# Darkkey/erlamsa

Measured on AMD Instinct MI355X. Metric: mutated_MB_per_s, higher is better.
Workload: dtype u8 (byte edits) + f64 (AS183 draws)

## Files before the change

erlamsa_amd/csrc/eh_common.h:

```cpp
#pragma once
#include <stdint.h>

#if defined(__HIP_DEVICE_COMPILE__) && !defined(HIPEMU)
#define EH_G __attribute__((address_space(1)))
#else
#define EH_G
#endif

namespace eh {

typedef EH_G uint8_t* bptr;   typedef const EH_G uint8_t* cbptr;
typedef EH_G uint32_t* wptr;  typedef const EH_G uint32_t* cwptr;
typedef EH_G uint64_t* qptr;  typedef const EH_G uint64_t* cqptr;

enum MutaId : int {
  M_SGM, M_JS, M_UW, M_UI, M_AB, M_AD, M_TR2, M_TD, M_NUM, M_TS1, M_TR, M_TS2, M_BD, M_BEI, M_BED,
  M_BF, M_BI, M_BER, M_BR, M_SP, M_SR, M_SD, M_SNAND, M_SRND, M_LD, M_LDS, M_LR2, M_LRI, M_LR,
  M_LS, M_LP, M_LIS, M_LRS, M_FT, M_FN, M_FO, M_LEN, M_B64, M_URI, M_ZIP, M_NIL, M_COUNT
};
enum PatId : int { P_OD, P_ND, P_BU, P_SK, P_SZ, P_CS, P_AR, P_CP, P_CO, P_NU, P_COUNT };
enum GenId : int { G_DIRECT = 0, G_RANDOM = 1, G_FILE = 2, G_JUMP = 3, G_COUNT = 4 };

enum CaseStatus : int { CASE_OK = 0, CASE_CRASHED = 1, CASE_OVERFLOW = 2, CASE_UNSUPPORTED = 3, CASE_ARENA_FULL = 4, CASE_BUDGET = 5 };

constexpr int MAX_FS = 64;
constexpr int MAX_BLOCKS = 2048;
constexpr int MAX_EMITS = 4096;
constexpr int MAX_FRAMES = 16;
constexpr uint32_t TRACE_CAP = 32768;

enum TraceKind : int {
  TRK_AA = 1,
  TRK_AI = 2,
  TRK_SIZER = 3,
  TRK_CSUM = 4,
  TRK_SKIPPED = 5,
  TRK_ARCHIVER = 6,
};
#define EH_ATOMS(X)                                                                                                              \
  X(sgm) X(js) X(uw) X(ui) X(ab) X(ad) X(tr2) X(td) X(num) X(ts1) X(tr) X(ts2) X(bd) X(bei) X(bed) X(bf) X(bi) X(ber) X(br) X(sp)  \
  X(sr) X(sd) X(snand) X(srnd) X(ld) X(lds) X(lr2) X(lri) X(lr) X(ls) X(lp) X(lis) X(lrs) X(ft) X(fn) X(fo) X(len) X(b64) X(uri)  \
  X(zip) X(nil)                                                                                                                   \
  X(failed) X(used) X(pattern) X(skipped_big) X(once_dec) X(many_dec) X(burst) X(skipper) X(sizer) X(csum) X(archiver)            \
  X(compressed) X(no_muta) X(mutate_once) X(empty_stopped) X(decompressed) X(gzip) X(zlib) X(ok) X(success) X(json)               \
  X(base64_mutator) X(sed_utf8_widen) X(sed_utf8_insert) X(ascii_bad) X(ascii_delimeter) X(tree_dup) X(tree_del) X(muta_num)      \
  X(tree_swap_one) X(tree_stutter) X(tree_swap_two) X(byte_drop) X(byte_inc) X(byte_dec) X(byte_flip) X(byte_insert)              \
  X(byte_swap_random) X(byte_repeat) X(seq_perm) X(seq_repeat) X(seq_drop) X(seq_randmask) X(line_del) X(line_del_seq)            \
  X(line_dup) X(line_clone) X(line_repeat) X(line_swap) X(line_perm) X(list_ins) X(list_replace) X(fuse_this) X(fuse_next)        \
  X(fuse_old) X(muta_len) X(muta_zippath) X(nomutation) X(json_swap) X(json_dup) X(json_pump) X(json_repeat) X(json_insert)       \
  X(json_unserialize) X(json_innertext) X(null) X(bool) X(sgml_swap) X(sgml_dup) X(sgml_pump) X(sgml_repeat) X(sgml_insert2)      \
  X(sgml_permparams) X(sgml_breaktag) X(sgml_insert) X(sgml_xmlfeatures) X(xmlns) X(sgml_innertext)
enum AtomId : int {
#define EH_ATOM_ENUM(n) AT_##n,
  EH_ATOMS(EH_ATOM_ENUM)
#undef EH_ATOM_ENUM
  AT_COUNT
};
static_assert((int)AT_nil == (int)M_NIL && (int)AT_sgm == (int)M_SGM && (int)AT_b64 == (int)M_B64, "the mutator codes are the first atoms, in MutaId order");
constexpr int POOL_TIERS = 8;

constexpr uint32_t INITIAL_IP = 24;
constexpr uint32_t AVG_BLOCK_SIZE = 2048;
constexpr uint32_t MIN_BLOCK_SIZE = 256;
constexpr uint32_t MAX_BLOCK_SIZE = 4096;
constexpr uint32_t ABSMAXHALF_BINARY_BLOCK = 500000;
constexpr uint32_t ABSMAX_BINARY_BLOCK = 1000000;
constexpr uint32_t SIZER_MAX_FIRST_BYTES = 512;
constexpr uint32_t PREAMBLE_MAX_BYTES = 32;

struct Blk {
  uint64_t ptr;
  uint32_t len;
  uint32_t aux;
};

struct RunState {
  uint32_t a1, a2, a3;
  int32_t gen;
  int32_t nfs;
  int32_t snand_mask;
  uint8_t fs_name[MAX_FS];
  uint8_t fs_score[MAX_FS];
  uint32_t fs_pri[MAX_FS];
};

struct DevConfig {
  int32_t nsel;
  uint8_t sel_name[MAX_FS];
  uint32_t sel_pri[MAX_FS];
  int32_t npat;
  int32_t pat_total;
  uint8_t pat_id[P_COUNT];
  uint32_t pat_pri[P_COUNT];
  int32_t ngen;
  int32_t gen_total;
  uint8_t gen_id[G_COUNT];
  uint32_t gen_pri[G_COUNT];
  uint32_t max_block_scaled;
  uint32_t min_block_scaled;
  char ssrf_host[64];
  char ssrf_port[12];
};

constexpr uint32_t MAX_PROFILES = 1024;
struct ProfileCfg {
  int32_t nsel;
  uint8_t sel_name[MAX_FS];
  uint32_t sel_pri[MAX_FS];
  int32_t npat;
  int32_t pat_total;
  uint8_t pat_id[P_COUNT];
  uint8_t pad[2];
  uint32_t pat_pri[P_COUNT];
  uint32_t max_block_scaled;
  uint32_t min_block_scaled;
};

constexpr uint32_t CO_JOBS = 64, CO_ARGS = 12;
enum CoKind : uint32_t { CO_COPY = 1, CO_EQUAL = 2, CO_FBPASS = 3, CO_FBCOUNT = 4 };
struct CoJob {
  uint64_t a[CO_ARGS];
  unsigned long long acc;
  uint32_t kind, nchunks, done, pad;
};
struct CoBoard {
  unsigned long long word[CO_JOBS];
  uint32_t owner[CO_JOBS];
  uint32_t open;
  uint32_t posters;
  uint32_t pad[14];
  unsigned long long stat[8];
  CoJob job[CO_JOBS];
};

struct KParams {
  cbptr corpus;
  cqptr coff;
  uint64_t corpus_first;
  uint64_t n_paths;
  uint64_t n;
  uint64_t first_case;
  int32_t mode;
  const EH_G RunState* run;
  const EH_G int64_t* seeds;
  DevConfig cfg;
  uint64_t work_cap;
  uint64_t work_budget;
  uint64_t fuse_stream_min;
  bptr out;
  uint64_t out_cap;
  EH_G unsigned long long* out_cursor;
  qptr out_off;
  qptr out_len;
  EH_G int32_t* status;
  qptr draws;
  EH_G int32_t* lastm;
  qptr cycles;
  qptr peak;
  qptr trace_off;
  wptr trace_len;
  uint32_t flags;
  EH_G unsigned long long* prof;
  EH_G unsigned long long* ticket;
  EH_G unsigned long long* in_bytes;
  bptr slot_base;
  uint64_t slot_stride;
  int32_t ntiers;
  bptr pool_base[POOL_TIERS + 1];
  uint64_t pool_stride[POOL_TIERS + 1];
  uint64_t pool_cap[POOL_TIERS + 1];
  uint32_t pool_cnt[POOL_TIERS + 1];
  wptr pool_ring[POOL_TIERS + 1];
  EH_G unsigned long long* pool_ctr;
  EH_G CoBoard* board;
  EH_G unsigned long long* summary_out;
  uint64_t batch_seq;
  uint32_t co_copy_min, co_copy_chunk;
  uint32_t co_fb_min, co_fb_chunk;
  uint32_t co_linger, pad_co;
  const EH_G ProfileCfg* profiles;
  const EH_G uint32_t* profile_id;
};

struct MutaInfo { const char* name; int pri; int on_gpu; };
struct PatInfo { const char* name; int pri; int on_gpu; };

}
```

erlamsa_amd/csrc/eh_device.h:

```cpp
#pragma once
#include <hip/hip_runtime.h>
#include <stdint.h>

#include "eh_common.h"

namespace eh {

#define EH_LANE ((int)threadIdx.x)
#define EH_DEV __device__ __forceinline__

EH_DEV uint32_t uni(uint32_t v) { return (uint32_t)__builtin_amdgcn_readfirstlane((int)v); }
EH_DEV uint64_t uni64(uint64_t v) { return ((uint64_t)uni((uint32_t)(v >> 32)) << 32) | uni((uint32_t)v); }
EH_DEV void wave_sync() { __syncthreads(); }

struct alignas(16) TabU16x65 { uint16_t v[65]; };
constexpr TabU16x65 as183_powers(uint32_t mult, uint32_t prime) {
  TabU16x65 t{};
  uint32_t a = 1;
  for (int k = 0; k <= 64; k++) { t.v[k] = (uint16_t)a; a = a * mult % prime; }
  return t;
}
__constant__ TabU16x65 c_T1 = as183_powers(171, 30269);
__constant__ TabU16x65 c_T2 = as183_powers(172, 30307);
__constant__ TabU16x65 c_T3 = as183_powers(170, 30323);
// ... 98 lines not shown
EH_DEV bool rng_occurs(Rng& r, uint32_t nom, uint32_t den) {
  uint32_t n = rng_rand(r, den);
  return nom == 1 ? (n != 0) : (n < nom);
}
EH_DEV uint32_t rng_log(Rng& r, uint32_t n) {
  if (n == 0) return 0;
  uint32_t k = rng_rand(r, n);
  if (k == 0) return 0;
  uint32_t hi = 1u << (k - 1);
  return hi | rng_rand(r, hi);
}

#ifdef HIPEMU
EH_DEV uint4 ldg16(const void* p) { uint4 v; memcpy(&v, p, 16); return v; }
EH_DEV uint4 ldg16a(const void* p) { uint4 v; memcpy(&v, p, 16); return v; }
EH_DEV void stg16(void* p, const uint4& v) { memcpy(p, &v, 16); }
EH_DEV void stg16a(void* p, const uint4& v) { memcpy(p, &v, 16); }
EH_DEV uint64_t ldg8(const void* p) { uint64_t v; memcpy(&v, p, 8); return v; }
EH_DEV uint32_t ldg4(const void* p) { uint32_t v; memcpy(&v, p, 4); return v; }
#else
typedef uint32_t eh_v4 __attribute__((ext_vector_type(4)));
typedef eh_v4 __attribute__((aligned(1))) eh_v4u;
typedef uint64_t __attribute__((aligned(1))) eh_u64u;
typedef uint32_t __attribute__((aligned(1))) eh_u32u;
EH_DEV uint4 ldg16(const EH_G void* p) { eh_v4 v = *reinterpret_cast<const EH_G eh_v4u*>(p); uint4 r; r.x = v.x; r.y = v.y; r.z = v.z; r.w = v.w; return r; }
EH_DEV uint4 ldg16a(const EH_G void* p) { eh_v4 v = *reinterpret_cast<const EH_G eh_v4*>(p); uint4 r; r.x = v.x; r.y = v.y; r.z = v.z; r.w = v.w; return r; }
EH_DEV void stg16(EH_G void* p, const uint4& r) { eh_v4 v; v.x = r.x; v.y = r.y; v.z = r.z; v.w = r.w; *reinterpret_cast<EH_G eh_v4u*>(p) = v; }
EH_DEV void stg16a(EH_G void* p, const uint4& r) { eh_v4 v; v.x = r.x; v.y = r.y; v.z = r.z; v.w = r.w; *reinterpret_cast<EH_G eh_v4*>(p) = v; }
EH_DEV uint64_t ldg8(const EH_G void* p) { return *reinterpret_cast<const EH_G eh_u64u*>(p); }
EH_DEV uint32_t ldg4(const EH_G void* p) { return *reinterpret_cast<const EH_G eh_u32u*>(p); }
#endif

#ifdef HIPEMU
constexpr uint32_t CO_COPY_MIN = 8u << 10;
#else
constexpr uint32_t CO_COPY_MIN = 256u << 10;
#endif
__device__ void co_copy(bptr dst, cbptr src, uint32_t n);
__device__ bool co_equal(cbptr a, cbptr b, uint32_t n);
EH_DEV void wave_copy_raw(bptr dst, cbptr src, uint32_t n) {
  const int l = EH_LANE;
  uint32_t head = (uint32_t)((16 - ((uintptr_t)dst & 15)) & 15);
  if (head > n) head = n;
  if ((uint32_t)l < head) dst[l] = src[l];
  dst += head; src += head; n -= head;
  uint32_t nv = n >> 4;
  uint32_t i = l;
  for (; i + 192 < nv; i += 256) {
    const uint4 v0 = ldg16(src + 16 * (size_t)i), v1 = ldg16(src + 16 * (size_t)(i + 64));
    const uint4 v2 = ldg16(src + 16 * (size_t)(i + 128)), v3 = ldg16(src + 16 * (size_t)(i + 192));
    stg16a(dst + 16 * (size_t)i, v0);
    stg16a(dst + 16 * (size_t)(i + 64), v1);
    stg16a(dst + 16 * (size_t)(i + 128), v2);
    stg16a(dst + 16 * (size_t)(i + 192), v3);
  }
  for (; i < nv; i += 64) {
    const uint4 v = ldg16(src + 16 * (size_t)i);
    stg16a(dst + 16 * (size_t)i, v);
  }
  uint32_t done = nv << 4;
  if (done + l < n) dst[done + l] = src[done + l];
}
EH_DEV void wave_copy(bptr dst, cbptr src, uint32_t n) {
  if (__builtin_expect(n >= CO_COPY_MIN, 0)) { co_copy(dst, src, n); return; }
  wave_copy_raw(dst, src, n);
}
EH_DEV void wave_move_down(bptr dst, cbptr src, uint32_t n) {
  const int l = EH_LANE;
  uint32_t nv = n >> 4;
  for (uint32_t base = 0; base < nv; base += 256) {
    uint4 v[4]; bool ok[4];
#pragma unroll
    for (int u = 0; u < 4; u++) { uint32_t i = base + 64u * u + (uint32_t)l; ok[u] = i < nv; if (ok[u]) v[u] = ldg16(src + 16 * (size_t)i); }
    wave_sync();
#pragma unroll
    for (int u = 0; u < 4; u++) { uint32_t i = base + 64u * u + (uint32_t)l; if (ok[u]) stg16(dst + 16 * (size_t)i, v[u]); }
  }
  uint32_t done = nv << 4;
  uint8_t t = 0; bool tk = done + (uint32_t)l < n;
  if (tk) t = src[done + l];
  wave_sync();
  if (tk) dst[done + l] = t;
}
EH_DEV void wave_fill_periodic(bptr dst, cbptr pat, uint32_t plen, uint64_t total) {
  if (total == 0) return;
  uint64_t have = plen < total ? plen : total;
  wave_copy(dst, pat, (uint32_t)have);
  while (have < total) {
    wave_sync();
    uint64_t chunk = have < total - have ? have : total - have;
    uint64_t done = 0;
    while (done < chunk) { uint32_t c = chunk - done > 0x40000000ull ? 0x40000000u : (uint32_t)(chunk - done); wave_copy(dst + have + done, dst + done, c); done += c; }
    have += chunk;
  }
}
EH_DEV bool wave_equal_raw(cbptr a, cbptr b, uint32_t n) {
  const int l = EH_LANE;
  uint32_t nv = n >> 4;
  for (uint32_t base = 0; base < nv; base += 128) {
    uint32_t i0 = base + l, i1 = base + 64 + l;
    bool ne = false;
    uint4 x0, y0, x1, y1;
    if (i0 < nv) { x0 = ldg16(a + 16 * (size_t)i0); y0 = ldg16(b + 16 * (size_t)i0); }
    if (i1 < nv) { x1 = ldg16(a + 16 * (size_t)i1); y1 = ldg16(b + 16 * (size_t)i1); }
    if (i0 < nv) ne |= (x0.x != y0.x) | (x0.y != y0.y) | (x0.z != y0.z) | (x0.w != y0.w);
    if (i1 < nv) ne |= (x1.x != y1.x) | (x1.y != y1.y) | (x1.z != y1.z) | (x1.w != y1.w);
    if (__ballot(ne) != 0) return false;
  }
  uint32_t done = nv << 4;
  bool ne = false;
  if (done + l < n) ne = a[done + l] != b[done + l];
  return __ballot(ne) == 0;
}
EH_DEV bool wave_equal(cbptr a, cbptr b, uint32_t n) {
  if (__builtin_expect(n >= CO_COPY_MIN, 0)) return co_equal(a, b, n);
  return wave_equal_raw(a, b, n);
}

constexpr int MAX_CHUNKS = POOL_TIERS + 1;
constexpr int MAX_NEST = 6;
constexpr int LEX_LEVELS = MAX_NEST + 1;
constexpr int ST_STATE_WORDS = 84;
#define EH_SET_OVERFLOW(c, site) ((c).ovf_line = (site), (c).ovf_need = 0, (c).ovf_req = 0, (c).status = CASE_OVERFLOW)
struct MuFrame;
struct Ctx {
  Rng rng;
  const EH_G KParams* p;
  EH_G Blk* bl;
  EH_G Blk* bl2;
  int nb, cur;
  EH_G Blk* em;
  int nem;
  uint32_t max_block_scaled;
  bptr aux;
  bptr ws;
  uint64_t ws_used, ws_cap;
  int nchunk;
  int view;
  uint64_t ws_lo;
  uint64_t ch_vstart[MAX_CHUNKS], ch_vend[MAX_CHUNKS]; bptr ch_base[MAX_CHUNKS]; uint32_t ch_area[MAX_CHUNKS]; int32_t ch_tier[MAX_CHUNKS];
  uint64_t lex_ptr[LEX_LEVELS];
  bptr trace;
  uint32_t ntrace, tr_base;
  uint32_t co_posted;
  int32_t call_req, mu_phase, call_nres, call_nfs;
  uint64_t call_bin; uint32_t call_len;
  EH_G MuFrame* mu;
  uint64_t t_case;
  uint32_t min_block_scaled;
  int32_t m_aux;
  uint64_t ws_peak, ws_top;
  int status;
  int lastm;
  uint64_t work;
  int r_kind;
  bptr r_ptr;
  uint32_t r_len;
  int r_flush;
  int r_drop_next;
  int r_changed;
  int r2; bptr r2_ptr; uint32_t r2_len;
  int nfs;
  uint64_t work_budget;
  uint64_t ovf_need, ovf_req;
  int ovf_line;
  int depth;
  int gen_pending;
  uint32_t gen_e1, gen_e2;
  int pat_ret; uint32_t pat_ip; int pat_cont;
  uint32_t fp_on, fp_g, fp_special, fp_keypos, fp_bA, fp_bB;
};
__shared__ Ctx g_ctx;
#ifdef HIPEMU
#define EH_LDS_ARRAY(type, name, n) static type name[n]
#define EH_KEEP(v) do {} while (0)
#else
// ... 35 lines not shown
  if (nb > 1) tr_b(c, b1);
  if (nv > 0) tr_v(c, v0);
  if (nv > 1) tr_v(c, v1);
  if (nv > 2) tr_v(c, v2);
}
__device__ __noinline__ void tr_name_emit(cbptr nm, uint32_t nl, uint32_t up) {
  Ctx& c = g_ctx;
  tr_b(c, TRK_ARCHIVER); tr_v(c, nl + 3u * up);
  for (uint32_t k = 0; k < up; k++) { tr_b(c, '.'); tr_b(c, '.'); tr_b(c, '/'); }
  for (uint32_t k = 0; k < nl; k++) tr_b(c, uni(nm[k]));
}
EH_DEV void tr_aa(Ctx& c, int a, int b) { if (__builtin_expect(c.trace != nullptr, 0)) tr_aa_emit(a, b); }
EH_DEV void tr_ai(Ctx& c, int a, int64_t v) { if (__builtin_expect(c.trace != nullptr, 0)) tr_ai_emit(a, v); }
EH_DEV void tr_drop_before(Ctx& c, uint32_t start) {
  if (!c.trace || start <= c.tr_base || c.ntrace >= TRACE_CAP) return;
  const uint32_t n = c.ntrace - start;
  wave_sync();
  if (n) wave_move_down(c.trace + c.tr_base, c.trace + start, n);
  wave_sync();
  c.ntrace = c.tr_base + n;
}

EH_DEV void pool_nap() {
#ifndef HIPEMU
  __builtin_amdgcn_s_sleep(64);
#else
  fprintf(stderr, "hipemu: a wait for a pool area can never end with one wavefront running (block %u)\n", blockIdx.x); abort();
#endif
}
EH_DEV uint32_t pool_pop(const EH_G KParams& p, int t) {
  uint32_t v = 0xFFFFFFFFu;
  if (EH_LANE == 0) {
    unsigned long long h = atomicAdd(&p.pool_ctr[2 * t], 1ull);
    wptr e = p.pool_ring[t] + (h % p.pool_cnt[t]);
    v = atomicExch(e, 0xFFFFFFFFu);
    if (v == 0xFFFFFFFFu) {
      uint64_t w0 = __builtin_readcyclecounter();
      for (;;) { pool_nap(); v = atomicExch(e, 0xFFFFFFFFu); if (v != 0xFFFFFFFFu) break; }
      atomicAdd(&p.pool_ctr[20 + t], (unsigned long long)(__builtin_readcyclecounter() - w0));
      atomicAdd(&p.pool_ctr[30 + t], 1ull);
    }
    unsigned long long back = atomicAdd(&p.pool_ctr[2 * t + 1], 0ull);
    unsigned long long outn = h + 1 + p.pool_cnt[t] > back ? h + 1 + p.pool_cnt[t] - back : 0;
    atomicMax(&p.pool_ctr[40 + t], outn);
  }
#ifndef EH_NO_POOL_FENCE
  __threadfence();
#endif
  return uni(v);
}
EH_DEV void pool_push(const EH_G KParams& p, int t, uint32_t v) {
#ifndef EH_NO_POOL_FENCE
  __threadfence();
#endif
  if (EH_LANE == 0) {
    unsigned long long h = atomicAdd(&p.pool_ctr[2 * t + 1], 1ull);
    wptr e = p.pool_ring[t] + (h % p.pool_cnt[t]);
    while (atomicCAS(e, 0xFFFFFFFFu, v) != 0xFFFFFFFFu) pool_nap();
  }
}

struct CoArgs { uint64_t a[CO_ARGS]; };
__device__ void co_exec(const EH_G CoJob* j, uint32_t t);
EH_DEV void co_nap() {
#ifndef HIPEMU
  __builtin_amdgcn_s_sleep(16);
#else
  fprintf(stderr, "hipemu: a wait for a helper's chunk can never end with one wavefront running (block %u)\n", blockIdx.x); abort();
#endif
}
EH_DEV void co_release() {
#ifndef HIPEMU
  __builtin_amdgcn_fence(__ATOMIC_RELEASE, "agent");
  asm volatile("s_waitcnt vmcnt(0)" ::: "memory");
#endif
}
EH_DEV void co_acquire() {
#ifndef HIPEMU
  __builtin_amdgcn_fence(__ATOMIC_ACQUIRE, "agent");
#endif
}
EH_DEV uint32_t co_ld32(const EH_G uint32_t* p) { return __atomic_load_n(p, __ATOMIC_RELAXED); }
EH_DEV unsigned long long co_ld64(const EH_G unsigned long long* p) { return __atomic_load_n(p, __ATOMIC_RELAXED); }
__device__ __noinline__ bool co_run(uint32_t kind, uint32_t nchunks, CoArgs args, unsigned long long* acc) {
  Ctx& c = g_ctx;
  EH_G CoBoard* bd = c.p ? c.p->board : nullptr;
  const int l = EH_LANE;
  if (!bd || nchunks < 2) return false;
  uint32_t slot = CO_JOBS;
  if (l == 0) {
    const uint32_t h = (blockIdx.x * 2654435761u) >> 26;
    for (uint32_t k = 0; k < 4 && slot == CO_JOBS; k++) { const uint32_t s = (h + 17u * k) & (CO_JOBS - 1); if (atomicCAS(&bd->owner[s], 0u, 1u) == 0u) slot = s; }
    if (slot == CO_JOBS) atomicAdd(&bd->stat[4], 1ull);
  }
  slot = uni(slot);
  if (slot == CO_JOBS) return false;
  EH_G CoJob* j = &bd->job[slot];
  unsigned long long gen = 0;
  if (l == 0) {
#pragma unroll
    for (uint32_t k = 0; k < CO_ARGS; k++) j->a[k] = args.a[k];
    j->kind = kind; j->nchunks = nchunks; j->done = 0; j->acc = 0;
  }
  wave_sync();
  co_release();
  if (l == 0) {
    if (!c.co_posted) atomicAdd(&bd->posters, 1u);
    gen = ((co_ld64(&bd->word[slot]) >> 32) + 1ull) | 1ull;
    atomicExch(&bd->word[slot], gen << 32);
    atomicAdd(&bd->open, 1u);
    atomicAdd(&bd->stat[0], 1ull);
  }
  c.co_posted = 1;
  uint32_t mine = 0;
  for (;;) {
    unsigned long long old = 0;
    if (l == 0) old = atomicAdd(&bd->word[slot], 1ull);
    const uint32_t t = uni((uint32_t)old);
    if (t >= nchunks) break;
    co_exec(j, t);
    mine++;
  }
  wave_sync();
  unsigned long long sum = 0;
  if (l == 0) {
    atomicAdd(&j->done, mine);
    const uint64_t w0 = __builtin_readcyclecounter();
    while (co_ld32(&j->done) < nchunks) co_nap();
    atomicAdd(&bd->open, 0xFFFFFFFFu);
    atomicExch(&bd->word[slot], (gen + 1ull) << 32);
    sum = co_ld64(&j->acc);
    atomicAdd(&bd->stat[2], (unsigned long long)mine);
    atomicAdd(&bd->stat[3], (unsigned long long)(__builtin_readcyclecounter() - w0));
  }
  sum = uni64(sum);
  co_acquire();
  if (l == 0) atomicExch(&bd->owner[slot], 0u);
  if (acc) *acc = sum;
  return true;
}
__device__ __noinline__ void co_help(EH_G CoBoard* bd, uint32_t most) {
  const int l = EH_LANE;
  uint32_t ran = 0;
  for (uint32_t guard = 0; guard < 64 && ran < most; guard++) {
    if (uni(co_ld32(&bd->open)) == 0) return;
    const unsigned long long w = co_ld64(&bd->word[l]);
    const bool cand = ((w >> 32) & 1ull) && (uint32_t)w < co_ld32(&bd->job[l].nchunks);
    unsigned long long m = __ballot(cand);
    if (!m) return;
    const uint32_t rot = blockIdx.x & 63u;
    const unsigned long long mr = rot ? ((m >> rot) | (m << (64u - rot))) : m;
    const uint32_t s = ((uint32_t)__builtin_ctzll(mr) + rot) & 63u;
    unsigned long long old = 0;
    if (l == 0) old = atomicAdd(&bd->word[s], 1ull);
    old = uni64(old);
    if (!((old >> 32) & 1ull)) continue;
    co_acquire();
    const EH_G CoJob* j = &bd->job[s];
    const uint32_t nchunks = uni(co_ld32(&j->nchunks)), t = (uint32_t)old;
    if (uni64(co_ld64(&bd->word[s])) >> 32 != old >> 32 || t >= nchunks) continue;
    co_exec(j, t);
    ran++;
    wave_sync();
    co_release();
    if (l == 0) { atomicAdd(&bd->job[s].done, 1u); atomicAdd(&bd->stat[1], 1ull); }
  }
}
__device__ __noinline__ void co_copy(bptr dst, cbptr src, uint32_t n) {
  const EH_G KParams* kp = g_ctx.p;
  if (!kp || !kp->board || n < kp->co_copy_min) { wave_copy_raw(dst, src, n); return; }
  const uint32_t ch = kp->co_copy_chunk;
  CoArgs a; for (uint32_t k = 0; k < CO_ARGS; k++) a.a[k] = 0;
  a.a[0] = (uint64_t)dst; a.a[1] = (uint64_t)src; a.a[2] = n; a.a[3] = ch;
  if (!co_run(CO_COPY, (n + ch - 1) / ch, a, nullptr)) wave_copy_raw(dst, src, n);
}
__device__ __noinline__ bool co_equal(cbptr x, cbptr y, uint32_t n) {
  const EH_G KParams* kp = g_ctx.p;
  if (!kp || !kp->board || n < 2 * kp->co_copy_min) return wave_equal_raw(x, y, n);
  const uint32_t ch = kp->co_copy_chunk;
  CoArgs a; for (uint32_t k = 0; k < CO_ARGS; k++) a.a[k] = 0;
  a.a[0] = (uint64_t)x; a.a[1] = (uint64_t)y; a.a[2] = n; a.a[3] = ch;
  unsigned long long ne = 0;
  if (!co_run(CO_EQUAL, (n + ch - 1) / ch, a, &ne)) return wave_equal_raw(x, y, n);
  return ne == 0;
}

struct LexChunk;
struct LexCache { uint64_t ptr; uint32_t len; int32_t n; EH_G LexChunk* tab; uint32_t tcap; uint32_t pad; };
constexpr uint32_t AUX_LEXCACHE = 2048;
constexpr uint64_t AUX_BYTES = 4096;
constexpr uint64_t SLOT_TABLE_BYTES = (uint64_t)(2 * MAX_BLOCKS + MAX_EMITS) * sizeof(Blk) + AUX_BYTES + TRACE_CAP;
EH_DEV EH_G LexCache& lex_slot(Ctx& c) { return ((EH_G LexCache*)(c.aux + AUX_LEXCACHE))[c.depth]; }
EH_DEV void lex_forget_from(Ctx& c, uint64_t v0) {
  const uint64_t key = c.lex_ptr[c.depth];
  if (key == 0) return;
  bool dead = false;
  for (int j = 0; j <= c.nchunk; j++) {
    uint64_t v = key - (uint64_t)(uintptr_t)c.ch_base[j], lo = v0 > c.ch_vstart[j] ? v0 : c.ch_vstart[j];
    if (v >= lo && v < c.ch_vstart[j] + c.p->pool_cap[c.ch_tier[j]]) dead = true;
  }
  if (dead) { c.lex_ptr[c.depth] = 0; if (EH_LANE == 0) lex_slot(c).n = -1; }
}
EH_DEV void ws_set_view(Ctx& c, int j) { c.view = j; c.ws = c.ch_base[j]; c.ws_lo = c.ch_vstart[j]; c.ws_cap = c.ch_vend[j]; }
EH_DEV bool ws_slow(Ctx& c, uint64_t need, int site) {
  int j = c.nchunk;
  while (j > 0 && c.ws_used < c.ch_vstart[j]) j--;
  for (; j <= c.nchunk; j++) {
    uint64_t at = c.ws_used > c.ch_vstart[j] ? c.ws_used : c.ch_vstart[j];
    if (at + need <= c.ch_vend[j]) { c.ws_used = at; ws_set_view(c, j); return true; }
  }
  const int k = c.nchunk;
  EH_SET_OVERFLOW(c, site); c.ovf_need = c.ws_used + need + (c.ch_vstart[k] + c.p->pool_cap[c.ch_tier[k]] - c.ch_vend[k]); c.ovf_req = need;
  return false;
}
EH_DEV uint64_t ws_max_request(const Ctx& c) { return c.p->pool_cap[c.p->ntiers]; }
EH_DEV bptr ws_alloc(Ctx& c, uint64_t n) {
  uint64_t need = (n + 15) & ~(uint64_t)15;
  if ((c.ws_used < c.ws_lo || c.ws_used + need > c.ws_cap) && !ws_slow(c, need, 102)) return nullptr;
  bptr p = c.ws + c.ws_used;
  c.ws_used += need;
  if (c.ws_used > c.ws_peak) c.ws_peak = c.ws_used;
  return p;
}
EH_DEV bptr ws_alloc_top(Ctx& c, uint64_t n) {
  uint64_t need = (n + 15) & ~(uint64_t)15;
  if ((c.ws_used < c.ws_lo || c.ws_used + need > c.ws_cap) && !ws_slow(c, need, 501)) return nullptr;
  c.ws_cap -= need; c.ch_vend[c.view] = c.ws_cap; c.ws_top += need;
  return c.ws + c.ws_cap;
}
__device__ __noinline__ void ws_release_to(Ctx&, uint64_t mark) {
  Ctx& c = g_ctx;
  c.ws_used = mark;
  while (c.nchunk > 0 && mark <= c.ch_vstart[c.nchunk]) {
    const int k = c.nchunk;
    const EH_G KParams& p = *c.p;
    bptr lo = c.ch_base[k] + c.ch_vstart[k]; bptr hi = lo + p.pool_cap[c.ch_tier[k]];
    for (int d = 0; d < LEX_LEVELS; d++) {
      EH_G LexCache* lc = (EH_G LexCache*)(c.aux + AUX_LEXCACHE) + d;
      uint64_t tab = uni64((uint64_t)lc->tab), key = c.lex_ptr[d];
      bool tin = uni(lc->tcap) != 0 && tab >= (uint64_t)lo && tab < (uint64_t)hi, kin = key >= (uint64_t)lo && key < (uint64_t)hi;
      if (tin || kin) { c.lex_ptr[d] = 0; if (EH_LANE == 0) { lc->n = -1; if (tin) lc->tcap = 0; } }
    }
    wave_sync();
    pool_push(p, c.ch_tier[k], c.ch_area[k]);
    c.nchunk = k - 1;
  }
  int j = c.nchunk;
  while (j > 0 && mark < c.ch_vstart[j]) j--;
  ws_set_view(c, j);
}
__device__ __noinline__ bool ws_regrow(Ctx&, uint64_t mark, int* last_tier) {
  Ctx& c = g_ctx;
  const EH_G KParams& p = *c.p;
  const uint64_t asked = c.ovf_need > mark ? c.ovf_need - mark : c.ovf_req, req = c.ovf_req;
  const int site = c.ovf_line;
  ws_release_to(c, mark);
  int tt = c.ch_tier[c.nchunk] + 1;
  if (tt <= *last_tier) tt = *last_tier + 1;
  while (tt < p.ntiers && p.pool_cap[tt] < asked + asked / 4) tt++;
  if (tt > p.ntiers || c.nchunk + 1 >= MAX_CHUNKS || req > p.pool_cap[tt] || asked > p.pool_cap[tt]) { EH_SET_OVERFLOW(c, site); return false; }
  wave_sync();
  const uint32_t area = pool_pop(p, tt);
  const int k = c.nchunk + 1;
  c.ch_vstart[k] = mark; c.ch_vend[k] = mark + p.pool_cap[tt]; c.ch_tier[k] = tt; c.ch_area[k] = area;
  c.ch_base[k] = (bptr)((uintptr_t)(p.pool_base[tt] + (uint64_t)area * p.pool_stride[tt]) - (uintptr_t)mark);
  c.nchunk = k;
  ws_set_view(c, k);
// ... 562 lines not shown
```

erlamsa_amd/csrc/eh_engine.hip:

```cpp
#include <hip/hip_runtime.h>
#include <stdio.h>
#include <stdlib.h>
#include <string.h>

#include <algorithm>
#include <atomic>
#include <condition_variable>
#include <map>
#include <mutex>
#include <thread>
#include <unordered_map>
#include <string>
#include <vector>

#include "../../include/erlamsa_hip.h"
#include "eh_otp_sort.h"
#include "eh_device.h"
#include "eh_text.h"
#include "eh_lex.h"
#include "eh_tree.h"
#include "eh_field.h"
#include "eh_fuse.h"
#include "eh_fuse2.h"
#include "eh_doc.h"
// ... 16 lines not shown
  switch (fn) {
    case M_LD: case M_LDS: case M_LR2: case M_LRI: case M_LR: case M_LS: case M_LP: return muta_line(c, (int)fn);
    case M_LIS: return muta_st_line(c, (int)fn, st);
    case M_LRS: return muta_st_line(c, (int)fn, st + 1);
    case M_NUM: return muta_num(c);
    case M_AB: case M_AD: return muta_ascii(c, lex_slot(c), (int)fn);
    case M_URI: return muta_uri(c, lex_slot(c));
    case M_B64: return muta_b64(c, lex_slot(c));
    case M_ZIP: return muta_zip(c);
    case M_LEN: return muta_len(c);
    case M_FT: case M_FN: case M_FO: return muta_fuse(c, (int)fn, (EH_G FoState*)(c.aux + 704));
    case M_TR2: case M_TD: case M_TS1: case M_TS2: case M_TR: return muta_tree(c, (int)fn);
    case M_SGM: return muta_sgml(c);
    case M_JS: return muta_json(c);
    default: c.status = CASE_UNSUPPORTED; c.r_kind = R_SAME; return 0;
  }
}

template <class Sel, class Gen>
EH_DEV void setup_run(const Sel& sel, const Gen& cfg, int64_t s1, int64_t s2, int64_t s3, Rng& rng, int& gen, int& snand_mask,
                      uint32_t& e_pri, uint32_t& e_meta, int& nfs) {
  const int l = EH_LANE;
  rng.draws = 0;
  rng_seed(rng, s1, s2, s3);
  snand_mask = (int)rng_rand(rng, 3);
  (void)rng_rand(rng, 1);
  nfs = sel.nsel;
  uint32_t score = 0;
  if (l < nfs) {
    double u = rng_peek(rng, (uint32_t)(nfs - 1 - l) + 1);
    uint32_t n = (uint32_t)(u * 10.0);
    score = n < 2 ? 2 : n;
  }
  rng_skip(rng, (uint64_t)nfs);
  uint32_t name = l < nfs ? sel.sel_name[l] : 0;
  e_pri = l < nfs ? sel.sel_pri[l] : 0;
  uint32_t mask = name == M_SNAND ? (uint32_t)snand_mask : 3u;
  e_meta = em_pack(score, name, name, mask);
  uint32_t g = rng_rand(rng, (uint32_t)cfg.gen_total);
  gen = cfg.gen_id[cfg.ngen - 1];
  for (int i = 0; i < cfg.ngen; i++) {
    if (g == 0 || g < cfg.gen_pri[i]) { gen = cfg.gen_id[i]; break; }
    g -= cfg.gen_pri[i];
  }
}
struct SelView { int32_t nsel; const EH_G uint8_t* sel_name; const EH_G uint32_t* sel_pri; };
template <class Pats>
EH_DEV int choose_pattern(const Pats& t, Rng& rng) {
  uint32_t r = rng_rand(rng, (uint32_t)t.pat_total);
  int pat = t.npat > 0 ? t.pat_id[t.npat - 1] : -1;
  for (int k = 0; k < t.npat; k++) {
    if (r == 0 || r < t.pat_pri[k]) { pat = t.pat_id[k]; break; }
    r -= t.pat_pri[k];
  }
  return pat;
}

__global__ void __launch_bounds__(64) eh_prologue_kernel(KParams p, int64_t s1, int64_t s2, int64_t s3, RunState* out_, KParams* params_out_,
                                                         unsigned long long* counters_) {
  EH_G RunState* out = (EH_G RunState*)out_; EH_G KParams* params_out = (EH_G KParams*)params_out_; EH_G unsigned long long* counters = (EH_G unsigned long long*)counters_;
  const int l = EH_LANE;
  for (int i = l; i < 512; i += 64) counters[i] = 0;
#ifdef EH_PROF
  if (l == 0) counters[8 + 2 * 127] = ~0ull;
#endif
  static_assert(sizeof(KParams) % 4 == 0, "KParams is copied word by word");
  cwptr src = (cwptr)&p;
  wptr dst = (wptr)params_out;
  for (int i = l; i < (int)(sizeof(KParams) / 4); i += 64) dst[i] = src[i];
  if (p.mode != 0) return;
  Rng rng; int gen, mask, nfs; uint32_t e_pri, e_meta;
  setup_run(p.cfg, p.cfg, s1, s2, s3, rng, gen, mask, e_pri, e_meta, nfs);
  if (l == 0) { out->a1 = rng.a1; out->a2 = rng.a2; out->a3 = rng.a3; out->gen = gen; out->nfs = nfs; out->snand_mask = mask; }
  if (l < nfs) { out->fs_name[l] = (uint8_t)em_name(e_meta); out->fs_score[l] = (uint8_t)em_score(e_meta); out->fs_pri[l] = e_pri; }
}

#include "eh_patterns.h"
#include "eh_gen.h"

__device__ __noinline__ void co_exec(const EH_G CoJob* j, uint32_t t) {
  const uint32_t kind = uni(co_ld32(&j->kind));
  const uint64_t a0 = uni64(j->a[0]), a1 = uni64(j->a[1]), a2 = uni64(j->a[2]);
  if (kind == CO_COPY || kind == CO_EQUAL) {
    const uint32_t ch = uni((uint32_t)j->a[3]);
    const uint64_t off = (uint64_t)t * ch;
    const uint32_t len = a2 - off < ch ? (uint32_t)(a2 - off) : ch;
    if (kind == CO_COPY) wave_copy_raw((bptr)a0 + off, (cbptr)a1 + off, len);
    else if (!wave_equal_raw((cbptr)a0 + off, (cbptr)a1 + off, len)) { if (EH_LANE == 0) atomicAdd((EH_G unsigned long long*)&j->acc, 1ull); }
    return;
  }
  if (kind == CO_FBPASS) { fb_pass_chunk(j, t); return; }
}

EH_DEV void sys_store(EH_G unsigned long long* p, unsigned long long v) {
#ifdef HIPEMU
  *p = v;
#else
  __hip_atomic_store(p, v, __ATOMIC_RELAXED, __HIP_MEMORY_SCOPE_SYSTEM);
#endif
}
constexpr int CTR_OCC = 272;
constexpr int CTR_STATUS = 264;
constexpr unsigned int CO_LINGER = 24;
#ifndef EH_WAVES_PER_SIMD
#define EH_WAVES_PER_SIMD 2
#endif
__global__ void __launch_bounds__(64, EH_WAVES_PER_SIMD) eh_mutate_kernel(const KParams* __restrict__ pp_) {
  const EH_G KParams* pp = (const EH_G KParams*)pp_;
  const int l = EH_LANE;
  const EH_G KParams& p = *pp;
  Ctx& c = g_ctx;
  LaneTab lt;
  c.p = pp;
  c.work_budget = p.work_budget;
#ifdef EH_PROF
  if (l == 0) { unsigned long long t = __builtin_amdgcn_s_memrealtime(); atomicMin(&pp->prof[2 * 127], t ? t : 1ull); atomicMax(&pp->prof[2 * 127 + 1], t); }
#endif
  const uint32_t slot_id = blockIdx.x;
  bptr slot = p.slot_base + (uint64_t)slot_id * p.slot_stride;
  c.bl = (EH_G Blk*)slot;
  c.bl2 = c.bl + MAX_BLOCKS;
  c.em = c.bl2 + MAX_BLOCKS;
  c.aux = (bptr)(c.em + MAX_EMITS);
  bptr const trace0 = c.aux + AUX_BYTES;
  bptr const ws0 = trace0 + TRACE_CAP;

  Rng parent; int gen0 = 0; uint32_t pri0 = 0, meta0 = 0; int nfs0 = 0;
  if (p.mode == 0) {
    const EH_G RunState* rs = p.run;
    parent.a1 = rs->a1; parent.a2 = rs->a2; parent.a3 = rs->a3; parent.draws = 0;
    gen0 = rs->gen; nfs0 = rs->nfs;
    if (l < nfs0) {
      uint32_t name = rs->fs_name[l];
      pri0 = rs->fs_pri[l];
      meta0 = em_pack(rs->fs_score[l], name, name, name == M_SNAND ? (uint32_t)rs->snand_mask : 3u);
    }
  }

  const unsigned long long wg_t0 = __builtin_amdgcn_s_memrealtime();
  unsigned long long case_ticks = 0, linger_ticks = 0;
  const uint64_t TICKET_BATCH = 4;
  uint64_t tk_next = 0, tk_end = 0;
  while (true) {
    if (tk_next == tk_end) {
      unsigned long long t = 0;
      if (l == 0) t = atomicAdd(p.ticket, (unsigned long long)TICKET_BATCH);
      tk_next = uni64(t); tk_end = tk_next + TICKET_BATCH;
    }
    if (p.board && uni(co_ld32(&p.board->open)) != 0) co_help(p.board, 2);
    uint64_t i = tk_next++;
    if (i >= p.n) {
#ifndef HIPEMU
      if (p.board) {
        unsigned int mine = p.co_linger;
        if (l == 0) mine = (unsigned int)atomicAdd(p.ticket + 4, 1ull);
        if (uni(mine) < p.co_linger) {
          const unsigned long long lg0 = __builtin_amdgcn_s_memrealtime();
          EH_G CoBoard* bd = p.board;
          for (uint32_t spins = 0; spins < (1u << 24); spins++) {
            if (uni64(co_ld64(p.ticket + 3)) >= p.n || uni(co_ld32(&bd->posters)) == 0) break;
            if (uni(co_ld32(&bd->open)) != 0) co_help(bd, 8);
            else { for (int z = 0; z < 6; z++) __builtin_amdgcn_s_sleep(127); }
          }
          linger_ticks = __builtin_amdgcn_s_memrealtime() - lg0;
        }
      }
#endif
      break;
    }
    c.co_posted = 0;
    const unsigned long long case_t0 = __builtin_amdgcn_s_memrealtime();
    uint64_t tick0 = __builtin_readcyclecounter();
#ifndef HIPEMU
    c.t_case = tick0;
#else
    c.t_case = 0;
#endif
    c.nchunk = 0; c.ws_peak = 0; c.ws_top = 0;
    c.trace = (p.flags & EH_FLAG_META_TRACE) ? trace0 : nullptr; c.ntrace = 0; c.tr_base = 0; c.m_aux = -1;
    c.ch_vstart[0] = 0; c.ch_vend[0] = p.work_cap; c.ch_base[0] = ws0; c.ch_tier[0] = 0; c.ch_area[0] = slot_id;
    ws_set_view(c, 0);
    for (int d = 0; d < LEX_LEVELS; d++) c.lex_ptr[d] = 0;
    unsigned long long base = 0; uint64_t total = 0;
    c.work = 0; c.depth = 0;
    c.status = CASE_OK; c.lastm = -1; c.nb = 0; c.cur = 0; c.nem = 0; c.ws_used = 0;
    c.r_kind = R_SAME; c.r_flush = 0; c.r_drop_next = 0; c.r2 = 0;
    if (l == 0) { ((EH_G StState*)c.aux)[0].count = 0; ((EH_G StState*)c.aux)[1].count = 0; for (int d = 0; d < LEX_LEVELS; d++) { EH_G LexCache& lc = ((EH_G LexCache*)(c.aux + AUX_LEXCACHE))[d]; lc.n = -1; lc.tcap = 0; } ((EH_G FoState*)(c.aux + 704))->has = 0; }
    wave_sync();
    int gen;
    Rng pr;
    c.max_block_scaled = p.cfg.max_block_scaled; c.min_block_scaled = p.cfg.min_block_scaled;
    if (p.mode == 0) {
      pr = parent;
      rng_skip(pr, 3 * (p.first_case + i - 1));
      gen = gen0; lt.e_pri = pri0; lt.e_meta = meta0; c.nfs = nfs0;
    } else {
      int mask;
      SelView sel = {p.cfg.nsel, p.cfg.sel_name, p.cfg.sel_pri};
      if (p.profile_id) {
        const EH_G ProfileCfg* pf = p.profiles + uni(p.profile_id[i]);
        c.max_block_scaled = uni(pf->max_block_scaled); c.min_block_scaled = uni(pf->min_block_scaled);
        sel.nsel = (int32_t)uni((uint32_t)pf->nsel); sel.sel_name = pf->sel_name; sel.sel_pri = pf->sel_pri;
      }
      setup_run(sel, p.cfg, p.seeds[3 * i], p.seeds[3 * i + 1], p.seeds[3 * i + 2], pr, gen, mask, lt.e_pri, lt.e_meta, c.nfs);
    }
#ifdef EH_PROF
#define EH_PH(k) do { uint64_t now_ = __builtin_readcyclecounter(); if (l == 0) { atomicAdd(&p.prof[2 * (64 + (k))], (unsigned long long)(now_ - ph0)); atomicAdd(&p.prof[2 * (64 + (k)) + 1], 1ull); } ph0 = now_; } while (0)
    uint64_t ph0 = __builtin_readcyclecounter();
#else
#define EH_PH(k) do {} while (0)
#endif
    int64_t t1 = (int64_t)rng_erand(pr, 99999), t2 = (int64_t)rng_erand(pr, 99999), t3 = (int64_t)rng_erand(pr, 99999);
    c.rng.draws = 0;
    rng_seed(c.rng, t1, t2, t3);

    uint64_t o0 = p.coff[p.corpus_first + i], o1 = p.coff[p.corpus_first + i + 1];
    o0 = uni64(o0); o1 = uni64(o1);
    EH_PH(0);
    c.gen_pending = 0;
    if (gen == G_DIRECT) gen_direct(c, p.corpus + o0, (uint32_t)(o1 - o0));
    else if (gen == G_RANDOM) gen_random(c);
    else if (gen == G_FILE) { c.gen_e1 = rng_erand(c.rng, (uint32_t)p.n_paths) - 1; c.gen_pending = G_FILE; }
    else { c.gen_e1 = rng_erand(c.rng, (uint32_t)p.n_paths) - 1; c.gen_e2 = rng_erand(c.rng, (uint32_t)p.n_paths) - 1; c.gen_pending = G_JUMP; }
    EH_PH(1);

    if (c.status == CASE_OK) {
      const int pat = p.mode != 0 && p.profile_id ? choose_pattern(p.profiles[uni(p.profile_id[i])], c.rng) : choose_pattern(p.cfg, c.rng);
      if (pat < 0) c.status = CASE_CRASHED; else run_patterns(c, lt, pat);
    }

    EH_PH(2);
    wave_sync();
    total = 0; base = 0;
    if (c.status == CASE_OK) for (int k = 0; k < c.nem; k++) total += blk_load(c.em, k).len;
    if (total > 0) {
      if (l == 0) base = atomicAdd(p.out_cursor, (unsigned long long)((total + 15) & ~15ull));
      base = uni64(base);
      if (base + total > p.out_cap) { c.status = CASE_ARENA_FULL; total = 0; }
    }
    if (total > 0) {
      uint64_t pos = base;
      for (int k = 0; k < c.nem; k++) { Blk b = blk_load(c.em, k); wave_copy(p.out + pos, (cbptr)b.ptr, b.len); pos += b.len; }
    }
    unsigned long long tbase = 0;
// ... 14 lines not shown
      atomicAdd(p.ticket + 5, (unsigned long long)total);
      atomicAdd(p.ticket + CTR_STATUS + (c.status >= 0 && c.status < 6 ? c.status : 1), 1ull);
    }
    wave_sync();
    if (c.nchunk > 0) ws_release_to(c, 0);
    if (l == 0) {
      p.out_off[i] = base; p.out_len[i] = total; p.status[i] = c.status;
      p.draws[i] = c.rng.draws; p.lastm[i] = c.status == CASE_OVERFLOW ? -c.ovf_line : c.lastm; p.cycles[i] = __builtin_readcyclecounter() - tick0;
      p.peak[i] = c.ws_peak + c.ws_top;
      if (p.flags & EH_FLAG_META_TRACE) { p.trace_off[i] = tbase; p.trace_len[i] = c.trace ? c.ntrace : 0u; }
    }
    case_ticks += __builtin_amdgcn_s_memrealtime() - case_t0;
    wave_sync();
  }
  wave_sync();
  unsigned long long left = 0;
  if (l == 0) {
    atomicAdd(p.ticket + 7, __builtin_amdgcn_s_memrealtime() - wg_t0);
    atomicAdd(p.ticket + CTR_OCC, case_ticks);
    atomicAdd(p.ticket + CTR_OCC + 1, linger_ticks);
  }
  if (l == 0) left = atomicAdd(p.ticket + 6, 1ull);
  if (uni64(left) + 1 == (unsigned long long)gridDim.x && p.summary_out) {
    if (l < 6) sys_store(p.summary_out + 3 + l, co_ld64(p.ticket + CTR_STATUS + l));
    if (l == 6) { sys_store(p.summary_out + 1, co_ld64(p.ticket + 5)); sys_store(p.summary_out + 2, p.n); }
    if (l == 7) { sys_store(p.summary_out + 10, co_ld64(p.ticket + 7)); sys_store(p.summary_out + 11, co_ld64(p.ticket + CTR_OCC)); sys_store(p.summary_out + 12, co_ld64(p.ticket + CTR_OCC + 1)); sys_store(p.summary_out + 13, (unsigned long long)gridDim.x); }
    wave_sync();
    if (l == 0) sys_store(p.summary_out + 9, p.batch_seq);
  }
}

__global__ void __launch_bounds__(64) eh_order_scan_kernel(const uint64_t* out_len_, uint64_t* ord_off_, uint64_t n) {
  cqptr out_len = (cqptr)out_len_; qptr ord_off = (qptr)ord_off_;
  const int l = EH_LANE;
  uint64_t run = 0;
  for (uint64_t base = 0; base < n; base += 64) {
    uint64_t i = base + (uint64_t)l;
    uint64_t v = i < n ? out_len[i] : 0;
    uint64_t inc = v;
#pragma unroll
    for (int d = 1; d < 64; d <<= 1) {
      uint64_t t = ((uint64_t)(uint32_t)__shfl_up((int)(uint32_t)(inc >> 32), d) << 32) | (uint32_t)__shfl_up((int)(uint32_t)inc, d);
      if (l >= d) inc += t;
    }
    if (i < n) ord_off[i] = run + inc - v;
    run += uni64(((uint64_t)(uint32_t)__shfl((int)(uint32_t)(inc >> 32), 63) << 32) | (uint32_t)__shfl((int)(uint32_t)inc, 63));
  }
  if (l == 0) ord_off[n] = run;
}
__global__ void __launch_bounds__(64) eh_order_gather_kernel(const uint8_t* src_, uint8_t* dst_, const uint64_t* out_off_, const uint64_t* out_len_,
                                                             const uint64_t* ord_off_, uint64_t n, uint64_t ord_base) {
  cbptr src = (cbptr)src_; bptr dst = (bptr)dst_; cqptr out_off = (cqptr)out_off_, out_len = (cqptr)out_len_, ord_off = (cqptr)ord_off_;
  for (uint64_t i = blockIdx.x; i < n; i += gridDim.x) {
    uint64_t len = uni64(out_len[i]), so = uni64(out_off[i]), d0 = uni64(ord_off[i]) - ord_base;
    uint64_t done = 0;
    while (done < len) { uint32_t c = len - done > 0x40000000ull ? 0x40000000u : (uint32_t)(len - done); wave_copy_raw(dst + d0 + done, src + so + done, c); done += c; }
  }
}

__global__ void __launch_bounds__(64) eh_test_copy_kernel(uint8_t* buf_, const uint32_t* jobs_, uint32_t njobs, uint32_t* eq_out_) {
  bptr buf = (bptr)buf_; cwptr jobs = (cwptr)jobs_; wptr eq_out = (wptr)eq_out_;
  g_ctx.p = nullptr;
  for (uint32_t j = blockIdx.x; j < njobs; j += gridDim.x) {
    uint32_t kind = jobs[5 * j], d = jobs[5 * j + 1], s = jobs[5 * j + 2], n = jobs[5 * j + 3], pl = jobs[5 * j + 4];
    if (kind == 0) wave_copy_raw(buf + d, buf + s, n);
    else if (kind == 1) wave_fill_periodic(buf + d, buf + s, pl, n);
    else if (kind == 2) { bool e = wave_equal_raw(buf + d, buf + s, n); if (EH_LANE == 0) eq_out[j] = e ? 1u : 0u; }
    else {
      MaskWin<4> a, b; a.p = buf + s; a.L = n; b.p = buf + s; b.L = n;
      mw_load(a, d, LexCls()); mw_load_ref(b, d, LexCls());
      uint32_t bad = 0;
      for (int k = 0; k < 4; k++) bad += a.m[k] != b.m[k] ? 1u : 0u;
      bad += a.inrange != b.inrange ? 1u : 0u;
      MaskWin<4> c2, d2; c2.p = buf + s; c2.L = n; d2.p = buf + s; d2.L = n;
      mw_load(c2, d, DelimCls()); mw_load_ref(d2, d, DelimCls());
      for (int k = 0; k < 4; k++) bad += c2.m[k] != d2.m[k] ? 1u : 0u;
      bad = wave_sum(bad);
      if (EH_LANE == 0) eq_out[j] = bad;
    }
    wave_sync();
  }
}

__global__ void __launch_bounds__(64) eh_test_zlib_kernel(int op, const uint8_t* in_, uint64_t n, uint8_t* out_, uint64_t cap, uint8_t* scratch_, uint64_t* res_) {
  cbptr in = (cbptr)in_; bptr out = (bptr)out_, scratch = (bptr)scratch_; qptr res = (qptr)res_;
  g_ctx.p = nullptr;
  uint64_t len = 0; int ok = 1;
  if (op <= 2) { len = z_compress((EH_G ZDef*)scratch, op, in, n, out, cap); ok = len != 0; }
  else {
    EH_G ZInf* zi = (EH_G ZInf*)scratch; uint64_t off = 0;
    ok = z_uncompress_size(zi, op - 3, in, n, &len, &off);
    if (ok && len > cap) ok = 0;
    if (ok) ok = z_uncompress_write(zi, op - 3, in, n, off, out, len);
  }
  if (EH_LANE == 0) { res[0] = len; res[1] = (uint64_t)ok; }
}

}

#include "eh_host_queues.h"
__attribute__((constructor)) static void eh_runtime_defaults() {
  const int want = eh::hw_queues_to_write(getenv("GPU_MAX_HW_QUEUES"));
  if (want) { char v[16]; snprintf(v, sizeof v, "%d", want); setenv("GPU_MAX_HW_QUEUES", v, 1); }
}

#include "eh_host.h"
#include "eh_host_pool.h"
#include "eh_host_launch.h"
#include "eh_host_corpus.h"
#include "eh_host_results.h"
#include "eh_host_coalesce.h"
#include "eh_host_options.h"
#include "eh_host_unique.h"
#include "eh_host_seen.h"
#include "eh_host_promote.h"
#include "eh_host_selftest.h"
```

erlamsa_amd/csrc/eh_fuse.h:

```cpp
#pragma once
#include "eh_field.h"

namespace eh {

struct FNode { uint32_t fo, fc, to, tc; };

EH_DEV uint32_t wave_sort64(uint32_t key) {
  const uint32_t l = (uint32_t)EH_LANE;
#pragma unroll
  for (uint32_t k2 = 2; k2 <= 64; k2 <<= 1) {
#pragma unroll
    for (uint32_t j = k2 >> 1; j > 0; j >>= 1) {
      uint32_t other = (uint32_t)__shfl_xor((int)key, (int)j);
      bool up = (l & k2) == 0 || k2 == 64, lower = (l & j) == 0;
      bool take_min = lower == up;
      uint32_t mn = key < other ? key : other, mx = key < other ? other : key;
      key = take_min ? mn : mx;
    }
  }
  return key;
}
EH_DEV uint32_t lanes_le(uint32_t v, uint32_t cnt, uint32_t x) {
  uint32_t lo = 0;
#pragma unroll
// ... 278 lines not shown
  EH_PT0;
  uint32_t from = la, tpos = lb;
  uint32_t prof_rounds = 0;
  c.fp_on = 0;
  if ((sym ? (uint64_t)la : (uint64_t)la + lb) > FL_NMAX && !c.work_budget && !(c.p->flags & EH_FLAG_FUSE_NO_REDUCE)) {
    const uint32_t rd = fr_peek_rounds(c.rng);
    if (rd < 64) {
      const uint32_t R = rd + 2u;
      uint32_t la2 = la, lb2 = lb;
      cbptr A2 = fr_reduce(c, A, &la2, R);
      if (!A2) return false;
      cbptr B2 = A2;
      if (sym) lb2 = la2; else { B2 = fr_reduce(c, B, &lb2, R); if (!B2) return false; }
      if ((uint64_t)la2 + lb2 <= ((uint64_t)la + lb) / 4u * 3u) {
        EH_PT(c, 97);
        c.fp_on = 1;
        bool ok;
        if ((sym ? (uint64_t)la2 : (uint64_t)la2 + lb2) <= FL_NMAX && !(c.p->flags & EH_FLAG_FUSE_NO_LDS)) ok = fuse_jump_lds(c, A2, la2, B2, lb2, sym, &from, &tpos, &prof_rounds);
        else ok = fuse_jump_stream(c, A2, la2, B2, lb2, sym, &from, &tpos, &prof_rounds);
        c.fp_on = 0;
        if (!ok) return false;
        EH_PT(c, 54);
        const uint32_t g = c.fp_g, par = g & 1u;
        from = la; tpos = lb;
        if (g == 0) { from = rng_rand(c.rng, la); tpos = rng_rand(c.rng, lb); }
        else if (c.fp_special) { (void)rng_rand(c.rng, 1); (void)rng_rand(c.rng, 1); }
        else {
          cbptr key = A2 + c.fp_keypos;
          const uint32_t limA = la > g ? la - g : 0u, limB = lb > g ? lb - g : 0u;
          const uint32_t fc0 = fr_occ(A, la, limA, key, g, FR_NONE, nullptr), fc = fc0 + c.fp_bA;
          uint32_t pos = 0;
          if (fc > 0) { uint32_t j = rng_rand(c.rng, fc); j = par ? fc - 1u - j : j; if (j < fc0) { (void)fr_occ(A, la, limA, key, g, j, &pos); from = uni(pos) + g; } }
          const uint32_t tc0 = sym ? fc0 : fr_occ(B, lb, limB, key, g, FR_NONE, nullptr), tc = tc0 + c.fp_bB;
          if (tc > 0) { uint32_t j = rng_rand(c.rng, tc); j = par ? tc - 1u - j : j; if (j < tc0) { (void)fr_occ(B, lb, limB, key, g, j, &pos); tpos = uni(pos) + g; } }
        }
        EH_PT(c, 55);
        goto jump;
      }
    }
    EH_PT(c, 98);
    c.ws_used = mark;
  }
  if ((sym ? (uint64_t)la : (uint64_t)la + lb) <= FL_NMAX && !(c.p->flags & EH_FLAG_FUSE_NO_LDS)) {
    if (!fuse_jump_lds(c, A, la, B, lb, sym, &from, &tpos, &prof_rounds)) { if (c.status == CASE_BUDGET) c.ws_used = mark; return false; }
  } else if ((uint64_t)la + lb >= c.p->fuse_stream_min) {
    if (!fuse_jump_stream(c, A, la, B, lb, sym, &from, &tpos, &prof_rounds)) { if (c.status == CASE_BUDGET) c.ws_used = mark; return false; }
  } else {
    FuseGen g[2];
    for (int k = 0; k < 2; k++) {
      g[k].nd = (EH_G FNode*)ws_alloc(c, ((uint64_t)la + 4) * sizeof(FNode));
      g[k].F = (wptr)ws_alloc(c, ((uint64_t)la + 4) * 4);
      g[k].T = sym ? g[k].F : (wptr)ws_alloc(c, ((uint64_t)lb + 4) * 4);
      if (!g[k].nd || !g[k].F || !g[k].T) return false;
    }
    if (la > 1) for (uint32_t i = l; i < la; i += 64) g[0].F[i] = i;
    if (lb > 1 && !sym) for (uint32_t i = l; i < lb; i += 64) g[0].T[i] = i;
    if (l == 0) { FNode n0; n0.fo = 0; n0.fc = la; n0.to = 0; n0.tc = lb; g[0].nd[0] = n0; }
    uint32_t nn = 1, par = 0;
    int64_t fuel = 100000;
    uint64_t gen_entries = (uint64_t)la + lb;
    wave_sync();
    while (true) {
      if (fuel < 0) break;
      if (rng_rand(c.rng, 8) == 0) break;
      if (c.work_budget) {
        c.work += 16ull * gen_entries;
        if (c.work > c.work_budget) { c.status = CASE_BUDGET; c.ws_used = mark; return false; }
      }
      uint32_t nchild = fuse_round(A, la, B, lb, g[par], nn, g[par ^ 1], par, sym, &gen_entries);
      if (nchild == 0) break;
      par ^= 1; nn = nchild;
      fuel -= (int64_t)nchild;
      prof_rounds++;
    }
    uint32_t ni = rng_rand(c.rng, nn);
    FNode nd = g[par].nd[par ? nn - 1 - ni : ni];
    uint32_t fo = uni(nd.fo), fc = uni(nd.fc), to = sym ? fo : uni(nd.to), tc = sym ? fc : uni(nd.tc);
    if (fc > 0) { uint32_t j = rng_rand(c.rng, fc); from = fc == 1 ? fo : uni(g[par].F[fo + (par ? fc - 1 - j : j)]); }
    if (tc > 0) { uint32_t j = rng_rand(c.rng, tc); tpos = tc == 1 ? to : uni(g[par].T[to + (par ? tc - 1 - j : j)]); }
  }
jump:
#ifdef EH_PROF
  {
    uint32_t tot = la + lb, b = 0; while ((256u << b) < tot && b < 13) b++;
    EH_PT(c, 112 + b);
    if (EH_LANE == 0) { atomicAdd(&c.p->prof[2 * 126], (unsigned long long)prof_rounds); atomicAdd(&c.p->prof[2 * 126 + 1], 1ull); }
  }
#endif
  c.ws_used = mark;
  uint32_t nl = from + (lb - tpos);
  bptr dst = ws_alloc(c, nl);
  if (!dst) return false;
  wave_copy(dst, A, from);
  wave_copy(dst + from, B + tpos, lb - tpos);
  wave_sync();
  *out = dst; *outlen = nl;
  return true;
}

struct FoState { uint64_t ptr; uint32_t len; uint32_t has; };

__device__ __noinline__ int muta_fuse(Ctx&, int fn, EH_G FoState* fo) {
  EH_CTX;
  Blk hb = blk_load(c.bl, c.cur);
  cbptr H = (cbptr)hb.ptr; uint32_t L = hb.len;
  c.r_kind = R_SAME;
  bptr r; uint32_t rl;
  if (fn == M_FT) {
    if (!fuse_lists(c, H, L, H, L, &r, &rl)) return 0;
    int d = rng_delta(c.rng);
    c.r_kind = R_NEW; c.r_ptr = r; c.r_len = rl;
    return d;
  }
  uint32_t h1 = L / 2;
  if (fn == M_FN) {
    Blk nb = hb; bool have_next = c.cur + 1 < c.nb;
    if (have_next) nb = blk_load(c.bl, c.cur + 1);
    bptr abl; uint32_t abll;
    if (!fuse_lists(c, H, h1, (cbptr)nb.ptr, nb.len, &abl, &abll)) return 0;
    if (!fuse_lists(c, abl, abll, H + h1, L - h1, &r, &rl)) return 0;
    int d = rng_delta(c.rng);
    c.r_kind = R_NEW; c.r_ptr = r; c.r_len = rl; c.r_flush = 1; c.r_drop_next = have_next ? 1 : 0;
    return d;
  }
  uint32_t has = uni(fo->has);
  uint64_t optr = has ? uni64(fo->ptr) : hb.ptr; uint32_t olen = has ? uni(fo->len) : L;
  uint32_t o1 = olen / 2;
  bptr a; uint32_t al; bptr b; uint32_t bl;
  if (!fuse_lists(c, H, h1, (cbptr)optr, o1, &a, &al)) return 0;
  if (!fuse_lists(c, (cbptr)optr + o1, olen - o1, H + h1, L - h1, &b, &bl)) return 0;
  uint32_t swap = rng_rand(c.rng, 3);
  int d = rng_delta(c.rng);
  if (EH_LANE == 0) { if (!has || swap == 0) { fo->ptr = hb.ptr; fo->len = L; } fo->has = 1; }
  wave_sync();
  c.r_kind = R_NEW; c.r_ptr = a; c.r_len = al; c.r_flush = 1;
  c.r2_ptr = b; c.r2_len = bl; c.r2 = 1;
  return d;
}

}
```

erlamsa_amd/csrc/eh_fuse2.h:

```cpp
#pragma once
#include "eh_fuse.h"

namespace eh {

constexpr uint32_t FB_DEAD = 0xFFFFFFFFu;
constexpr uint32_t FB_LDS_SC_NODES = 1024, FB_LDS_NEXT = 2048, FB_LDS_WORDS = 2048, FB_LDS_N1_NODES = 2048;
constexpr uint32_t FB_TEST_WORDS = 65536;
struct RkWord { uint32_t mask, prefix; };

EH_DEV uint32_t fb_tr(uint32_t b, uint32_t g) { return (g & 1u) ? 255u - b : b; }
EH_DEV uint32_t fb_ld(cwptr p) { return __atomic_load_n(p, __ATOMIC_RELAXED); }
EH_DEV uint32_t wave_min(uint32_t v) {
#pragma unroll
  for (int d = 32; d > 0; d >>= 1) { uint32_t t = (uint32_t)__shfl_xor((int)v, d); v = t < v ? t : v; }
  return uni(v);
}
EH_DEV void fb_clear(wptr p, uint32_t nwords) {
  uint4 z; z.x = z.y = z.z = z.w = 0;
  for (uint32_t i = 4u * (uint32_t)EH_LANE; i < nwords; i += 256) stg16a(p + i, z);
}

__device__ __noinline__ void fb_bits0(cbptr S, uint32_t len, wptr M) {
  const uint32_t l = (uint32_t)EH_LANE;
  for (uint32_t i = l; i < 256; i += 64) g_fuse_lds[i] = 0;
// ... 357 lines not shown
  const bool coop = c.p->board != nullptr && (la >= co_min || lb >= co_min);
  EH_PT0;
  uint32_t special_node = FB_DEAD;
  while (true) {
    if (fuel < 0) break;
    if (rng_rand(c.rng, 8) == 0) break;
    if (c.work_budget) {
      c.work += 16ull * gen_entries;
      if (c.work > c.work_budget) { c.status = CASE_BUDGET; return false; }
    }
    if (!ids[0]) {
      for (int s = 0; s < nside; s++) { ids[s] = (wptr)ws_alloc(c, ((uint64_t)len[s] + 8) * 4); if (!ids[s]) return false; }
    }
    if (nn > rk_rows) {
      rk_rows = nn < 1024u ? 1024u : nn;
      RK = (EH_G RkWord*)ws_alloc(c, ((uint64_t)rk_rows + 4) * 64);
      SC = (EH_G ScEnt*)ws_alloc(c, ((uint64_t)rk_rows + 4) * 8);
      if (!RK || !SC) return false;
    }
    if (nn > m_rows) {
      m_rows = nn < 1024u ? 1024u : nn;
      for (int s = 0; s < nside; s++) {
        M[s] = (wptr)ws_alloc(c, ((uint64_t)m_rows + 4) * 32); N1[s] = (wptr)ws_alloc(c, ((uint64_t)m_rows + 8) * 4);
        if (!M[s] || !N1[s]) return false;
        fb_clear(M[s], (m_rows + 4) * 8u); fb_clear(N1[s], (m_rows + 8u) & ~3u);
      }
      wave_sync();
    }
    const uint32_t nwords = nn * 8u;
    EH_PT(c, 100);
    if (!have_bits) for (int s = 0; s < nside; s++) fb_bits0(S[s], len[s], M[s]);
    EH_PT(c, 101);
    uint32_t e_pos[2] = {FB_DEAD, FB_DEAD}, e_alone[2] = {0, 0}, e_w[2] = {0, 0}, e_bit[2] = {0, 0};
    for (int s = 0; s < nside; s++) {
      if (len[s] < g + 1) continue;
      uint32_t ep = len[s] - 1 - g;
      uint32_t id = g == 0 ? 0u : uni(ids[s][ep]);
      if (id == FB_DEAD) continue;
      uint32_t b = fb_tr(uni(S[s][len[s] - 1]), g);
      e_pos[s] = ep; e_w[s] = id * 8u + (b >> 5); e_bit[s] = 1u << (b & 31u);
      e_alone[s] = fb_end_member(M[s], cur_n1 ? N1[s] : nullptr, id, b) ? 0u : 1u;
    }
    wave_sync();
    EH_PT(c, 102);
    const bool forced = !sym && e_pos[0] != FB_DEAD && e_alone[0];
    uint32_t sp = FB_DEAD, nfull = 0;
    uint32_t nchild = fb_scan(M[0], sym ? nullptr : M[1], cur_n1 ? N1[0] : nullptr, (cur_n1 && !sym) ? N1[1] : nullptr, nwords,
                              forced ? e_w[0] : FB_DEAD, forced ? e_bit[0] : 0u, RK, SC, &sp, &nfull);
    EH_PT(c, 103);
    if (nchild == 0) break;
    fuel -= (int64_t)nchild;
    const bool next = fuel >= 0 && (uint32_t)(rng_peek(c.rng, 1) * 8.0) != 0;
    const bool lds = next && nchild * 8u <= FB_LDS_WORDS && !coop;
    const bool n1 = next && !lds && nchild <= 2u * nn;
    const bool n1_lds = n1 && nchild <= FB_LDS_N1_NODES && !coop;
    const EH_G ScEnt* look = nfull * 4u <= nn ? SC : nullptr;
    const bool sc_lds = look && nn <= FB_LDS_SC_NODES;
    if (sc_lds) { cwptr scw = (cwptr)SC; lanes_sync(); for (uint32_t i = l; i < 2u * nn; i += 64) g_fuse_lds[i] = scw[i]; lanes_sync(); }
    if (next && nchild > m_rows) {
      m_rows = nchild;
      for (int s = 0; s < nside; s++) {
        M[s] = (wptr)ws_alloc(c, ((uint64_t)m_rows + 4) * 32); N1[s] = (wptr)ws_alloc(c, ((uint64_t)m_rows + 8) * 4);
        if (!M[s] || !N1[s]) return false;
        fb_clear(M[s], (m_rows + 4) * 8u); fb_clear(N1[s], (m_rows + 8u) & ~3u);
      }
      wave_sync();
    }
    uint64_t entries = 0;
    for (int s = 0; s < nside; s++) {
      if (lds) { for (uint32_t i = l; i < nchild * 8u; i += 64) g_fuse_lds[FB_LDS_NEXT + i] = 0; lanes_sync(); }
      if (n1_lds) { for (uint32_t i = l; i < nchild; i += 64) g_fuse_lds[FB_LDS_NEXT + i] = 0; lanes_sync(); }
      EH_PT(c, 104);
      bool ek = sym ? (!e_alone[0] && (g & 1u)) : (e_alone[s] || (g & 1u));
      uint32_t kill = (s == 1 && forced) ? sp : FB_DEAD;
      const int ins = lds ? 1 : n1_lds ? 4 : n1 ? 3 : (next && nchild * 8u <= FB_TEST_WORDS) ? 2 : 0;
      wptr mn = (ins == 0 && !next) ? nullptr : M[s]; wptr n1n = (ins == 3 || ins == 4) ? N1[s] : nullptr;
      uint32_t alive = 0;
      bool posted = false;
      if (coop && len[s] >= co_min) {
        CoArgs a; for (uint32_t k = 0; k < CO_ARGS; k++) a.a[k] = 0;
        a.a[0] = (uint64_t)S[s]; a.a[1] = (uint64_t)len[s] | ((uint64_t)g << 32); a.a[2] = (uint64_t)ids[s]; a.a[3] = (uint64_t)RK; a.a[4] = (uint64_t)look;
        a.a[5] = (uint64_t)kill | ((uint64_t)e_pos[s] << 32); a.a[6] = (ek ? 1u : 0u) | ((uint32_t)ins << 8) | (sc_lds ? 2u : 0u); a.a[7] = (uint64_t)mn; a.a[8] = (uint64_t)n1n; a.a[9] = nn; a.a[10] = co_chunk;
        unsigned long long acc = 0;
        posted = co_run(CO_FBPASS, (len[s] + co_chunk - 1) / co_chunk, a, &acc);
        alive = (uint32_t)acc;
      }
      if (!posted)
        alive = ins == 1 ? fb_pass<1>(S[s], len[s], ids[s], g, RK, look, sc_lds, kill, ek ? e_pos[s] : FB_DEAD, len[s], mn, nullptr)
              : ins == 4 ? fb_pass<4>(S[s], len[s], ids[s], g, RK, look, sc_lds, kill, ek ? e_pos[s] : FB_DEAD, len[s], mn, n1n)
              : ins == 3 ? fb_pass<3>(S[s], len[s], ids[s], g, RK, look, sc_lds, kill, ek ? e_pos[s] : FB_DEAD, len[s], mn, n1n)
              : ins == 2 ? fb_pass<2>(S[s], len[s], ids[s], g, RK, look, sc_lds, kill, ek ? e_pos[s] : FB_DEAD, len[s], mn, nullptr)
              : fb_pass<0>(S[s], len[s], ids[s], g, RK, look, sc_lds, kill, ek ? e_pos[s] : FB_DEAD, len[s], mn, nullptr);
      entries += alive;
      EH_PT(c, lds ? 105 : (n1_lds ? 96 : (n1 ? 111 : (next ? (nchild * 8u <= FB_TEST_WORDS ? 110 : 106) : 107))));
      if (lds) { lanes_sync(); for (uint32_t i = l; i < nchild * 8u; i += 64) M[s][i] = g_fuse_lds[FB_LDS_NEXT + i]; wave_sync(); }
      if (n1_lds) { lanes_sync(); for (uint32_t i = l; i < nchild; i += 64) N1[s][i] = g_fuse_lds[FB_LDS_NEXT + i]; wave_sync(); }
    }
    if (sym) entries *= 2; else if (forced) entries += 2;
    gen_entries = entries;
    special_node = forced ? sp : FB_DEAD;
    nn = nchild; g++; have_bits = next; cur_n1 = n1;
    EH_PT(c, 108);
    (*rounds)++;
  }
  const uint32_t par = g & 1u;
  uint32_t ni = rng_rand(c.rng, nn);
  uint32_t node = par ? nn - 1 - ni : ni;
  if (c.fp_on) {
    c.fp_g = g; c.fp_special = 0; c.fp_keypos = 0; c.fp_bA = 0; c.fp_bB = 0;
    if (g == 0) return true;
    if (node == special_node) { c.fp_special = 1; return true; }
    const uint32_t fcn = fb_count(ids[0], la, node);
    const uint32_t m0 = fb_find(ids[0], la, node, 0), ml = fb_find(ids[0], la, node, fcn - 1u);
    c.fp_keypos = m0;
    c.fp_special = (fcn == 1u && m0 + g == la) ? 1u : 0u;
    c.fp_bA = (ml + g == la) ? 1u : 0u;
    if (sym) c.fp_bB = c.fp_bA;
    else { const uint32_t tcn = fb_count(ids[1], lb, node); c.fp_bB = (tcn > 0 && fb_find(ids[1], lb, node, tcn - 1u) + g == lb) ? 1u : 0u; }
    EH_PT(c, 109);
    return true;
  }
  if (g == 0) {
    *from = rng_rand(c.rng, la);
    *tpos = rng_rand(c.rng, lb);
    return true;
  }
  if (node == special_node) { (void)rng_rand(c.rng, 1); (void)rng_rand(c.rng, 1); *from = la; *tpos = lb; return true; }
  uint32_t fc = fb_count(ids[0], la, node);
  uint32_t tc = sym ? fc : fb_count(ids[1], lb, node);
  uint32_t f = la, t = lb;
  if (fc > 0) { uint32_t j = rng_rand(c.rng, fc); f = fb_find(ids[0], la, node, par ? fc - 1 - j : j) + g; }
  if (tc > 0) { uint32_t j = rng_rand(c.rng, tc); t = fb_find(sym ? ids[0] : ids[1], lb, node, par ? tc - 1 - j : j) + g; }
  *from = f; *tpos = t;
  EH_PT(c, 109);
  return true;
}

}
```

erlamsa_amd/csrc/eh_host_launch.h:

```cpp
#pragma once
const uint64_t SEED_ROW = 3 * sizeof(int64_t) + sizeof(uint32_t);
static int ensure_seeds(eh_ctx* ctx, uint64_t n) {
  HIPCHK(ctx, ctx->profiles.d_table.grow(MAX_PROFILES));
  HIPCHK(ctx, ctx->res.d_seeds.grow(n * SEED_ROW));
  return EH_OK;
}
static int64_t* seeds_of(eh_ctx* ctx) { return (int64_t*)ctx->res.d_seeds.p; }
static uint32_t* profile_ids_of(eh_ctx* ctx) { return (uint32_t*)(seeds_of(ctx) + 3 * (ctx->res.d_seeds.cap / SEED_ROW)); }

static int ensure_results(eh_ctx* ctx, uint64_t n) {
  HIPCHK(ctx, ctx->res.d_cycles.grow(n));
  HIPCHK(ctx, ctx->res.d_peak.grow(n));
  HIPCHK(ctx, ctx->res.d_toff.grow(n));
  HIPCHK(ctx, ctx->res.d_tlen.grow(n));
  HIPCHK(ctx, ctx->res.d_off.grow(n));
  HIPCHK(ctx, ctx->res.d_len.grow(n));
  HIPCHK(ctx, ctx->res.d_status.grow(n));
  HIPCHK(ctx, ctx->res.d_draws.grow(n));
  HIPCHK(ctx, ctx->res.d_lastm.grow(n));
  return EH_OK;
}

static int reserve(eh_ctx* ctx, uint64_t n, uint64_t in_bytes) {
  HIPCHK(ctx, hipSetDevice(ctx->device));
  int rc = ensure_results(ctx, n ? n : 1);
  if (rc) return rc;
  uint64_t work_cap = ctx->max_case_bytes ? ctx->max_case_bytes : (8ull << 20);
  uint64_t big = ctx->big_case_bytes ? ctx->big_case_bytes : (32 * work_cap < (1024ull << 20) ? 32 * work_cap : (1024ull << 20));
  if (big < work_cap) big = work_cap;
  rc = pool_acquire(ctx, work_cap, big, ctx->pool_bytes_opt);
  if (rc) return rc;
  uint32_t want_slots = ctx->max_slots_opt ? ctx->max_slots_opt : (uint32_t)ctx->cus * 4u * EH_WAVES_PER_SIMD;
  if (want_slots > n) want_slots = (uint32_t)(n ? n : 1);
  uint64_t stride = (SLOT_TABLE_BYTES + work_cap + 255) & ~255ull;
  if (!ctx->d_slots || ctx->nslots < want_slots || ctx->slot_cap != work_cap) {
    HIPCHK(ctx, ctx->d_slots.reset(stride * want_slots));
    ctx->nslots = want_slots; ctx->slot_cap = work_cap; ctx->slot_stride = stride;
  }
  uint64_t want_out = ctx->out_capacity_opt ? ctx->out_capacity_opt : (8 * (in_bytes ? in_bytes : ctx->corpus.bytes) + (2048ull << 20));
  HIPCHK(ctx, ctx->res.d_out.grow(want_out));
  return EH_OK;
}

static int launch(eh_ctx* ctx, int mode, const int64_t seed[3], uint64_t first_case, uint64_t corpus_first, uint64_t n, hipStream_t st, bool profiled = false) {
  if (!ctx->configured || !ctx->corpus.d) { ctx->err = "configure and load a corpus first"; return EH_E_STATE; }
  if (corpus_first + n > ctx->corpus.n || (mode == 0 && first_case < 1)) { ctx->err = "case range outside the corpus"; return EH_E_INVALID; }
  if (ctx->corpus.n < (uint64_t)ctx->needs_paths || ctx->corpus.n > 0xFFFFFFFFull) { ctx->err = "generator file needs one corpus entry (path), jump two"; return EH_E_INVALID; }
  HIPCHK(ctx, hipSetDevice(ctx->device));
  uint64_t in_bytes = 0;
  if (!ctx->corpus.h_off.empty()) in_bytes = ctx->corpus.h_off[corpus_first + n] - ctx->corpus.h_off[corpus_first];
  int rc = reserve(ctx, n, in_bytes);
  if (rc) return rc;
  HIPCHK(ctx, ctx->res.d_counters.grow(512));
  HIPCHK(ctx, ctx->res.d_run.grow(1));
  HIPCHK(ctx, ctx->res.d_params.grow(1));
  if (!ctx->res.h_sum) { HIPCHK(ctx, hipHostMalloc((void**)&ctx->res.h_sum, 128, hipHostMallocDefault)); memset(ctx->res.h_sum, 0, 128); }

  KParams p;
  memset(&p, 0, sizeof(p));
  p.corpus = dp(ctx->corpus.d); p.coff = dp(ctx->corpus.d_off); p.corpus_first = corpus_first; p.n_paths = ctx->corpus.n; p.n = n; p.first_case = first_case;
  p.mode = mode; p.run = dp(ctx->res.d_run); p.seeds = dp(seeds_of(ctx)); p.cfg = ctx->cfg;
  if (profiled) { p.profiles = dp(ctx->profiles.d_table); p.profile_id = dp(profile_ids_of(ctx)); }
  const DevPool* pl = ctx->pool;
  p.work_cap = pl->work_cap;
  p.work_budget = ctx->work_budget;
  p.fuse_stream_min = ctx->fuse_stream_min;
  p.out = dp(ctx->res.d_out); p.out_cap = ctx->res.d_out.cap; p.out_cursor = dp(ctx->res.d_counters + 1);
  p.out_off = dp(ctx->res.d_off); p.out_len = dp(ctx->res.d_len); p.status = dp(ctx->res.d_status); p.draws = dp(ctx->res.d_draws); p.lastm = dp(ctx->res.d_lastm); p.cycles = dp(ctx->res.d_cycles); p.peak = dp(ctx->res.d_peak); p.trace_off = dp(ctx->res.d_toff); p.trace_len = dp(ctx->res.d_tlen); p.flags = ctx->flags;
  p.ticket = dp(ctx->res.d_counters); p.in_bytes = dp(ctx->res.d_counters + 2); p.prof = dp(ctx->res.d_counters + 8);
  p.slot_base = dp(ctx->d_slots); p.slot_stride = ctx->slot_stride;
  p.ntiers = pl->ntiers; p.pool_ctr = dp(pl->d_ctr); p.pool_cap[0] = pl->work_cap;
  p.board = (ctx->flags & EH_FLAG_NO_COOP) ? dp((CoBoard*)nullptr) : dp(pl->d_board);
  co_defaults(&p, ctx->cus);
  p.summary_out = dp(ctx->res.h_sum); p.batch_seq = ++ctx->res.batch_seq;
  if (n == 0) { memset(ctx->res.h_sum, 0, 128); ctx->res.h_sum[9] = ctx->res.batch_seq; }
  for (int t = 1; t <= pl->ntiers; t++) { p.pool_base[t] = dp(pl->base[t]); p.pool_stride[t] = pl->stride[t]; p.pool_cap[t] = pl->cap[t]; p.pool_cnt[t] = pl->cnt[t]; p.pool_ring[t] = dp(pl->ring[t]); }
  uint32_t grid0 = ctx->nslots < n ? ctx->nslots : (uint32_t)n;

  hipLaunchKernelGGL(eh_prologue_kernel, dim3(1), dim3(64), 0, st, p, mode == 0 ? seed[0] : 0, mode == 0 ? seed[1] : 0, mode == 0 ? seed[2] : 0,
                     ctx->res.d_run, ctx->res.d_params, ctx->res.d_counters);
  HIPCHK(ctx, hipEventRecord(ctx->res.ev0, st));
  if (n > 0) hipLaunchKernelGGL(eh_mutate_kernel, dim3(grid0), dim3(64), 0, st, (const KParams*)ctx->res.d_params);
  HIPCHK(ctx, hipEventRecord(ctx->res.ev1, st));
  HIPCHK(ctx, hipGetLastError());
  ctx->res.ordered = false;
  if ((ctx->flags & EH_FLAG_ORDERED_OUTPUT) && n > 0) {
    HIPCHK(ctx, ctx->res.d_out2.grow(ctx->res.d_out.cap));
    HIPCHK(ctx, ctx->res.d_ord.grow(n + 1));
    hipLaunchKernelGGL(eh_order_scan_kernel, dim3(1), dim3(64), 0, st, ctx->res.d_len, ctx->res.d_ord, n);
    uint32_t g = (uint32_t)ctx->cus * 32u; if (g > n) g = (uint32_t)n;
    hipLaunchKernelGGL(eh_order_gather_kernel, dim3(g), dim3(64), 0, st, ctx->res.d_out, ctx->res.d_out2, ctx->res.d_off, ctx->res.d_len, ctx->res.d_ord, n, 0ull);
    HIPCHK(ctx, hipMemcpyAsync(ctx->res.d_off, ctx->res.d_ord, n * 8, hipMemcpyDeviceToDevice, st));
    HIPCHK(ctx, hipGetLastError());
    ctx->res.d_out.swap(ctx->res.d_out2);
    ctx->res.ordered = true;
  }
  ctx->res.last_stream = st; ctx->res.last_n = n; ctx->res.last_in_bytes = in_bytes; ctx->res.have_result = true;
  return EH_OK;
}

int eh_create(int device, eh_ctx** out) {
  if (!out) return EH_E_INVALID;
  *out = nullptr;
  int count = 0;
  if (hipGetDeviceCount(&count) != hipSuccess || count <= 0 || device < 0 || device >= count) return EH_E_NODEVICE;
  eh_ctx* ctx = new (std::nothrow) eh_ctx();
  if (!ctx) return EH_E_NOMEM;
  ctx->device = device;
  if (hipSetDevice(device) != hipSuccess) { delete ctx; return EH_E_NODEVICE; }
  hipDeviceProp_t prop;
  if (hipGetDeviceProperties(&prop, device) != hipSuccess) { delete ctx; return EH_E_NODEVICE; }
  ctx->cus = prop.multiProcessorCount;
  if (hipEventCreate(&ctx->res.ev0) != hipSuccess || hipEventCreate(&ctx->res.ev1) != hipSuccess) {
    eh_destroy(ctx);
    return EH_E_HIP;
  }
  *out = ctx;
  return EH_OK;
}

void eh_destroy(eh_ctx* ctx) {
  if (!ctx) return;
  (void)hipSetDevice(ctx->device);
  (void)hipDeviceSynchronize();
  if (ctx->comm) { ehcomm::Api* a = ehcomm::api(); if (a->h) (void)a->CommDestroy(ctx->comm); ctx->comm = nullptr; }
  pool_release(ctx);
  delete ctx;
}

int eh_reserve(eh_ctx* ctx, uint64_t max_cases) {
  if (!ctx) return EH_E_INVALID;
  if (!ctx->configured || !ctx->corpus.d) { ctx->err = "configure and load a corpus first"; return EH_E_STATE; }
  std::lock_guard<std::mutex> g(ctx->co_lock);
  int rc = reserve(ctx, max_cases, 0);
  return rc ? rc : ensure_seeds(ctx, max_cases);
}

int eh_fuzz_batch(eh_ctx* ctx, const int64_t seed[3], uint64_t first_case, uint64_t corpus_first, uint64_t n, void* stream) {
  if (!ctx || !seed) return EH_E_INVALID;
  std::lock_guard<std::mutex> g(ctx->co_lock); if (int rc = co_idle(ctx)) return rc;
  return launch(ctx, 0, seed, first_case, corpus_first, n, (hipStream_t)stream);
}
static int fuzz_calls(eh_ctx* ctx, const int64_t* seeds, const uint32_t* profile, uint64_t corpus_first, uint64_t n, void* stream) {
  if (profile) {
    if (!ctx->configured) { ctx->err = "configure first"; return EH_E_STATE; }
    const uint32_t count = (uint32_t)ctx->profiles.list.size();
    for (uint64_t i = 0; i < n; i++) if (profile[i] >= count) { ctx->err = "case " + std::to_string(i) + ": no profile " + std::to_string(profile[i]) + " (eh_profile_count = " + std::to_string(count) + ")"; return EH_E_INVALID; }
  }
  HIPCHK(ctx, hipSetDevice(ctx->device));
  int rc = ensure_seeds(ctx, n);
  if (rc) return rc;
  if (n) { HIPCHK(ctx, hipStreamSynchronize((hipStream_t)stream)); HIPCHK(ctx, hipMemcpy(seeds_of(ctx), seeds, n * 24, hipMemcpyHostToDevice)); }
  if (profile && n) {
    HIPCHK(ctx, hipMemcpy(profile_ids_of(ctx), profile, n * 4, hipMemcpyHostToDevice));
    const uint32_t have = ctx->profiles.on_device, count = (uint32_t)ctx->profiles.list.size();
    if (count > have) HIPCHK(ctx, hipMemcpy(ctx->profiles.d_table + have, ctx->profiles.list.data() + have, (size_t)(count - have) * sizeof(ProfileCfg), hipMemcpyHostToDevice));
// ... 58 lines not shown
```

erlamsa_amd/csrc/eh_host_pool.h:

```cpp
#pragma once
static std::mutex g_pool_lock;
static std::vector<DevPool*> g_pools;

static void pool_free(DevPool* pl) {
  (void)hipSetDevice(pl->device);
  (void)hipDeviceSynchronize();
  delete pl;
}
static void pool_release(eh_ctx* ctx) {
  if (!ctx->pool) return;
  std::lock_guard<std::mutex> g(g_pool_lock);
  DevPool* pl = ctx->pool; ctx->pool = nullptr;
  if (--pl->refs > 0) return;
  for (size_t i = 0; i < g_pools.size(); i++) if (g_pools[i] == pl) { g_pools.erase(g_pools.begin() + i); break; }
  pool_free(pl);
}
static int pool_acquire(eh_ctx* ctx, uint64_t work_cap, uint64_t big, uint64_t pool_bytes_opt) {
  if (ctx->pool && ctx->pool->work_cap == work_cap && ctx->pool->big == big && ctx->pool->pool_bytes_opt == pool_bytes_opt) return EH_OK;
  pool_release(ctx);
  std::lock_guard<std::mutex> g(g_pool_lock);
  for (DevPool* q : g_pools)
    if (q->device == ctx->device && q->work_cap == work_cap && q->big == big && q->pool_bytes_opt == pool_bytes_opt) { q->refs++; ctx->pool = q; return EH_OK; }
  DevPool* pl = new (std::nothrow) DevPool();
  if (!pl) return EH_E_NOMEM;
  pl->device = ctx->device; pl->work_cap = work_cap; pl->big = big; pl->pool_bytes_opt = pool_bytes_opt;
  pl->cap[0] = work_cap;
  uint32_t SHARE[POOL_TIERS] = {12, 23, 17, 7, 10, 10, 9, 12};
  if (const char* ev = getenv("EH_POOL_SHARES")) {
    uint32_t v[POOL_TIERS]; int k = 0;
    for (const char* q = ev; *q && k < POOL_TIERS; ) { char* end = nullptr; unsigned long x = strtoul(q, &end, 10); if (end == q) break; v[k++] = (uint32_t)x; q = *end ? end + 1 : end; }
    if (k == POOL_TIERS) { bool ok = true; for (int i = 0; i < k; i++) ok = ok && v[i] >= 1 && v[i] <= 1000; if (ok) memcpy(SHARE, v, sizeof(v)); }
  }
  size_t fr = 0, tot = 0;
  hipError_t e = hipSuccess;
  uint64_t pool_bytes = pool_bytes_opt;
  if (!pool_bytes) { pool_bytes = 16ull << 30; if (hipMemGetInfo(&fr, &tot) == hipSuccess) { pool_bytes = (uint64_t)fr / 4; if (pool_bytes > (64ull << 30)) pool_bytes = 64ull << 30; if (pool_bytes < (1ull << 30)) pool_bytes = 1ull << 30; } }
  uint64_t caps[POOL_TIERS]; int nt = 0;
  for (uint64_t cap = work_cap; cap < big && nt < POOL_TIERS; ) { cap = (cap * 2 < big && nt < POOL_TIERS - 1) ? cap * 2 : big; caps[nt++] = cap; }
  uint32_t share_sum = 0;
  for (int k = 0; k < nt; k++) share_sum += SHARE[k == nt - 1 ? POOL_TIERS - 1 : k];
  for (int k = 0; k < nt; k++) {
    uint64_t stride_t = (caps[k] + 255) & ~255ull;
    uint64_t cnt = pool_bytes / share_sum * SHARE[k == nt - 1 ? POOL_TIERS - 1 : k] / stride_t; if (cnt < 1) cnt = 1; if (cnt > 4096) cnt = 4096;
    if (ctx->cus < 64 && cnt > 2) cnt = 2;
    int t = pl->ntiers + 1;
    for (; cnt >= 1; cnt /= 2) { e = pl->base[t].grow(stride_t * cnt); if (e == hipSuccess) break; }
    if (e != hipSuccess) break;
    pl->stride[t] = stride_t; pl->cap[t] = caps[k]; pl->cnt[t] = (uint32_t)cnt; pl->ntiers++;
  }
  uint64_t nring = 4;
  for (int t = 1; t <= pl->ntiers; t++) nring += pl->cnt[t];
  std::vector<uint32_t> init(nring);
  std::vector<unsigned long long> ctr(64, 0ull);
  if (pl->d_rings.grow(nring) != hipSuccess || pl->d_ctr.grow(64) != hipSuccess) { pool_free(pl); ctx->err = "work-area pool: out of device memory"; return EH_E_NOMEM; }
  uint64_t o = 0;
  for (int t = 1; t <= pl->ntiers; t++) {
    pl->ring[t] = pl->d_rings + o;
    for (uint32_t k = 0; k < pl->cnt[t]; k++) init[o + k] = k;
    ctr[2 * t] = 0; ctr[2 * t + 1] = pl->cnt[t];
    o += pl->cnt[t];
  }
  if (hipMemcpy(pl->d_rings, init.data(), nring * 4, hipMemcpyHostToDevice) != hipSuccess ||
      hipMemcpy(pl->d_ctr, ctr.data(), 64 * 8, hipMemcpyHostToDevice) != hipSuccess) { pool_free(pl); ctx->err = "work-area pool: hipMemcpy failed"; return EH_E_HIP; }
  if (pl->d_board.grow(1) != hipSuccess || hipMemset(pl->d_board, 0, sizeof(CoBoard)) != hipSuccess) { pool_free(pl); ctx->err = "work-area pool: no memory for the cooperation board"; return EH_E_NOMEM; }
  pl->refs = 1; g_pools.push_back(pl); ctx->pool = pl;
  return EH_OK;
}

static uint32_t co_env(const char* name, uint32_t dflt) { const char* v = getenv(name); if (!v || !*v) return dflt; unsigned long long x = strtoull(v, nullptr, 10); return x > 0 && x < (1ull << 31) ? (uint32_t)x : dflt; }
static void co_defaults(KParams* p, int cus) {
  const bool emu = cus < 64;
  p->co_copy_min = co_env("EH_CO_COPY_MIN", emu ? (8u << 10) : (2u << 20));
  p->co_copy_chunk = co_env("EH_CO_COPY_CHUNK", emu ? (2u << 10) : (256u << 10));
  p->co_fb_min = co_env("EH_CO_FB_MIN", emu ? (16u << 10) : (512u << 10));
  p->co_fb_chunk = co_env("EH_CO_FB_CHUNK", emu ? (4u << 10) : (64u << 10)) & ~1023u;
  { const char* v = getenv("EH_CO_LINGER"); p->co_linger = v && *v ? (uint32_t)strtoul(v, nullptr, 10) : CO_LINGER; p->pad_co = 0; }
  if (p->co_copy_chunk < 1024) p->co_copy_chunk = 1024;
  if (p->co_fb_chunk < 1024) p->co_fb_chunk = 1024;
}

int eh_pool_stats(eh_ctx* ctx, uint64_t* out ) {
  if (!ctx || !out) return EH_E_INVALID;
  if (!ctx->pool) { ctx->err = "no work-area pool yet (eh_reserve or a first batch creates it)"; return EH_E_STATE; }
  HIPCHK(ctx, hipSetDevice(ctx->device));
  uint64_t raw[64];
  HIPCHK(ctx, hipMemcpy(raw, ctx->pool->d_ctr, 64 * 8, hipMemcpyDeviceToHost));
  memcpy(out, raw, 40 * 8);
  out[40] = (uint64_t)ctx->pool->ntiers;
  for (int t = 0; t <= POOL_TIERS; t++) {
    out[41 + t] = t >= 1 && t <= ctx->pool->ntiers ? (uint64_t)ctx->pool->cnt[t] | (raw[40 + t] << 32) : 0;
    out[51 + t] = t <= ctx->pool->ntiers ? ctx->pool->cap[t] : 0;
  }
  out[61] = (uint64_t)ctx->pool->refs; out[62] = ctx->nslots; out[63] = 0;
  return EH_OK;
}
int eh_coop_stats(eh_ctx* ctx, uint64_t* out ) {
  if (!ctx || !out) return EH_E_INVALID;
  if (!ctx->pool) { ctx->err = "no work-area pool yet (eh_reserve or a first batch creates it)"; return EH_E_STATE; }
  HIPCHK(ctx, hipSetDevice(ctx->device));
  HIPCHK(ctx, hipMemcpy(out, (const uint8_t*)ctx->pool->d_board.p + offsetof(CoBoard, stat), 8 * 8, hipMemcpyDeviceToHost));
  return EH_OK;
}
```

erlamsa_amd/csrc/eh_host_selftest.h:

```cpp
#pragma once
int eh_selftest_movers(eh_ctx* ctx, uint8_t* buf, uint64_t buf_len, const uint32_t* jobs, uint32_t njobs, uint32_t* eq_out) {
  if (!ctx || !buf || !jobs) return EH_E_INVALID;
  HIPCHK(ctx, hipSetDevice(ctx->device));
  DevBuf<uint8_t> d_buf; DevBuf<uint32_t> d_jobs, d_eq;
  hipError_t e = d_buf.grow(buf_len);
  if (e == hipSuccess) e = d_jobs.grow(5 * (uint64_t)njobs);
  if (e == hipSuccess) e = d_eq.grow(njobs);
  uint8_t* d = d_buf; uint32_t* dj = d_jobs; uint32_t* de = d_eq;
  if (e == hipSuccess) e = hipMemcpy(d, buf, buf_len, hipMemcpyHostToDevice);
  if (e == hipSuccess) e = hipMemcpy(dj, jobs, njobs * 20, hipMemcpyHostToDevice);
  if (e == hipSuccess) e = hipMemset(de, 0, njobs * 4);
  if (e == hipSuccess) {
    hipLaunchKernelGGL(eh_test_copy_kernel, dim3(njobs < 256 ? njobs : 256), dim3(64), 0, 0, d, dj, njobs, de);
    e = hipDeviceSynchronize();
  }
  if (e == hipSuccess) e = hipMemcpy(buf, d, buf_len, hipMemcpyDeviceToHost);
  if (e == hipSuccess && eq_out) e = hipMemcpy(eq_out, de, njobs * 4, hipMemcpyDeviceToHost);
  HIPCHK(ctx, e);
  return EH_OK;
}
int eh_selftest_zlib(eh_ctx* ctx, int op, const uint8_t* in, uint64_t n, uint8_t* out, uint64_t cap, uint64_t* out_len, int32_t* ok) {
  if (!ctx || (!in && n) || !out || !out_len || !ok || op < 0 || op > 5 || op == 3 || (op <= 2 && cap < 64)) return EH_E_INVALID;
  HIPCHK(ctx, hipSetDevice(ctx->device));
  DevBuf<uint8_t> d_in, d_out, d_scratch; DevBuf<uint64_t> d_res;
  hipError_t e = d_in.grow(n + 16);
  if (e == hipSuccess) e = d_out.grow(cap + 16);
  if (e == hipSuccess) e = d_scratch.grow(sizeof(ZDef) > sizeof(ZInf) ? sizeof(ZDef) : sizeof(ZInf));
  if (e == hipSuccess) e = d_res.grow(2);
  uint8_t* di = d_in; uint8_t* dout = d_out; uint8_t* ds = d_scratch; uint64_t* dr = d_res;
  if (e == hipSuccess && n) e = hipMemcpy(di, in, n, hipMemcpyHostToDevice);
  uint64_t r[2] = {0, 0};
  if (e == hipSuccess) {
    hipLaunchKernelGGL(eh_test_zlib_kernel, dim3(1), dim3(64), 0, 0, op, (const uint8_t*)di, n, dout, cap, ds, dr);
    e = hipDeviceSynchronize();
  }
  if (e == hipSuccess) e = hipMemcpy(r, dr, 16, hipMemcpyDeviceToHost);
  if (e == hipSuccess && r[1] && r[0] <= cap && r[0]) e = hipMemcpy(out, dout, r[0], hipMemcpyDeviceToHost);
  HIPCHK(ctx, e);
  *out_len = r[0]; *ok = (int32_t)r[1];
  return EH_OK;
}
int eh_selftest_sort_by_priority(const uint32_t* pri, uint32_t n, uint32_t* perm) {
  if ((!pri || !perm) && n) return EH_E_INVALID;
  PL in;
  for (uint32_t i = 0; i < n; i++) in.push_back(PItem{pri[i], (int)i});
  PL out = otp_sort_desc_strict(in);
  for (uint32_t i = 0; i < n; i++) perm[i] = (uint32_t)out[i].id;
  return EH_OK;
}
```

erlamsa_amd/csrc/eh_sgml.h:

```cpp
#pragma once
#include "eh_doc.h"

namespace eh {

enum { E_LT = 1, E_GT, E_WS, E_EQ, E_SL, E_SQ, E_DQ, E_DASH, E_QM, E_BANG, E_SLGT, E_QGT, E_CMTEND, E_SPACE };
constexpr uint32_t ES_WS = (1u << E_WS) | (1u << E_SPACE);
constexpr uint32_t ES_EV = ES_WS | (1u << E_GT) | (1u << E_EQ);
constexpr uint32_t ES_STOP = ES_EV | (1u << E_SLGT);
constexpr uint32_t ES_DASH = (1u << E_DASH) | (1u << E_CMTEND);
EH_DEV uint32_t sg_class(uint32_t b) {
  const uint64_t t0 = ((uint64_t)E_WS << 36) | ((uint64_t)E_WS << 40) | ((uint64_t)E_WS << 52);
  const uint64_t t2 = ((uint64_t)E_SPACE << 0) | ((uint64_t)E_BANG << 4) | ((uint64_t)E_DQ << 8) | ((uint64_t)E_SQ << 28) | ((uint64_t)E_DASH << 52) | ((uint64_t)E_SL << 60);
  const uint64_t t3 = ((uint64_t)E_LT << 48) | ((uint64_t)E_EQ << 52) | ((uint64_t)E_GT << 56) | ((uint64_t)E_QM << 60);
  uint64_t t = b < 16 ? t0 : (b < 32 ? 0ull : (b < 48 ? t2 : t3));
  return b < 64 ? (uint32_t)((t >> (4 * (b & 15))) & 15) : 0u;
}

__constant__ uint8_t c_sglit[24] = {'<', '>', ' ', '=', '\'', '"', '<', '/', ' ', '/', '>', '<', '?', '?', '>', '<', '!', '<', '!', '-', '-', '-', '-', '>'};
enum { SL_LT = 0, SL_GT = 1, SL_SP = 2, SL_EQ = 3, SL_SQ = 4, SL_DQ = 5, SL_LTSL = 6, SL_SPSLGT = 8, SL_LTQ = 11, SL_QGT = 13, SL_LTBANG = 15, SL_CMT = 17, SL_CMTEND = 21 };
EH_DEV cbptr sglit(int k) { return (cbptr)&c_sglit[k]; }

enum { TK_OPEN = 1, TK_CLOSE = 2, TK_SC = 3, TK_TEXT = 4, TK_BANG = 5, TK_COMMENT = 6, TK_QUE = 7, TK_KIND = 0xFF, TF_EMPTY = 0x100, TF_PAIRED = 0x200 };
struct SgTok { uint32_t kind, p0, np, na, nb, par0, npar; int32_t match; };
struct SgParam { uint32_t na, nb, va, vb, delim, pad; };
// ... 194 lines not shown
  };
  auto find_stop = [&](uint32_t from) -> uint32_t {
    uint32_t i = from;
    for (int k = 0; k < 8; k++) { if (!have(i)) return nev; if ((ES_STOP >> (EV(i) & 15u)) & 1u) return i; i++; }
    if (!have(i)) return nev;
    const uint32_t j = mm.nstop[i];
    if (j < nev && j >= reach) reach = j + 1;
    return j;
  };
  do {
    if (pos >= L) break;
    const uint32_t ca = cls_here();
    if (ca == E_SLGT || ca == E_GT || ca == E_EQ) break;
    R.an = pos;
    step1();
    const uint32_t ja = find_stop(ei);
    if (ja >= nev || bail) break;
    R.ae = EV(ja) >> 4; pos = R.ae; ei = ja;
    skipws();
    R.va = pos; R.vb = pos;
    if (pos < L && cls_here() == E_EQ) {
      R.eqpos = pos;
      step1(); skipws();
      if (pos >= L) break;
      const uint32_t cv = cls_here();
      if (cv == E_SQ || cv == E_DQ) {
        const uint32_t ff = cv == E_SQ ? mm.sq : mm.dq;
        uint32_t i = ei + 1, jq = nev;
        if (i < ff) { while (have(i)) { if ((EV(i) & 15u) == cv) { jq = i; break; } i++; } }
        if (jq >= nev) break;
        R.va = pos + 1; R.vb = EV(jq) >> 4; R.delim = cv == E_SQ ? 1u : 2u;
        pos = R.vb + 1; ei = jq + 1;
      } else {
        const uint32_t ju = find_stop(ei);
        if (ju >= nev || bail) break;
        R.va = pos; R.vb = EV(ju) >> 4; pos = R.vb; ei = ju;
      }
      skipws();
    }
    if (bail) break;
    R.term = 0; R.npos = pos; R.nei = ei; R.nws = ws_sp ? 1u : 0u;
  } while (false);
  R.reach = reach;
  return R;
}

__device__ __noinline__ int sgml_tokenize(Ctx&, cbptr H, uint32_t L, SgDoc* out) {
  EH_CTX;
  const int l = EH_LANE;
#ifdef EH_PROF
  const uint64_t ph1_t0 = __builtin_readcyclecounter();
#endif
  wptr ev = (wptr)ws_alloc(c, ((uint64_t)L + 80) * 4);
  if (!ev) return -3;
  uint32_t nev = 0, nlt = 0, nstop = 0;
  for (uint32_t tb = 0; tb < L; tb += 1024) {
    uint32_t i0 = tb + 16u * (uint32_t)l;
    uint8_t b[18];
    if (i0 + 18 <= L) { uint4 v = ldg16(H + i0); __builtin_memcpy(b, &v, 16); b[16] = H[i0 + 16]; b[17] = H[i0 + 17]; }
    else { for (uint32_t k = 0; k < 18; k++) b[k] = i0 + k < L ? H[i0 + k] : 0; }
    uint32_t cls[16]; uint32_t cnt = 0, lts = 0, stops = 0;
#pragma unroll
    for (uint32_t k = 0; k < 16; k++) {
      uint32_t x = b[k];
      uint32_t cl = i0 + k < L ? sg_class(x) : 0u;
      if (cl == E_SL && b[k + 1] == '>') cl = E_SLGT;
      if (cl == E_QM && b[k + 1] == '>') cl = E_QGT;
      if (cl == E_DASH && b[k + 1] == '-' && b[k + 2] == '>') cl = E_CMTEND;
      cls[k] = cl; cnt += cl ? 1u : 0u; lts += cl == E_LT ? 1u : 0u; stops += (cl == E_WS || cl == E_SPACE || cl == E_GT || cl == E_EQ || cl == E_SL || cl == E_SLGT) ? 1u : 0u;
    }
    uint32_t inc = wave_incl_scan(cnt);
    uint32_t o = nev + inc - cnt;
#pragma unroll
    for (uint32_t k = 0; k < 16; k++) if (cls[k]) ev[o++] = ((i0 + k) << 4) | cls[k];
    nev += (uint32_t)__builtin_amdgcn_readlane((int)inc, 63);
    nlt += lts; nstop += stops;
  }
  nlt = wave_sum(nlt); nstop = wave_sum(nstop);
#ifdef EH_PROF
  uint64_t sub_t0 = __builtin_readcyclecounter();
#define SG_SUB0() do { sub_t0 = __builtin_readcyclecounter(); } while (0)
#define SG_SUB(k) do { uint64_t n_ = __builtin_readcyclecounter(); if (l == 0) { atomicAdd(&c.p->prof[2 * (k)], (unsigned long long)(n_ - sub_t0)); atomicAdd(&c.p->prof[2 * (k) + 1], 1ull); } sub_t0 = n_; } while (0)
#define SG_CNT(k, v) do { if (l == 0) { atomicAdd(&c.p->prof[2 * (k)], (unsigned long long)(v)); atomicAdd(&c.p->prof[2 * (k) + 1], 1ull); } } while (0)
  if (l == 0) { atomicAdd(&c.p->prof[2 * 117], (unsigned long long)(sub_t0 - ph1_t0)); atomicAdd(&c.p->prof[2 * 117 + 1], 1ull); atomicAdd(&c.p->prof[2 * 119], (unsigned long long)nev); atomicAdd(&c.p->prof[2 * 119 + 1], (unsigned long long)L); }
  uint64_t tz_t0 = __builtin_readcyclecounter();
#define SG_TZ(k) do { uint64_t n_ = __builtin_readcyclecounter(); if (l == 0) { atomicAdd(&c.p->prof[2 * (k)], (unsigned long long)(n_ - tz_t0)); atomicAdd(&c.p->prof[2 * (k) + 1], 1ull); } tz_t0 = n_; } while (0)
#else
#define SG_TZ(k) do {} while (0)
#define SG_SUB0() do {} while (0)
#define SG_SUB(k) do {} while (0)
#define SG_CNT(k, v) do {} while (0)
#endif
  if (nlt == 0) return -1;
  uint32_t cap_tok = 2 * nlt + 8, cap_par = nstop + 8;
  uint64_t cap_pc = 4ull * cap_tok + (uint64_t)SG_PARPCS * cap_par + nlt + 32;
  EH_G SgTok* tok = (EH_G SgTok*)ws_alloc(c, (uint64_t)cap_tok * sizeof(SgTok));
  EH_G SgParam* par = (EH_G SgParam*)ws_alloc(c, (uint64_t)cap_par * sizeof(SgParam));
  EH_G Piece* pc = (EH_G Piece*)ws_alloc(c, cap_pc * sizeof(Piece));
  if (!tok || !par || !pc) return -3;
  wave_sync();
  uint32_t ntok = 0, npar = 0, npc = 0;

  constexpr uint32_t SG_EVC = 4096, SG_EVBACK = 512;
  uint32_t cbase = 0xFFFFFFFFu;
  uint32_t bev = 0, bbase = 0xFFFFFFFFu;
  uint32_t reach_ev = 0;
  auto need = [&](uint32_t i) {
    if (bbase != 0xFFFFFFFFu && i >= bbase && i < bbase + 64) return;
    bbase = i & ~63u;
    if (bbase + 64 > reach_ev) reach_ev = bbase + 64;
    if (cbase == 0xFFFFFFFFu || bbase < cbase || bbase + 64 > cbase + SG_EVC) {
      cbase = bbase > SG_EVBACK ? bbase - SG_EVBACK : 0u;
      lanes_sync();
      for (uint32_t k0 = 0; k0 < SG_EVC; k0 += 256) {
        uint32_t v[4];
#pragma unroll
        for (int u = 0; u < 4; u++) { uint32_t j = cbase + k0 + 64u * (uint32_t)u + (uint32_t)l; v[u] = j < nev ? ev[j] : 0u; }
#pragma unroll
        for (int u = 0; u < 4; u++) g_fuse_lds[k0 + 64u * (uint32_t)u + (uint32_t)l] = v[u];
      }
      lanes_sync();
    }
    bev = g_fuse_lds[bbase - cbase + (uint32_t)l];
  };
  auto find = [&](uint32_t from, uint32_t set) -> uint32_t {
    while (from < nev) {
      need(from);
      unsigned long long m = __ballot(((set >> (bev & 15u)) & 1u) != 0 && bbase + (uint32_t)l >= from && bbase + (uint32_t)l < nev);
      if (m) return bbase + (uint32_t)__builtin_ctzll(m);
      from = bbase + 64;
    }
    return nev;
  };
  auto evget = [&](uint32_t i) -> uint32_t { need(i); return (uint32_t)__builtin_amdgcn_readlane((int)bev, (int)(i - bbase)); };
  uint32_t ff_gt = nev, ff_qgt = nev, ff_cmt = nev, ff_sq = nev, ff_dq = nev;
  auto find1 = [&](uint32_t from, uint32_t cls, uint32_t& ff) -> uint32_t {
    if (from >= ff) return nev;
    uint32_t j = find(from, 1u << cls);
    if (j >= nev) ff = from;
    return j;
  };
  wptr nstop_tab = nullptr;
  auto build_nstop = [&]() __attribute__((always_inline)) -> bool {
    EH_CTX;
    nstop_tab = (wptr)ws_alloc(c, ((uint64_t)nev + 64) * 4);
    if (!nstop_tab) return false;
#ifdef EH_PROF
    const uint64_t bn_t0 = __builtin_readcyclecounter();
#endif
    uint32_t carry = nev;
    for (uint32_t base = (nev - 1) & ~63u;; base -= 64) {
      uint32_t j = base + (uint32_t)l; uint32_t e = j < nev ? ev[j] : 0u;
      unsigned long long ms = __ballot(j < nev && ((ES_STOP >> (e & 15u)) & 1u));
      unsigned long long mm = ms & ~((1ull << l) - 1);
      if (j < nev) nstop_tab[j] = mm ? base + (uint32_t)__builtin_ctzll(mm) : carry;
      if (ms) carry = base + (uint32_t)__builtin_ctzll(ms);
      if (base == 0) break;
    }
    wave_sync();
#ifdef EH_PROF
    if (l == 0) { atomicAdd(&c.p->prof[2 * 116], (unsigned long long)(__builtin_readcyclecounter() - bn_t0)); atomicAdd(&c.p->prof[2 * 116 + 1], 1ull); }
#endif
    return true;
  };
  auto find_stop = [&](uint32_t from, uint32_t set) -> uint32_t {
    if (from >= nev) return nev;
    need(from);
    unsigned long long m = __ballot(((set >> (bev & 15u)) & 1u) != 0 && bbase + (uint32_t)l >= from && bbase + (uint32_t)l < nev);
    if (m) return bbase + (uint32_t)__builtin_ctzll(m);
    from = bbase + 64;
    if (from >= nev) return nev;
    if (!nstop_tab && !build_nstop()) return 0xFFFFFFFFu;
    for (;;) {
      uint32_t j = uni(nstop_tab[from]);
      if (j >= nev) return nev;
      if (set == ES_STOP || ((set >> (evget(j) & 15u)) & 1u)) return j;
      from = j + 1;
      if (from >= nev) return nev;
    }
  };
  uint32_t pos = 0, ei = 0;
  auto cls_here = [&]() -> uint32_t { if (ei >= nev) return 0u; uint32_t e = evget(ei); return (e >> 4) == pos ? (e & 15u) : 0u; };
  auto step1 = [&]() { if (ei < nev && (evget(ei) >> 4) == pos) ei++; pos++; };
  bool ws_sp = false;
  auto skipws = [&]() {
    ws_sp = false;
    while (ei < nev) {
      need(ei);
      uint32_t off = ei - bbase;
      bool ok = (uint32_t)l >= off && bbase + (uint32_t)l < nev && ((ES_WS >> (bev & 15u)) & 1u) && (bev >> 4) == pos + ((uint32_t)l - off);
      unsigned long long notok = ~__ballot(ok) & ~((1ull << off) - 1);
      uint32_t run = notok ? (uint32_t)__builtin_ctzll(notok) - off : 64u - off;
      if (run > 0) ws_sp = ((uint32_t)__builtin_amdgcn_readlane((int)bev, (int)(off + run - 1)) & 15u) == E_SPACE;
      pos += run; ei += run;
      if (off + run < 64) break;
    }
  };
  auto put = [&](cbptr p, uint32_t len) { if (l == 0) { Piece q; q.ptr = (uint64_t)p; q.len = len; q.rep = 1; pc[npc] = q; } npc++; };

  const bool lanes_on = !(c.p->flags & EH_FLAG_SGML_NO_LANES);
  static_assert(4096 + 64 <= EH_FUSE_LDS_WORDS, "g_fuse_lds: event window + the batch's '<' list");
  uint32_t rp_P = 0, rp_lo = 0, rp_end = 0;
  int rp_state = 0, rp_tries = 0;
  uint32_t rq_lo[4], rq_end[4], rq_P[4]; int rq_n = 0, rp_budget = 8; uint32_t rp_scan_from = 0;
  auto rp_detect = [&](uint32_t a, uint32_t b) __attribute__((always_inline)) -> bool {
    EH_CTX;
    if (rp_budget <= 0 || rq_n >= 4 || b <= a || b - a < 16384u) return false;
    rp_budget--;
    uint32_t u = 0, D = 0, P = 0;
    const bool found = fr_find_cut(H + a, b - a, 0, &u, &D, &P) && P > 0;
#ifdef EH_PROF
    if (l == 0) { atomicAdd(&c.p->prof[2 * 95 + 1], 1ull); atomicAdd(&c.p->prof[2 * 95], found ? 1ull : 0ull); }
#endif
    if (!found) return false;
    rq_lo[rq_n] = a + u - P; rq_end[rq_n] = a + u + D; rq_P[rq_n] = P; rq_n++;
    return true;
  };
  auto rp_load = [&](uint32_t at) __attribute__((always_inline)) {
    rp_P = 0; rp_state = 0; rp_tries = 0;
    for (;;) {
      while (rq_n > 0 && (uint64_t)at + 4ull * rq_P[rq_n - 1] > rq_end[rq_n - 1]) rq_n--;
      if (rq_n == 0) {
        const uint32_t from = at > rp_scan_from ? at : rp_scan_from;
        if (!rp_detect(from, L)) return;
        rp_scan_from = rq_end[rq_n - 1];
        continue;
      }
      const int top = rq_n - 1;
      if (rq_lo[top] > at && rq_lo[top] - at >= 32768u && rp_detect(at, rq_lo[top])) continue;
      rp_P = rq_P[top]; rp_lo = rq_lo[top]; rp_end = rq_end[top]; rq_n--;
      return;
    }
  };
  if (L >= 16384 && nlt >= 64 && !(c.p->flags & EH_FLAG_SGML_NO_REPLAY)) rp_load(0);
  uint32_t rp_s0 = 0, rp_tok0 = 0, rp_pc0 = 0, rp_par0 = 0, rp_e0 = 0, rp_dtok = 0, rp_dpc = 0, rp_dpar = 0, rp_de = 0, rp_reach1 = 0;
  bptr bad = nullptr; wptr chain = nullptr; uint32_t nchain = 0;
  int rc = 0;
  bool first = true;
  uint32_t lt = 0, seg_start = 0, text_p0 = 0, text_len = 0, seg_slot = 0;
  auto after_accept = [&]() __attribute__((always_inline)) -> int {
    EH_CTX;
      if (rp_P) {
        if (rp_state == 1 && pos == rp_s0 + rp_P) {
          rp_dtok = ntok - rp_tok0; rp_dpc = npc - rp_pc0; rp_dpar = npar - rp_par0; rp_de = ei - rp_e0; rp_reach1 = reach_ev; rp_state = 2;
// ... 278 lines not shown
      skipws();
      uint32_t nattr = 0;
      for (;;) {
        if (npc + 16 > cap_pc || npar + 1 > cap_par) { EH_SET_OVERFLOW(c, 602); return -3; }
        if (pos >= L) break;
        if (nattr >= 2 && lanes_on && (uint64_t)npc + 6u * 64u + 16u <= cap_pc && (uint64_t)npar + 65u <= cap_par) {
          if (ab_skip > 0) ab_skip--;
          else {
            if (!nstop_tab && !build_nstop()) return -3;
            const bool memo = nattr >= 16;
            const uint32_t maxc = memo ? 64u : 16u - nattr;
            if (memo && !chain) { chain = (wptr)ws_alloc(c, ((uint64_t)nstop + 8) * 4); if (!chain) return -3; }
            if (cbase != 0xFFFFFFFFu && cbase + SG_EVC < nev && ei + 1024u > cbase + SG_EVC) { cbase = 0xFFFFFFFFu; bbase = 0xFFFFFFFFu; }
            need(ei);
            const uint32_t wend = cbase + SG_EVC < nev ? cbase + SG_EVC : nev;
            const uint32_t lim = wend < nev ? wend - 1u : wend;
            const uint32_t send = ei + 1024u < lim ? ei + 1024u : lim;
            uint32_t nc = 1;
            lanes_sync();
            for (uint32_t base = ei; base < send && nc < maxc; base += 64) {
              const uint32_t idx = base + (uint32_t)l;
              const bool in = idx < send;
              const uint32_t v = in ? g_fuse_lds[idx - cbase] : 0u;
              const uint32_t vn = (in && idx + 1u < nev) ? g_fuse_lds[idx + 1u - cbase] : 0u;
              const uint32_t cl = v & 15u;
              const bool adj = in && idx + 1u < nev && (vn >> 4) == (v >> 4) + 1u && ((ES_WS >> (vn & 15u)) & 1u);
              const bool is = in && (((ES_WS >> cl) & 1u) || cl == E_SQ || cl == E_DQ) && !adj;
              const unsigned long long m = __ballot(is);
              const uint32_t rank = nc + (uint32_t)__popcll(m & ((1ull << l) - 1ull));
              if (is && rank < 64) g_fuse_lds[SG_EVC + rank] = idx;
              nc += (uint32_t)__popcll(m);
            }
            if (nc > maxc) nc = maxc;
            lanes_sync();
            const bool mine = (uint32_t)l < nc;
            const uint32_t cj = (l > 0 && mine) ? g_fuse_lds[SG_EVC + (uint32_t)l] : cbase;
            const uint32_t cv = g_fuse_lds[cj - cbase];
            const uint32_t cpos = l == 0 ? pos : (cv >> 4) + 1u, cei = l == 0 ? ei : cj + 1u, cws = l == 0 ? (ws_sp ? 1u : 0u) : ((cv & 15u) == E_SPACE ? 1u : 0u);
            SgLaneMemo mm; mm.gt = ff_gt; mm.qgt = ff_qgt; mm.cmt = ff_cmt; mm.sq = ff_sq; mm.dq = ff_dq; mm.bad = bad; mm.nstop = nstop_tab;
            SgLaneAttr A; A.term = 1; A.npos = 0; A.nei = 0; A.nws = 0; A.an = 0; A.ae = 0; A.va = 0; A.vb = 0; A.delim = 0; A.eqpos = 0; A.reach = 0;
            if (mine) A = sg_lane_attr(H, L, ev, nev, cbase, cpos, cei, cws, mm);
            const uint32_t isbad = (memo && mine && bad && cpos < L) ? (uint32_t)bad[cpos] : 0u;
            const uint32_t cpos_nx = (uint32_t)__shfl((int)cpos, (l + 1) & 63);
            const unsigned long long termm = __ballot(!mine || A.term != 0 || isbad != 0);
            const unsigned long long linkm = __ballot(mine && (uint32_t)l + 1u < nc && A.npos == cpos_nx);
            const unsigned long long chainable = linkm & ~termm & (~termm >> 1);
            unsigned long long visited = 0; uint32_t k = 0, cnt = 0;
            for (;;) {
              if ((termm >> k) & 1ull) break;
              const uint32_t r = (uint32_t)__builtin_ctzll(~(chainable >> k));
              visited |= ((2ull << r) - 1ull) << k; cnt += r + 1u; k += r;
              if ((linkm >> k) & 1ull) break;
              const uint32_t np = (uint32_t)__builtin_amdgcn_readlane((int)A.npos, (int)k);
              const unsigned long long m = __ballot(mine && (uint32_t)l > k && cpos == np);
              if (!m) break;
              k = (uint32_t)__builtin_ctzll(m);
            }
            if (cnt == 0) { ab_skip = ab_penalty; if (ab_penalty < 64) ab_penalty *= 2; }
            else {
              const bool cm = (visited >> l) & 1ull;
              const uint32_t rank = (uint32_t)__popcll(visited & ((1ull << l) - 1ull));
              if (cm) {
                SgParam q; q.na = A.an; q.nb = A.ae; q.va = A.va; q.vb = A.vb; q.delim = A.delim; q.pad = 0; par[npar + rank] = q;
                const bool has = A.vb > A.va, hd = has && A.delim != 0;
                cbptr qp = sglit(A.delim == 1 ? SL_SQ : SL_DQ);
                EH_G Piece* o = pc + npc + 6u * rank; Piece x; x.rep = 1;
                x.ptr = (uint64_t)(cws ? H + A.an - 1 : sglit(SL_SP)); x.len = 1; o[0] = x;
                x.ptr = (uint64_t)(H + A.an); x.len = A.ae - A.an; o[1] = x;
                x.ptr = (uint64_t)(has ? H + A.eqpos : sglit(SL_EQ)); x.len = has ? 1u : 0u; o[2] = x;
                x.ptr = (uint64_t)(hd ? H + A.va - 1 : qp); x.len = hd ? 1u : 0u; o[3] = x;
                x.ptr = (uint64_t)(H + A.va); x.len = has ? A.vb - A.va : 0u; o[4] = x;
                x.ptr = (uint64_t)(hd ? H + A.vb : qp); x.len = hd ? 1u : 0u; o[5] = x;
                if (memo) chain[nchain + rank] = cpos;
              }
              const uint32_t lastc = 63u - (uint32_t)__builtin_clzll(visited);
              pos = (uint32_t)__builtin_amdgcn_readlane((int)A.npos, (int)lastc); ei = (uint32_t)__builtin_amdgcn_readlane((int)A.nei, (int)lastc);
              ws_sp = (uint32_t)__builtin_amdgcn_readlane((int)A.nws, (int)lastc) != 0;
              npar += cnt; npc += 6u * cnt; nattr += cnt; if (memo) nchain += cnt;
              if (rp_state != 0) { const uint32_t r = wave_max(cm ? A.reach : 0u); if (r > reach_ev) reach_ev = r; }
              bbase = 0xFFFFFFFFu;
              wave_sync();
              ab_penalty = 1;
#ifdef EH_PROF
              if (l == 0) { atomicAdd(&c.p->prof[2 * 120], (unsigned long long)cnt); atomicAdd(&c.p->prof[2 * 120 + 1], 1ull); }
#endif
              continue;
            }
          }
        }
        if (nattr >= 16) {
          if (bad && uni(bad[pos])) break;
          if (!chain) { chain = (wptr)ws_alloc(c, ((uint64_t)nstop + 8) * 4); if (!chain) return -3; }
          if (l == 0) chain[nchain] = pos;
          nchain++;
        }
        uint32_t ca = cls_here();
        if (ca == E_SLGT) { put(ws_sp ? H + pos - 1 : sglit(SL_SPSLGT), 3); kind = TK_SC; next = pos + 2; nexte = ei + 2; ok = true; break; }
        if (ca == E_GT) { put(H + pos, 1); kind = TK_OPEN; next = pos + 1; nexte = ei + 1; ok = true; break; }
        const bool sp_before = ws_sp;
        if (ca == E_EQ) break;
        uint32_t an = pos;
        step1();
        uint32_t ja = find_stop(ei, ES_STOP);
        if (ja == 0xFFFFFFFFu) return -3;
        if (ja >= nev) break;
        uint32_t ae = evget(ja) >> 4; pos = ae; ei = ja;
        skipws();
        uint32_t va = pos, vb = pos, delim = 0, eqpos = 0xFFFFFFFFu;
        if (pos < L && cls_here() == E_EQ) {
          eqpos = pos;
          step1(); skipws();
          if (pos >= L) break;
          uint32_t cv = cls_here();
          if (cv == E_SQ || cv == E_DQ) {
            uint32_t jq = cv == E_SQ ? find1(ei + 1, E_SQ, ff_sq) : find1(ei + 1, E_DQ, ff_dq);
            if (jq >= nev) break;
            va = pos + 1; vb = evget(jq) >> 4; delim = cv == E_SQ ? 1u : 2u;
            pos = vb + 1; ei = jq + 1;
          } else {
            uint32_t ju = find_stop(ei, ES_STOP);
            if (ju == 0xFFFFFFFFu) return -3;
            if (ju >= nev) break;
            va = pos; vb = evget(ju) >> 4; pos = vb; ei = ju;
          }
          skipws();
        }
        if (l == 0) { SgParam q; q.na = an; q.nb = ae; q.va = va; q.vb = vb; q.delim = delim; q.pad = 0; par[npar] = q; }
        npar++; nattr++;
        bool has = vb > va;
        cbptr qp = sglit(delim == 1 ? SL_SQ : SL_DQ);
        put(sp_before ? H + an - 1 : sglit(SL_SP), 1); put(H + an, ae - an);
        put(has ? H + eqpos : sglit(SL_EQ), has ? 1u : 0u); put(has && delim ? H + va - 1 : qp, has && delim ? 1u : 0u);
        put(H + va, has ? vb - va : 0u); put(has && delim ? H + vb : qp, has && delim ? 1u : 0u);
      }
    } while (false);
    if (c.status != CASE_OK) return -3;
    if (ok) SG_TZ(88); else SG_TZ(87);
    SG_CNT(118, npar - par0);
    SG_SUB0();
    if (ok) {
      if (!first) {
        if (l == 0) { Piece q; q.ptr = (uint64_t)(H + seg_start); q.len = lt - seg_start; q.rep = 1; pc[seg_slot] = q; }
        text_len += lt - seg_start;
        if (l == 0) { SgTok t; t.kind = TK_TEXT | (text_len == 0 ? (uint32_t)TF_EMPTY : 0u); t.p0 = text_p0; t.np = seg_slot + 1 - text_p0; t.na = 0; t.nb = 0; t.par0 = 0; t.npar = 0; t.match = -1; tok[ntok] = t; }
        ntok++;
      }
      if (l == 0) { SgTok t; t.kind = kind; t.p0 = tag_p0; t.np = npc - tag_p0; t.na = na; t.nb = nb; t.par0 = par0; t.npar = npar - par0; t.match = -1; tok[ntok] = t; }
      ntok++;
      first = false;
      pos = next; ei = nexte; seg_start = next; text_p0 = npc; text_len = 0;
      fail_run = 0;
      { const int r = after_accept(); if (r) return r; }
      SG_SUB(113);
    } else {
      if (first) { rc = other ? -2 : -1; break; }
      if (nchain > 0) {
        if (!bad) {
          bad = ws_alloc(c, (uint64_t)L + 16);
          if (!bad) return -3;
          for (uint32_t i = 16u * (uint32_t)l; i < L + 16; i += 1024) { uint4 z = {0, 0, 0, 0}; stg16(bad + i, z); }
        }
        wave_sync();
        for (uint32_t i = l; i < nchain; i += 64) bad[chain[i]] = 1;
        wave_sync();
      }
      npc = seg_slot; npar = par0;
      if (tag0 > lt + 1) {
        put(H + seg_start, lt + 1 - seg_start);
        text_len += lt + 1 - seg_start; seg_start = tag0;
      }
      pos = tag0; ei = ei0;
      fail_run++;
    }
    SG_SUB0();
    { const int r = lane_batches(); if (r) return r; }
    SG_SUB(114);
    uint32_t j = find(ei, 1u << E_LT);
    SG_SUB(115);
    if (j >= nev) {
      uint32_t n = L - seg_start;
      put(H + seg_start, n); text_len += n;
      if (l == 0) { SgTok t; t.kind = TK_TEXT | (text_len == 0 ? (uint32_t)TF_EMPTY : 0u); t.p0 = text_p0; t.np = npc - text_p0; t.na = 0; t.nb = 0; t.par0 = 0; t.npar = 0; t.match = -1; tok[ntok] = t; }
      ntok++;
      break;
    }
    lt = evget(j) >> 4; seg_slot = npc; npc++;
    pos = lt + 1; ei = j + 1;
  }
  wave_sync();
  if (rc != 0) return rc;
  if (l == 0) { out->tok = tok; out->par = par; out->pc = pc; out->ntok = ntok; out->npar = npar; out->npc = npc; }
  wave_sync();
  return 0;
}

EH_DEV uint32_t latin1_lower(uint32_t ch) { return ((ch >= 'A' && ch <= 'Z') || (ch >= 0xC0 && ch <= 0xD6) || (ch >= 0xD8 && ch <= 0xDE)) ? ch + 32 : ch; }
EH_DEV uint32_t sg_name_hash(cbptr H, uint32_t a, uint32_t b) {
  uint32_t h = 0;
  for (uint32_t i = a + (uint32_t)EH_LANE; i < b; i += 64) {
    uint32_t v = (latin1_lower(H[i]) + 1u) * (0x9E3779B1u * ((i - a) + 1u) | 1u);
    uint32_t r = (i - a) & 31u;
    h += (v << r) | (r ? v >> (32 - r) : 0u);
  }
  return wave_sum(h) ^ ((b - a) * 0x85EBCA6Bu);
}
EH_DEV bool sg_name_eq(cbptr H, uint32_t a1, uint32_t b1, uint32_t a2, uint32_t b2) {
  if (b1 - a1 != b2 - a2) return false;
  uint32_t n = b1 - a1; bool ne = false;
  for (uint32_t i = EH_LANE; i < n; i += 64) ne |= latin1_lower(H[a1 + i]) != latin1_lower(H[a2 + i]);
  return __ballot(ne) == 0;
}

EH_DEV void sgml_pair(cbptr H, EH_G SgTok* tok, uint32_t ntok, wptr stk) {
  const int l = EH_LANE;
  uint32_t depth = 0;
  for (uint32_t base = 0; base < ntok; base += 64) {
    uint32_t idx = base + (uint32_t)l;
    uint32_t kind = 0, na = 0, nb = 0;
    if (idx < ntok) { SgTok t = tok[idx]; kind = t.kind & TK_KIND; na = t.na; nb = t.nb; }
    unsigned long long oc = __ballot(kind == TK_OPEN || kind == TK_CLOSE);
    while (oc) {
      int j = (int)__builtin_ctzll(oc); oc &= oc - 1;
      uint32_t k = (uint32_t)__builtin_amdgcn_readlane((int)kind, j), a = (uint32_t)__builtin_amdgcn_readlane((int)na, j), b = (uint32_t)__builtin_amdgcn_readlane((int)nb, j);
      uint32_t ti = base + (uint32_t)j;
      uint32_t h = sg_name_hash(H, a, b);
      if (k == TK_OPEN) {
        if (l == 0) { stk[2 * depth] = ti; stk[2 * depth + 1] = h; }
        depth++;
        continue;
      }
      wave_sync();
      uint32_t hi = depth; bool found = false; uint32_t at = 0;
      while (hi > 0 && !found) {
        uint32_t lo = hi > 64 ? hi - 64 : 0;
        uint32_t d = lo + (uint32_t)l;
        bool cand = d < hi && stk[2 * d + 1] == h;
        unsigned long long cm = __ballot(cand);
        while (cm && !found) {
          int q = 63 - (int)__builtin_clzll(cm); cm &= ~(1ull << q);
          uint32_t dd = lo + (uint32_t)q;
          uint32_t ot = uni(stk[2 * dd]);
          SgTok o = tok[ot];
          if (sg_name_eq(H, uni(o.na), uni(o.nb), a, b)) { found = true; at = dd; }
        }
        hi = lo;
      }
      if (found) {
        uint32_t ot = uni(stk[2 * at]);
        if (l == 0) { tok[ot].match = (int32_t)ti; tok[ot].kind |= TF_PAIRED; tok[ti].match = (int32_t)ot; tok[ti].kind |= TF_PAIRED; }
        depth = at;
      }
    }
  }
  wave_sync();
}

EH_DEV void sgml_flags(const EH_G SgTok* tok, uint32_t ntok, bptr ef, uint32_t* N, uint32_t* NT) {
  uint32_t n = 0, nt = 0;
  for (uint32_t i = EH_LANE; i < ntok; i += 64) {
    uint32_t k = tok[i].kind;
    uint32_t kk = k & TK_KIND;
// ... 368 lines not shown
```

erlamsa_amd/csrc/eh_tree.h:

```cpp
#pragma once
#include "eh_lex.h"

namespace eh {

struct TNode { uint32_t open, close, pend, pad; };

EH_DEV uint32_t usual_delim_close(uint32_t c) {
  switch (c) { case 40: return 41; case 91: return 93; case 60: return 62; case 123: return 125; case 34: return 34; case 39: return 39; }
  return 0;
}
struct DelimCls {
  EH_DEV uint32_t operator()(uint32_t b) const {
    switch (b) { case 40: return 1; case 41: return 2; case 91: return 3; case 93: return 4; case 60: return 5; case 62: return 6;
                 case 123: return 7; case 125: return 8; case 34: return 9; case 39: return 10; }
    return 0;
  }
};
EH_DEV uint32_t delim_close_code(uint32_t code) { return code == 9 ? 9u : (code == 10 ? 10u : code + 1); }
EH_DEV bool delim_is_opener(uint32_t code) { return code == 1 || code == 3 || code == 5 || code == 7 || code == 9 || code == 10; }
EH_DEV bool delim_bit(uint32_t b, uint32_t w1, uint32_t w23) { uint32_t m = b < 32 ? 0u : (b < 64 ? w1 : (b < 128 ? w23 : 0u)); return (m >> (b & 31u)) & 1u; }
struct IsOpener { EH_DEV bool operator()(uint32_t b, uint32_t) const { return delim_bit(b, (1u << 2) | (1u << 7) | (1u << 8) | (1u << 28), 1u << 27); } };

#ifndef EH_TREE_S
#define EH_TREE_S 32
// ... 223 lines not shown
      while (ekm) {
        const uint32_t j = (uint32_t)__builtin_ctz(ekm); ekm &= ekm - 1;
        const uint32_t cd = uni((uint32_t)tl_bytes()[4 * TL_COD + (uint32_t)k * TL_SP + j]);
        if (sp > 0 && cd == (top & 255u)) {
          if ((uint32_t)l == nclose) { cs = top >> 8; ce = ev0 + j; }
          nclose++;
          rs_pop();
          cur = sp > 0 ? top >> 8 : 0xFFFFFFFFu;
          if (nclose == 64) w_flush();
        }
        if (l == 0) g_fuse_lds[TL_TOP + (uint32_t)k * TL_S + e] = cur;
        e++;
      }
      if (dk > 0) {
        if (sp - sbase + dk > 64) rs_spill();
        const uint32_t at = sp - sbase, i = (uint32_t)l - at;
        const bool in = (uint32_t)l >= at && i < dk;
        const uint32_t en = in ? (uint32_t)tl_stack()[i * 64 + (uint32_t)k] : 0u;
        const uint32_t enp = (in && i > 0) ? (uint32_t)tl_stack()[(i - 1) * 64 + (uint32_t)k] : 0u;
        const uint32_t j = en >> 4, slot = ob + (uint32_t)__popc(okm & ((1u << j) - 1));
        if (in) {
          stk = (slot << 8) | (en & 15u);
          tab[slot].open = ev0 + j; tab[slot].pend = i > 0 ? ob + (uint32_t)__popc(okm & ((1u << (enp >> 4)) - 1)) : cur;
        }
        sp += dk;
        top = (uint32_t)__builtin_amdgcn_readlane((int)stk, (int)(sp - 1 - sbase));
        cur = top >> 8;
      }
      if (sj < TL_S) {
        const uint32_t rem = TL_S - sj;
        uint32_t mc = (uint32_t)l < rem ? (uint32_t)tl_bytes()[4 * TL_COD + (uint32_t)k * TL_SP + sj + (uint32_t)l] : 0u;
        mc |= delim_is_opener(mc) ? (0x100u | (delim_close_code(mc) << 16)) : 0u;
        const unsigned long long opm = __ballot((mc & 0x100u) != 0);
        const uint32_t rb = ob + (uint32_t)__popc(okm & ((1u << sj) - 1));
        for (uint32_t e2 = 0; e2 < rem; e2++) {
          const uint32_t code = (uint32_t)__builtin_amdgcn_readlane((int)mc, (int)e2);
          if (sp > 0 && (code & 255u) == (top & 255u)) {
            if ((uint32_t)l == nclose) { cs = top >> 8; ce = ev0 + sj + e2; }
            nclose++;
            rs_pop();
            if (nclose == 64) w_flush();
          } else if (code & 0x100u) {
            const uint32_t parent = sp > 0 ? top >> 8 : 0xFFFFFFFFu;
            const uint32_t slot = rb + (uint32_t)__popcll(opm & ((1ull << e2) - 1));
            if ((uint32_t)l == npush) { ps = slot; pe = ev0 + sj + e2; pp = parent; }
            npush++;
            rs_push((slot << 8) | (code >> 16));
            if (npush == 64) w_flush();
          }
        }
        nseq += rem;
      }
      if (l == k) topout = sp > 0 ? top >> 8 : 0xFFFFFFFFu;
    }
    w_flush();
    lanes_sync();
    {
      const unsigned long long below = items & ((1ull << l) - 1);
      const uint32_t t = (uint32_t)__shfl((int)topout, below ? 63 - (int)__builtin_clzll(below) : 0);
      if (!((items >> l) & 1ull)) topin = below ? t : top0;
    }
    {
      const uint32_t lb = 4 * TL_LNK + (uint32_t)l * TL_SP, ev0 = eb + (uint32_t)l * TL_S;
      uint32_t m = cm;
      while (m) {
        const uint32_t j = (uint32_t)__builtin_ctz(m); m &= m - 1;
        const uint32_t jo = tl_bytes()[lb + j], lp = tl_bytes()[lb + jo];
        const uint32_t slot = obase + (uint32_t)__popc(om & ((1u << jo) - 1));
        uint32_t par;
        if (lp != 255u) par = obase + (uint32_t)__popc(om & ((1u << lp) - 1));
        else { const uint32_t e = (uint32_t)__popc(em & ((1u << jo) - 1)); par = e ? g_fuse_lds[TL_TOP + (uint32_t)l * TL_S + e - 1] : topin; }
        tab[slot].open = ev0 + jo; tab[slot].close = ev0 + j; tab[slot].pend = par;
      }
    }
    orank += (uint32_t)__builtin_amdgcn_readlane((int)oinc, 63);
    eb += committed;
    nlane += committed - nseq; TL_COUNT(0, committed - nseq); TL_COUNT(1, 1);
    if (2 * nseq > committed) { TL_COUNT(2, 1); seq_left = seq_len; if (seq_len < TL_SEQ_MAX) seq_len *= 2; }
    else if (seq_len > TL_SEQ_MIN) seq_len /= 2;
  }
  wave_sync();
  TR_PH(12);
#ifdef EH_PROF
  if (l == 0) { atomicAdd(&c.p->prof[2 * 86], (unsigned long long)nlane); atomicAdd(&c.p->prof[2 * 86 + 1], (unsigned long long)nquote); }
#endif
  (void)nlane; (void)nquote;
  for (uint32_t i = (uint32_t)l; i < nopen; i += 64) {
    if (tab[i].close == 0xFFFFFFFFu) continue;
    uint32_t par = tab[i].pend, pe = L;
    if (par != 0xFFFFFFFFu) { uint32_t pc = tab[par].close; if (pc != 0xFFFFFFFFu) pe = evp[pc] + 1; }
    tab[i].pad = pe;
  }
  wave_sync();
  TR_PH(13);
  uint32_t n = 0;
  for (uint32_t base = 0; base < nopen; base += 64) {
    uint32_t i = base + (uint32_t)l;
    TNode t{0, 0xFFFFFFFFu, 0, 0};
    if (i < nopen) t = tab[i];
    bool ok = i < nopen && t.close != 0xFFFFFFFFu;
    unsigned long long m = __ballot(ok);
    uint32_t before = (uint32_t)__popcll(m & ((1ull << l) - 1));
    wave_sync();
    if (ok) { t.open = evp[t.open]; t.close = evp[t.close]; t.pend = t.pad; tab[n + before] = t; }
    n += (uint32_t)__popcll(m);
    wave_sync();
  }
  TR_PH(14);
  *out = tab;
  return (int)n;
}

EH_DEV bool node_eq(cbptr H, TNode a, TNode b) {
  uint32_t la = a.close - a.open + 1, lb = b.close - b.open + 1;
  if (la != lb) return false;
  if (a.open == b.open) return true;
  return wave_equal(H + a.open, H + b.open, la);
}
EH_DEV TNode node_load(const EH_G TNode* t, uint32_t i) { TNode x = t[i]; x.open = uni(x.open); x.close = uni(x.close); x.pend = uni(x.pend); return x; }

EH_DEV unsigned long long nodes_equal_mask(cbptr H, uint32_t my_open, bool cand, TNode sub) {
  uint32_t n = sub.close - sub.open + 1;
  if (n > 256) {
    unsigned long long cm = __ballot(cand), res = 0;
    while (cm) {
      int j = (int)__builtin_ctzll(cm); cm &= cm - 1;
      uint32_t o = (uint32_t)__builtin_amdgcn_readlane((int)my_open, j);
      if (o == sub.open || wave_equal(H + o, H + sub.open, n)) res |= 1ull << j;
    }
    return res;
  }
  bool ne = !cand;
  bool self = cand && my_open == sub.open;
  uint32_t k = 0;
  for (; k + 8 <= n; k += 8) {
    uint64_t a = 0, b;
    b = ldg8(H + sub.open + k);
    if (!ne && !self) a = ldg8(H + my_open + k);
    ne = ne || (!self && a != b);
    if (__ballot(!ne && !self) == 0) break;
  }
  if (k + 8 <= n) return __ballot(!ne);
  for (; k < n; k++) { uint32_t b = H[sub.open + k]; if (!ne && !self && H[my_open + k] != b) ne = true; }
  return __ballot(!ne);
}
template <class F>
EH_DEV void tree_matches(cbptr H, const EH_G TNode* nodes, uint32_t lo, uint32_t hi, uint32_t level_end, TNode sub, wptr anc, F f) {
  (void)anc;
  const int l = EH_LANE;
  (void)l;
  uint32_t skip_until = 0;
  uint32_t slen = sub.close - sub.open;
  for (uint32_t base = lo; base < hi; base += 64) {
    uint32_t i = base + (uint32_t)l;
    TNode q{0, 0, 0, 0};
    if (i < hi) q = nodes[i];
    bool cand = i < hi && q.close - q.open == slen && q.open >= skip_until;
    if (__ballot(cand) == 0) continue;
    unsigned long long cm = nodes_equal_mask(H, q.open, cand, sub);
    while (cm) {
      int j = (int)__builtin_ctzll(cm); cm &= cm - 1;
      TNode x; x.open = (uint32_t)__builtin_amdgcn_readlane((int)q.open, j); x.close = (uint32_t)__builtin_amdgcn_readlane((int)q.close, j);
      x.pend = (uint32_t)__builtin_amdgcn_readlane((int)q.pend, j); x.pad = 0;
      if (x.open < skip_until) continue;
      f(x, base + (uint32_t)j);
      skip_until = x.pend < level_end ? x.pend : level_end;
    }
// ... 270 lines not shown
```

erlamsa_amd/engine.py:

```python
import ctypes as C
import os

import numpy as np

_HERE = os.path.dirname(os.path.abspath(__file__))
LIB_PATH = os.environ.get("ERLAMSA_HIP_LIB") or os.path.join(_HERE, "liberlamsa_hip.so")

EH_ABI_VERSION = 8
EH_FLAG_ORDERED_OUTPUT = 1
EH_FLAG_META_TRACE = 2
EH_FLAG_FUSE_NO_LDS = 4
EH_FLAG_FUSE_NO_REDUCE = 8
EH_FLAG_SGML_NO_REPLAY = 16
EH_FLAG_SGML_NO_LANES = 32
EH_FLAG_NO_COOP = 64

UNIQUE_PIECE_BYTES = 65536

CASE_OK, CASE_CRASHED, CASE_OVERFLOW, CASE_UNSUPPORTED, CASE_ARENA_FULL, CASE_BUDGET = 0, 1, 2, 3, 4, 5

ABI_SYMBOLS = [
    "eh_create", "eh_destroy", "eh_configure", "eh_corpus_upload", "eh_corpus_attach", "eh_fuzz_batch",
    "eh_fuzz_calls", "eh_reserve", "eh_sync", "eh_result_device", "eh_result_download", "eh_result_fetch", "eh_result_totals", "eh_result_summary", "eh_result_occupancy", "eh_result_diag", "eh_result_cycles", "eh_result_peak", "eh_result_meta", "eh_result_write_files", "eh_result_prof", "eh_selftest_movers", "eh_selftest_zlib",
    "eh_last_kernel_ms", "eh_pool_stats", "eh_coop_stats", "eh_kernel_name", "eh_abi_version", "eh_mutator_count", "eh_mutator_name",
    "eh_mutator_default_pri", "eh_mutator_on_gpu", "eh_pattern_count", "eh_pattern_name",
    "eh_pattern_default_pri", "eh_pattern_on_gpu", "eh_strerror", "eh_last_error",
    "eh_coalesce_limits", "eh_submit", "eh_flush", "eh_poll", "eh_cancel",
    "eh_corpus_device", "eh_stream", "eh_host_alloc", "eh_host_free", "eh_selftest_sort_by_priority", "eh_last_error_copy",
    "eh_comm_unique_id", "eh_comm_init", "eh_comm_init_local", "eh_comm_destroy", "eh_corpus_broadcast", "eh_corpus_allgather",
    "eh_corpus_broadcast_local", "eh_device_count", "eh_meta_atom_count", "eh_meta_atom_name", "eh_batch_done",
    "eh_result_digests", "eh_result_unique", "eh_result_download_select", "eh_selftest_unique",
    "eh_profile_add", "eh_profile_count", "eh_fuzz_calls_profiled", "eh_submit_profiled",
    "eh_seen_reserve", "eh_seen_count", "eh_seen_add_keys", "eh_seen_add_corpus", "eh_seen_export", "eh_result_seen", "eh_selftest_seen",
    "eh_corpus_promote", "eh_corpus_promote_fresh", "eh_corpus_download", "eh_selftest_promote",
]

SEEN_FRESH, SEEN_IN_BATCH, SEEN_BEFORE, SEEN_NOT_OK = 0, 1, 2, 3

PROMOTE_REPLACE, PROMOTE_APPEND = 0, 1

MAX_PROFILES = 1024


class EhOptions(C.Structure):
    _fields_ = [("abi_version", C.c_uint32), ("mutations", C.c_char_p), ("patterns", C.c_char_p),
                ("generators", C.c_char_p), ("blockscale", C.c_double), ("ssrf_host", C.c_char_p),
                ("ssrf_port", C.c_int32), ("max_case_bytes", C.c_uint64), ("out_capacity", C.c_uint64),
                ("max_case_work", C.c_uint64), ("max_slots", C.c_uint32), ("flags", C.c_uint32), ("big_case_bytes", C.c_uint64),
                ("pool_bytes", C.c_uint64), ("download_chunk_bytes", C.c_uint64), ("fuse_stream_min", C.c_uint64),
                ("sequence_muta", C.c_uint32), ("reserved0", C.c_uint32)]


class EngineError(RuntimeError):
    def __init__(self, code, msg):
        super().__init__("erlamsa_hip error %d: %s" % (code, msg))
        self.code = code


_lib = None


def load_library():
    global _lib
    if _lib is not None:
        return _lib
    import sys
    if "torch" in sys.modules:
        import torch
        if torch.cuda.is_available():
            torch.cuda.init()
    if not os.path.exists(LIB_PATH):
        raise ImportError("%s not built: run `python -c 'import __graft_entry__ as g; g.build()'`" % LIB_PATH)
    lib = C.CDLL(LIB_PATH)
    vp, u64p, i64p, i32p = C.c_void_p, C.POINTER(C.c_uint64), C.POINTER(C.c_int64), C.POINTER(C.c_int32)
    lib.eh_create.argtypes = [C.c_int, C.POINTER(vp)]
    lib.eh_destroy.argtypes = [vp]
    lib.eh_destroy.restype = None
    lib.eh_configure.argtypes = [vp, C.POINTER(EhOptions)]
    lib.eh_corpus_upload.argtypes = [vp, vp, vp, C.c_uint64]
    lib.eh_corpus_attach.argtypes = [vp, vp, vp, C.c_uint64, C.c_uint64]
    lib.eh_fuzz_batch.argtypes = [vp, i64p, C.c_uint64, C.c_uint64, C.c_uint64, vp]
    lib.eh_fuzz_calls.argtypes = [vp, vp, C.c_uint64, C.c_uint64, vp]
    lib.eh_sync.argtypes = [vp]
    lib.eh_batch_done.argtypes = [vp, C.POINTER(C.c_int)]
    lib.eh_reserve.argtypes = [vp, C.c_uint64]
    lib.eh_result_device.argtypes = [vp, C.POINTER(vp), C.POINTER(vp), C.POINTER(vp), C.POINTER(vp), u64p]
    lib.eh_result_download.argtypes = [vp, vp, C.c_uint64, vp, vp]
    lib.eh_result_totals.argtypes = [vp, u64p, u64p, u64p]
    lib.eh_result_fetch.argtypes = [vp, C.c_uint64, vp, C.c_uint64, u64p]
    lib.eh_result_diag.argtypes = [vp, vp, vp]
    lib.eh_result_cycles.argtypes = [vp, vp]
    lib.eh_result_peak.argtypes = [vp, vp]
    lib.eh_result_write_files.argtypes = [vp, C.c_char_p, C.c_uint64, C.c_uint32, u64p, u64p, u64p]
    lib.eh_result_meta.argtypes = [vp, C.c_uint64, vp, C.c_uint64, u64p]
    lib.eh_result_prof.argtypes = [vp, vp]
    lib.eh_selftest_movers.argtypes = [vp, vp, C.c_uint64, vp, C.c_uint32, vp]
    lib.eh_selftest_zlib.argtypes = [vp, C.c_int, vp, C.c_uint64, vp, C.c_uint64, vp, vp]
    lib.eh_result_digests.argtypes = [vp, vp]
    lib.eh_result_unique.argtypes = [vp, vp, u64p, u64p]
    lib.eh_result_download_select.argtypes = [vp, vp, C.c_uint64, vp, C.c_uint64, vp]
    lib.eh_selftest_unique.argtypes = [vp, vp, vp, vp, C.c_uint64, vp, vp]
    lib.eh_seen_reserve.argtypes = [vp, C.c_uint64]
    lib.eh_seen_count.argtypes = [vp, vp]
    lib.eh_seen_add_keys.argtypes = [vp, vp, C.c_uint64, u64p]
    lib.eh_seen_add_corpus.argtypes = [vp, u64p]
    lib.eh_seen_export.argtypes = [vp, vp, C.c_uint64, u64p]
    lib.eh_result_seen.argtypes = [vp, C.c_uint32, vp, u64p, u64p]
    lib.eh_selftest_seen.argtypes = [vp, vp, vp, vp, C.c_uint64, C.c_uint32, vp]
    lib.eh_corpus_promote.argtypes = [vp, vp, C.c_uint64, C.c_uint32, u64p, u64p]
    lib.eh_corpus_promote_fresh.argtypes = [vp, C.c_uint64, C.c_uint64, C.c_uint32, u64p, u64p]
    lib.eh_corpus_download.argtypes = [vp, vp, C.c_uint64, vp, C.c_uint64, u64p, u64p]
    lib.eh_selftest_promote.argtypes = [vp, vp, vp, vp, vp, C.c_uint64, vp, C.c_uint64, C.c_uint64, C.c_uint64, C.c_uint32, u64p, u64p]
    lib.eh_last_kernel_ms.argtypes = [vp, C.POINTER(C.c_float)]
    lib.eh_pool_stats.argtypes = [vp, vp]
    lib.eh_result_summary.argtypes = [vp, vp]
    lib.eh_result_occupancy.argtypes = [vp, vp]
    lib.eh_coop_stats.argtypes = [vp, vp]
    lib.eh_coalesce_limits.argtypes = [vp, C.c_uint64, C.c_uint64]
    lib.eh_submit.argtypes = [vp, vp, C.c_uint64, i64p, u64p]
    lib.eh_flush.argtypes = [vp]
    lib.eh_profile_add.argtypes = [vp, C.c_char_p, C.c_char_p, C.c_double, C.POINTER(C.c_uint32)]
    lib.eh_profile_count.argtypes = [vp, C.POINTER(C.c_uint32)]
    lib.eh_fuzz_calls_profiled.argtypes = [vp, vp, vp, C.c_uint64, C.c_uint64, vp]
    lib.eh_submit_profiled.argtypes = [vp, vp, C.c_uint64, i64p, C.c_uint32, u64p]
    lib.eh_meta_atom_name.restype = C.c_char_p
    lib.eh_meta_atom_name.argtypes = [C.c_int]
    lib.eh_comm_unique_id.argtypes = [vp]
    lib.eh_comm_init.argtypes = [vp, vp, C.c_int, C.c_int]
    lib.eh_comm_init_local.argtypes = [vp, C.c_int]
    lib.eh_comm_destroy.argtypes = [vp]
    lib.eh_corpus_broadcast.argtypes = [vp, C.c_int, vp, vp, C.c_uint64]
    lib.eh_corpus_allgather.argtypes = [vp, vp, vp, C.c_uint64]
    lib.eh_corpus_broadcast_local.argtypes = [vp, C.c_int, C.c_int]
    lib.eh_cancel.argtypes = [vp, C.c_uint64]
    lib.eh_poll.argtypes = [vp, C.c_uint64, vp, C.c_uint64, u64p, C.POINTER(C.c_int32)]
    lib.eh_corpus_device.argtypes = [vp, C.POINTER(vp), C.POINTER(vp), u64p, u64p]
    lib.eh_stream.argtypes = [vp, C.POINTER(vp)]
    lib.eh_host_alloc.argtypes = [C.POINTER(vp), C.c_uint64]
    lib.eh_host_free.argtypes = [vp]
    lib.eh_host_free.restype = None
    lib.eh_selftest_sort_by_priority.argtypes = [vp, C.c_uint32, vp]
    lib.eh_kernel_name.restype = C.c_char_p
    lib.eh_abi_version.restype = C.c_uint32
    for f in ("eh_mutator_name", "eh_pattern_name", "eh_strerror"):
        getattr(lib, f).restype = C.c_char_p
        getattr(lib, f).argtypes = [C.c_int]
    lib.eh_last_error.restype = C.c_char_p
    lib.eh_last_error.argtypes = [vp]
    _lib = lib
    return lib


def mutator_table():
    lib = load_library()
    return [(lib.eh_mutator_name(i).decode(), lib.eh_mutator_default_pri(i), bool(lib.eh_mutator_on_gpu(i)))
            for i in range(lib.eh_mutator_count())]


def pattern_table():
    lib = load_library()
    return [(lib.eh_pattern_name(i).decode(), lib.eh_pattern_default_pri(i), bool(lib.eh_pattern_on_gpu(i)))
            for i in range(lib.eh_pattern_count())]


def sort_by_priority(pris):
    p = np.ascontiguousarray(pris, dtype=np.uint32)
    perm = np.zeros(max(len(p), 1), dtype=np.uint32)
    rc = load_library().eh_selftest_sort_by_priority(p.ctypes.data, len(p), perm.ctypes.data)
    if rc != 0:
        raise EngineError(rc, "eh_selftest_sort_by_priority")
    return [int(x) for x in perm[:len(p)]]


def gpu_mutators():
    return [n for n, _, g in mutator_table() if g]


def gpu_patterns():
    return [n for n, _, g in pattern_table() if g]
# ... 341 lines not shown
                                               idx.ctypes.data, len(idx), int(max_entry_bytes), int(max_total_bytes),
                                               PROMOTE_APPEND if append else PROMOTE_REPLACE, C.byref(t), C.byref(tb)))
        self.n_corpus = self.corpus_size()[0]
        return t.value, tb.value

    def download_into(self, host_ptr, cap):
        n = self.last_n
        off = np.zeros(n + 1, dtype=np.uint64)
        status = np.zeros(max(n, 1), dtype=np.int32)
        self._chk(self.lib.eh_result_download(self.h, C.c_void_p(host_ptr), cap, off.ctypes.data, status.ctypes.data))
        return off, status[:n]

    def status(self):
        n = self.last_n
        st = np.zeros(max(n, 1), dtype=np.int32)
        self._chk(self.lib.eh_result_download(self.h, None, 0, None, st.ctypes.data))
        return st[:n]

    def diag(self):
        n = self.last_n
        draws = np.zeros(max(n, 1), dtype=np.uint64)
        lastm = np.zeros(max(n, 1), dtype=np.int32)
        self._chk(self.lib.eh_result_diag(self.h, draws.ctypes.data, lastm.ctypes.data))
        return draws[:n], lastm[:n]

    def cycles(self):
        n = self.last_n
        cyc = np.zeros(max(n, 1), dtype=np.uint64)
        self._chk(self.lib.eh_result_cycles(self.h, cyc.ctypes.data))
        return cyc[:n]

    def write_files(self, template, first_number=1, threads=0):
        f, b, s = C.c_uint64(), C.c_uint64(), C.c_uint64()
        self._chk(self.lib.eh_result_write_files(self.h, template.encode(), first_number, threads, C.byref(f), C.byref(b), C.byref(s)))
        return f.value, b.value, s.value

    def meta_raw(self, i):
        buf = (C.c_uint8 * 32768)()
        n = C.c_uint64()
        self._chk(self.lib.eh_result_meta(self.h, i, buf, 32768, C.byref(n)))
        return bytes(buf[:min(n.value, 32768)])

    def meta_atoms(self):
        return [self.lib.eh_meta_atom_name(k).decode() for k in range(self.lib.eh_meta_atom_count())]

    def meta_terms(self, i):
        from . import meta as _meta
        return _meta.decode(self.meta_raw(i), self.meta_atoms())

    def meta(self, i):
        from . import meta as _meta
        terms, cut = self.meta_terms(i)
        out = _meta.legacy(terms, [self.lib.eh_mutator_name(k).decode() for k in range(self.lib.eh_mutator_count())])
        return out + ([("truncated", "")] if cut else [])

    def peak(self):
        n = self.last_n
        pk = np.zeros(max(n, 1), dtype=np.uint64)
        self._chk(self.lib.eh_result_peak(self.h, pk.ctypes.data))
        return pk[:n]

    def prof(self):
        pr = np.zeros(256, dtype=np.uint64)
        self._chk(self.lib.eh_result_prof(self.h, pr.ctypes.data))
        return pr

    def selftest_zlib(self, op, data, cap=None):
        src = np.frombuffer(bytes(data), dtype=np.uint8) if len(data) else np.zeros(1, dtype=np.uint8)
        if cap is None:
            cap = len(data) + len(data) // 8 + 1024 if op <= 2 else max(64 * len(data), 1 << 20)
        out = np.zeros(cap + 16, dtype=np.uint8)
        n = C.c_uint64(0)
        ok = C.c_int32(0)
        self._chk(self.lib.eh_selftest_zlib(self.h, op, src.ctypes.data, len(data), out.ctypes.data, cap, C.byref(n), C.byref(ok)))
        return bytes(out[:n.value]) if ok.value else None

    def selftest_movers(self, buf, jobs):
        buf = np.ascontiguousarray(buf, dtype=np.uint8).copy()
        jobs = np.ascontiguousarray(jobs, dtype=np.uint32)
        eq = np.zeros(len(jobs), dtype=np.uint32)
        self._chk(self.lib.eh_selftest_movers(self.h, buf.ctypes.data, buf.size, jobs.ctypes.data, len(jobs), eq.ctypes.data))
        return buf, eq

    def coalesce_limits(self, flush_cases, flush_bytes):
        self._chk(self.lib.eh_coalesce_limits(self.h, flush_cases, flush_bytes))

    def submit(self, data, seed, profile=0):
        b = bytes(data)
        t = C.c_uint64()
        buf = (C.c_char * max(len(b), 1)).from_buffer_copy(b or b"\0")
        if profile == 0:
            self._chk(self.lib.eh_submit(self.h, C.cast(buf, C.c_void_p), len(b), (C.c_int64 * 3)(*seed), C.byref(t)))
        else:
            self._chk(self.lib.eh_submit_profiled(self.h, C.cast(buf, C.c_void_p), len(b), (C.c_int64 * 3)(*seed), profile, C.byref(t)))
        return t.value

    def flush(self):
        self._chk(self.lib.eh_flush(self.h))

    def cancel(self, ticket):
        self._chk(self.lib.eh_cancel(self.h, ticket))

    def poll(self, ticket, cap=1 << 16):
        while True:
            out = (C.c_uint8 * cap)()
            n, st = C.c_uint64(), C.c_int32()
            rc = self.lib.eh_poll(self.h, ticket, out, cap, C.byref(n), C.byref(st))
            if rc == -7:
                return None
            if rc == -1 and n.value > cap:
                cap = int(n.value)
                continue
            self._chk(rc)
            return st.value, C.string_at(out, n.value)

    def result_device(self):
        d, o, l, s = C.c_void_p(), C.c_void_p(), C.c_void_p(), C.c_void_p()
        tot = C.c_uint64()
        self._chk(self.lib.eh_result_device(self.h, C.byref(d), C.byref(o), C.byref(l), C.byref(s), C.byref(tot)))
        return d.value, o.value, l.value, s.value, tot.value


class HostBuffer:

    def __init__(self, size):
        self.lib = load_library()
        p = C.c_void_p()
        rc = self.lib.eh_host_alloc(C.byref(p), size)
        if rc != 0:
            raise EngineError(rc, self.lib.eh_strerror(rc).decode())
        self.ptr, self.size = p.value, size
        self.array = np.ctypeslib.as_array(C.cast(p, C.POINTER(C.c_uint8)), shape=(max(size, 1),))

    def free(self):
        if self.ptr:
            self.array = None
            self.lib.eh_host_free(C.c_void_p(self.ptr))
            self.ptr = None

    def __del__(self):
        try:
            self.free()
        except Exception:
            pass
```

include/erlamsa_hip.h:

```cpp
#ifndef ERLAMSA_HIP_H
#define ERLAMSA_HIP_H
#include <stdint.h>
#ifdef __cplusplus
extern "C" {
#endif

#define EH_ABI_VERSION 8

typedef struct eh_ctx eh_ctx;

enum eh_error {
  EH_OK = 0,
  EH_E_INVALID = -1,
  EH_E_NODEVICE = -2,
  EH_E_HIP = -3,
  EH_E_NOMEM = -4,
  EH_E_STATE = -5,
  EH_E_UNSUPPORTED = -6,
  EH_E_AGAIN = -7
};

enum eh_case_status {
  EH_CASE_OK = 0,
  EH_CASE_CRASHED = 1,
// ... 45 lines not shown
int eh_comm_init(eh_ctx* ctx, const uint8_t id[128], int rank, int nranks);
int eh_comm_init_local(eh_ctx** ctxs, int nctx);
int eh_comm_destroy(eh_ctx* ctx);
int eh_corpus_broadcast(eh_ctx* ctx, int root, const uint8_t* data, const uint64_t* off, uint64_t n);
int eh_corpus_allgather(eh_ctx* ctx, const uint8_t* data, const uint64_t* off, uint64_t n_local);
int eh_corpus_broadcast_local(eh_ctx** ctxs, int nctx, int root);

int eh_corpus_device(eh_ctx* ctx, const void** d_data, const void** d_off, uint64_t* n, uint64_t* nbytes);

int eh_stream(eh_ctx* ctx, void** stream);

int eh_host_alloc(void** p, uint64_t bytes);
void eh_host_free(void* p);

int eh_reserve(eh_ctx* ctx, uint64_t max_cases);

int eh_fuzz_batch(eh_ctx* ctx, const int64_t seed[3], uint64_t first_case, uint64_t corpus_first, uint64_t n,
                  void* stream);
int eh_fuzz_calls(eh_ctx* ctx, const int64_t* seeds, uint64_t corpus_first, uint64_t n, void* stream);
int eh_sync(eh_ctx* ctx);
int eh_batch_done(eh_ctx* ctx, int* done);

int eh_coalesce_limits(eh_ctx* ctx, uint64_t flush_cases, uint64_t flush_bytes);
int eh_submit(eh_ctx* ctx, const uint8_t* data, uint64_t len, const int64_t seed[3], uint64_t* ticket);
int eh_flush(eh_ctx* ctx);
int eh_poll(eh_ctx* ctx, uint64_t ticket, uint8_t* out, uint64_t cap, uint64_t* out_len, int32_t* status);
int eh_cancel(eh_ctx* ctx, uint64_t ticket);

#define EH_MAX_PROFILES 1024
int eh_profile_add(eh_ctx* ctx, const char* mutations, const char* patterns, double blockscale, uint32_t* id);
int eh_profile_count(eh_ctx* ctx, uint32_t* n);
int eh_fuzz_calls_profiled(eh_ctx* ctx, const int64_t* seeds, const uint32_t* profile, uint64_t corpus_first, uint64_t n, void* stream);
int eh_submit_profiled(eh_ctx* ctx, const uint8_t* data, uint64_t len, const int64_t seed[3], uint32_t profile, uint64_t* ticket);

int eh_result_device(eh_ctx* ctx, const uint8_t** d_data, const uint64_t** d_off, const uint64_t** d_len,
                     const int32_t** d_status, uint64_t* total_bytes);
int eh_result_download(eh_ctx* ctx, uint8_t* data, uint64_t cap, uint64_t* off, int32_t* status);
int eh_result_fetch(eh_ctx* ctx, uint64_t i, uint8_t* buf, uint64_t cap, uint64_t* out_len);
int eh_result_totals(eh_ctx* ctx, uint64_t* in_bytes, uint64_t* out_bytes, uint64_t* n_cases);
int eh_result_summary(eh_ctx* ctx, uint64_t* out);
int eh_result_occupancy(eh_ctx* ctx, uint64_t* out);
int eh_result_diag(eh_ctx* ctx, uint64_t* draws, int32_t* last_mutator);

int eh_result_cycles(eh_ctx* ctx, uint64_t* cycles);

int eh_result_write_files(eh_ctx* ctx, const char* name_template, uint64_t first_number, uint32_t threads,
                          uint64_t* files_written, uint64_t* bytes_written, uint64_t* not_written);

int eh_meta_atom_count(void);
const char* eh_meta_atom_name(int id);
int eh_result_meta(eh_ctx* ctx, uint64_t i, uint8_t* buf, uint64_t cap, uint64_t* n_events);

#define EH_UNIQUE_PIECE_BYTES 65536
int eh_result_digests(eh_ctx* ctx, uint64_t* digest);
int eh_result_unique(eh_ctx* ctx, uint64_t* first_of, uint64_t* n_unique, uint64_t* unique_bytes);
int eh_result_download_select(eh_ctx* ctx, const uint64_t* idx, uint64_t m, uint8_t* data, uint64_t cap, uint64_t* off);
int eh_selftest_unique(eh_ctx* ctx, const uint8_t* data, const uint64_t* off, const int32_t* status, uint64_t n,
                       uint64_t* digest, uint64_t* first_of);

int eh_seen_reserve(eh_ctx* ctx, uint64_t capacity);
int eh_seen_count(eh_ctx* ctx, uint64_t out[4]);
int eh_seen_add_keys(eh_ctx* ctx, const uint64_t* keys, uint64_t m, uint64_t* added);
int eh_seen_add_corpus(eh_ctx* ctx, uint64_t* added);
int eh_seen_export(eh_ctx* ctx, uint64_t* keys, uint64_t cap_keys, uint64_t* n);
int eh_result_seen(eh_ctx* ctx, uint32_t commit, uint8_t* cls, uint64_t* n_fresh, uint64_t* fresh_bytes);
int eh_selftest_seen(eh_ctx* ctx, const uint8_t* data, const uint64_t* off, const int32_t* status, uint64_t n, uint32_t commit,
                     uint8_t* cls);

#define EH_PROMOTE_REPLACE 0u
#define EH_PROMOTE_APPEND 1u
int eh_corpus_promote(eh_ctx* ctx, const uint64_t* idx, uint64_t m, uint32_t mode, uint64_t* n_after, uint64_t* bytes_after);
int eh_corpus_promote_fresh(eh_ctx* ctx, uint64_t max_entry_bytes, uint64_t max_total_bytes, uint32_t mode, uint64_t* taken,
                            uint64_t* taken_bytes);
int eh_corpus_download(eh_ctx* ctx, uint8_t* data, uint64_t cap, uint64_t* off, uint64_t cap_entries, uint64_t* n, uint64_t* nbytes);
int eh_selftest_promote(eh_ctx* ctx, const uint8_t* data, const uint64_t* off, const int32_t* status, const uint8_t* cls, uint64_t n,
                        const uint64_t* idx, uint64_t m, uint64_t max_entry_bytes, uint64_t max_total_bytes, uint32_t mode,
                        uint64_t* taken, uint64_t* taken_bytes);

int eh_result_peak(eh_ctx* ctx, uint64_t* peak);

int eh_result_prof(eh_ctx* ctx, uint64_t* prof);

int eh_selftest_movers(eh_ctx* ctx, uint8_t* buf, uint64_t buf_len, const uint32_t* jobs, uint32_t njobs, uint32_t* eq_out);
int eh_selftest_zlib(eh_ctx* ctx, int op, const uint8_t* in, uint64_t n, uint8_t* out, uint64_t cap, uint64_t* out_len, int32_t* ok);

int eh_selftest_sort_by_priority(const uint32_t* pri, uint32_t n, uint32_t* perm);

int eh_pool_stats(eh_ctx* ctx, uint64_t* out);
int eh_coop_stats(eh_ctx* ctx, uint64_t* out);

int eh_last_kernel_ms(eh_ctx* ctx, float* ms);
const char* eh_kernel_name(void);

uint32_t eh_abi_version(void);
int eh_mutator_count(void);
const char* eh_mutator_name(int id);
int eh_mutator_default_pri(int id);
int eh_mutator_on_gpu(int id);
int eh_pattern_count(void);
const char* eh_pattern_name(int id);
int eh_pattern_default_pri(int id);
int eh_pattern_on_gpu(int id);
const char* eh_strerror(int code);
const char* eh_last_error(eh_ctx* ctx);
uint64_t eh_last_error_copy(eh_ctx* ctx, char* buf, uint64_t cap);

#ifdef __cplusplus
}
#endif
#endif
```

Measured before the change: 96270.

## Batch cooperative chunk claims and offload periodic fills to helper waves

```diff
diff --git a/erlamsa_amd/csrc/eh_co_claim.h b/erlamsa_amd/csrc/eh_co_claim.h
--- /dev/null
+++ b/erlamsa_amd/csrc/eh_co_claim.h
@@ -0,0 +1,28 @@
+#pragma once
+#include <cstdint>
+
+namespace eh {
+
+constexpr uint32_t co_claim_len(uint32_t handed, uint32_t nchunks, uint32_t div, uint32_t cap) {
+  const uint32_t rem = handed < nchunks ? nchunks - handed : 0;
+  const uint32_t k = rem / (div ? div : 1u);
+  const uint32_t hi = cap ? cap : 1u;
+  return k < 1u ? 1u : (k > hi ? hi : k);
+}
+
+struct CoSpan { uint64_t off; uint32_t len; };
+constexpr CoSpan co_chunk_span(uint64_t n, uint32_t ch, uint32_t t) {
+  const uint64_t off = (uint64_t)t * ch;
+  return off >= n ? CoSpan{n, 0u} : CoSpan{off, n - off < ch ? (uint32_t)(n - off) : ch};
+}
+constexpr uint64_t co_chunk_count(uint64_t n, uint32_t ch) { return (n + ch - 1) / ch; }
+
+constexpr uint32_t CO_FILL_PREFIX = 64u << 10;
+constexpr uint64_t co_fill_prefix(uint32_t plen) { return plen ? (((uint64_t)CO_FILL_PREFIX + plen - 1) / plen) * plen : 0; }
+struct CoFillSpan { uint64_t off; uint32_t len; uint64_t src; };
+constexpr CoFillSpan co_fill_span(uint64_t K, uint64_t total, uint32_t ch, uint32_t t) {
+  const uint64_t off = K + (uint64_t)t * ch;
+  return off >= total ? CoFillSpan{total, 0u, 0u} : CoFillSpan{off, total - off < ch ? (uint32_t)(total - off) : ch, off % K};
+}
+
+}
diff --git a/erlamsa_amd/csrc/eh_common.h b/erlamsa_amd/csrc/eh_common.h
--- a/erlamsa_amd/csrc/eh_common.h
+++ b/erlamsa_amd/csrc/eh_common.h
@@ -1,5 +1,6 @@
 #pragma once
 #include <stdint.h>
+#include "eh_co_claim.h"
 
 #if defined(__HIP_DEVICE_COMPILE__) && !defined(HIPEMU)
 #define EH_G __attribute__((address_space(1)))
@@ -117,11 +118,12 @@
 };
 
 constexpr uint32_t CO_JOBS = 64, CO_ARGS = 12;
-enum CoKind : uint32_t { CO_COPY = 1, CO_EQUAL = 2, CO_FBPASS = 3, CO_FBCOUNT = 4 };
+enum CoKind : uint32_t { CO_COPY = 1, CO_EQUAL = 2, CO_FBPASS = 3, CO_FBCOUNT = 4, CO_FILL = 5 };
 struct CoJob {
   uint64_t a[CO_ARGS];
   unsigned long long acc;
-  uint32_t kind, nchunks, done, pad;
+  uint32_t kind, nchunks, done;
+  uint32_t cost;
 };
 struct CoBoard {
   unsigned long long word[CO_JOBS];
@@ -177,7 +179,9 @@
   uint64_t batch_seq;
   uint32_t co_copy_min, co_copy_chunk;
   uint32_t co_fb_min, co_fb_chunk;
-  uint32_t co_linger, pad_co;
+  uint32_t co_linger;
+  uint32_t co_claim_div, co_claim_max;
+  uint32_t co_fill_min;
   const EH_G ProfileCfg* profiles;
   const EH_G uint32_t* profile_id;
 };
diff --git a/erlamsa_amd/csrc/eh_device.h b/erlamsa_amd/csrc/eh_device.h
--- a/erlamsa_amd/csrc/eh_device.h
+++ b/erlamsa_amd/csrc/eh_device.h
@@ -204,16 +204,14 @@
   wave_sync();
   if (tk) dst[done + l] = t;
 }
-EH_DEV void wave_fill_periodic(bptr dst, cbptr pat, uint32_t plen, uint64_t total) {
-  if (total == 0) return;
-  uint64_t have = plen < total ? plen : total;
-  wave_copy(dst, pat, (uint32_t)have);
-  while (have < total) {
-    wave_sync();
-    uint64_t chunk = have < total - have ? have : total - have;
-    uint64_t done = 0;
-    while (done < chunk) { uint32_t c = chunk - done > 0x40000000ull ? 0x40000000u : (uint32_t)(chunk - done); wave_copy(dst + have + done, dst + done, c); done += c; }
-    have += chunk;
+__device__ void wave_fill_periodic(bptr dst, cbptr pat, uint32_t plen, uint64_t total);
+EH_DEV void wave_fill_from_prefix(bptr dst, uint64_t K, uint64_t off, uint64_t len, uint64_t src) {
+  while (len) {
+    uint64_t piece = K - src < len ? K - src : len;
+    if (piece > 0x40000000ull) piece = 0x40000000ull;
+    wave_copy_raw(dst + off, dst + src, (uint32_t)piece);
+    off += piece; len -= piece; src += piece;
+    if (src == K) src = 0;
   }
 }
 EH_DEV bool wave_equal_raw(cbptr a, cbptr b, uint32_t n) {
@@ -415,7 +413,7 @@
 }
 EH_DEV uint32_t co_ld32(const EH_G uint32_t* p) { return __atomic_load_n(p, __ATOMIC_RELAXED); }
 EH_DEV unsigned long long co_ld64(const EH_G unsigned long long* p) { return __atomic_load_n(p, __ATOMIC_RELAXED); }
-__device__ __noinline__ bool co_run(uint32_t kind, uint32_t nchunks, CoArgs args, unsigned long long* acc) {
+__device__ __noinline__ bool co_run(uint32_t kind, uint32_t nchunks, uint32_t cost, CoArgs args, unsigned long long* acc) {
   Ctx& c = g_ctx;
   EH_G CoBoard* bd = c.p ? c.p->board : nullptr;
   const int l = EH_LANE;
@@ -433,7 +431,7 @@
   if (l == 0) {
 #pragma unroll
     for (uint32_t k = 0; k < CO_ARGS; k++) j->a[k] = args.a[k];
-    j->kind = kind; j->nchunks = nchunks; j->done = 0; j->acc = 0;
+    j->kind = kind; j->nchunks = nchunks; j->done = 0; j->acc = 0; j->cost = cost;
   }
   wave_sync();
   co_release();
@@ -445,14 +443,17 @@
     atomicAdd(&bd->stat[0], 1ull);
   }
   c.co_posted = 1;
-  uint32_t mine = 0;
+  const uint32_t div = uni(c.p->co_claim_div), cap = uni(c.p->co_claim_max);
+  uint32_t mine = 0, seen = 0;
   for (;;) {
+    const uint32_t k = co_claim_len(seen, nchunks, div, cap);
     unsigned long long old = 0;
-    if (l == 0) old = atomicAdd(&bd->word[slot], 1ull);
-    const uint32_t t = uni((uint32_t)old);
-    if (t >= nchunks) break;
-    co_exec(j, t);
-    mine++;
+    if (l == 0) old = atomicAdd(&bd->word[slot], (unsigned long long)k);
+    const uint32_t t0 = uni((uint32_t)old);
+    if (t0 >= nchunks) break;
+    const uint32_t t1 = nchunks - t0 < k ? nchunks : t0 + k;
+    for (uint32_t t = t0; t < t1; t++) co_exec(j, t);
+    mine += t1 - t0; seen = t1;
   }
   wave_sync();
   unsigned long long sum = 0;
@@ -472,50 +473,92 @@
   if (acc) *acc = sum;
   return true;
 }
-__device__ __noinline__ void co_help(EH_G CoBoard* bd, uint32_t most) {
+__device__ __noinline__ void co_help(EH_G CoBoard* bd, uint32_t budget, uint32_t div, uint32_t cap) {
   const int l = EH_LANE;
-  uint32_t ran = 0;
-  for (uint32_t guard = 0; guard < 64 && ran < most; guard++) {
+  uint32_t spent = 0;
+  for (uint32_t guard = 0; guard < 64 && spent < budget; guard++) {
     if (uni(co_ld32(&bd->open)) == 0) return;
     const unsigned long long w = co_ld64(&bd->word[l]);
-    const bool cand = ((w >> 32) & 1ull) && (uint32_t)w < co_ld32(&bd->job[l].nchunks);
+    const uint32_t nch_l = co_ld32(&bd->job[l].nchunks), cost_l = co_ld32(&bd->job[l].cost);
+    const bool cand = ((w >> 32) & 1ull) && (uint32_t)w < nch_l;
     unsigned long long m = __ballot(cand);
     if (!m) return;
     const uint32_t rot = blockIdx.x & 63u;
     const unsigned long long mr = rot ? ((m >> rot) | (m << (64u - rot))) : m;
     const uint32_t s = ((uint32_t)__builtin_ctzll(mr) + rot) & 63u;
+    const uint32_t handed = uni((uint32_t)__shfl((int)(uint32_t)w, (int)s)), nch_s = uni((uint32_t)__shfl((int)nch_l, (int)s));
+    uint32_t cost = uni((uint32_t)__shfl((int)cost_l, (int)s)); if (cost == 0) cost = 1;
+    uint32_t k = co_claim_len(handed, nch_s, div, cap);
+    const uint32_t room = (budget - spent) / cost;
+    if (k > room) k = room ? room : 1u;
     unsigned long long old = 0;
-    if (l == 0) old = atomicAdd(&bd->word[s], 1ull);
+    if (l == 0) old = atomicAdd(&bd->word[s], (unsigned long long)k);
     old = uni64(old);
     if (!((old >> 32) & 1ull)) continue;
     co_acquire();
     const EH_G CoJob* j = &bd->job[s];
-    const uint32_t nchunks = uni(co_ld32(&j->nchunks)), t = (uint32_t)old;
-    if (uni64(co_ld64(&bd->word[s])) >> 32 != old >> 32 || t >= nchunks) continue;
-    co_exec(j, t);
-    ran++;
+    const uint32_t nchunks = uni(co_ld32(&j->nchunks)), t0 = (uint32_t)old;
+    if (uni64(co_ld64(&bd->word[s])) >> 32 != old >> 32 || t0 >= nchunks) continue;
+    const uint32_t t1 = nchunks - t0 < k ? nchunks : t0 + k;
+    cost = uni(co_ld32(&j->cost)); if (cost == 0) cost = 1;
+    for (uint32_t t = t0; t < t1; t++) co_exec(j, t);
+    const uint32_t ran = t1 - t0;
+    const uint64_t did = (uint64_t)ran * cost;
+    spent = did >= budget - spent ? budget : spent + (uint32_t)did;
     wave_sync();
     co_release();
-    if (l == 0) { atomicAdd(&bd->job[s].done, 1u); atomicAdd(&bd->stat[1], 1ull); }
-  }
-}
-__device__ __noinline__ void co_copy(bptr dst, cbptr src, uint32_t n) {
-  const EH_G KParams* kp = g_ctx.p;
-  if (!kp || !kp->board || n < kp->co_copy_min) { wave_copy_raw(dst, src, n); return; }
-  const uint32_t ch = kp->co_copy_chunk;
+    if (l == 0) { atomicAdd(&bd->job[s].done, ran); atomicAdd(&bd->stat[1], (unsigned long long)ran); }
+  }
+}
+__device__ __noinline__ void co_copy_with(bptr dst, cbptr src, uint32_t n, uint32_t min, uint32_t ch) {
+  if (!ch || n < min) { wave_copy_raw(dst, src, n); return; }
   CoArgs a; for (uint32_t k = 0; k < CO_ARGS; k++) a.a[k] = 0;
   a.a[0] = (uint64_t)dst; a.a[1] = (uint64_t)src; a.a[2] = n; a.a[3] = ch;
-  if (!co_run(CO_COPY, (n + ch - 1) / ch, a, nullptr)) wave_copy_raw(dst, src, n);
-}
-__device__ __noinline__ bool co_equal(cbptr x, cbptr y, uint32_t n) {
-  const EH_G KParams* kp = g_ctx.p;
-  if (!kp || !kp->board || n < 2 * kp->co_copy_min) return wave_equal_raw(x, y, n);
-  const uint32_t ch = kp->co_copy_chunk;
+  if (!co_run(CO_COPY, (uint32_t)co_chunk_count(n, ch), ch, a, nullptr)) wave_copy_raw(dst, src, n);
+}
+__device__ __noinline__ bool co_equal_with(cbptr x, cbptr y, uint32_t n, uint32_t min, uint32_t ch) {
+  if (!ch || n < 2ull * min) return wave_equal_raw(x, y, n);
   CoArgs a; for (uint32_t k = 0; k < CO_ARGS; k++) a.a[k] = 0;
   a.a[0] = (uint64_t)x; a.a[1] = (uint64_t)y; a.a[2] = n; a.a[3] = ch;
   unsigned long long ne = 0;
-  if (!co_run(CO_EQUAL, (n + ch - 1) / ch, a, &ne)) return wave_equal_raw(x, y, n);
+  if (!co_run(CO_EQUAL, (uint32_t)co_chunk_count(n, ch), ch, a, &ne)) return wave_equal_raw(x, y, n);
   return ne == 0;
+}
+__device__ __noinline__ void co_fill_with(bptr dst, cbptr pat, uint32_t plen, uint64_t total, uint32_t min, uint32_t ch) {
+  if (total == 0 || plen == 0) return;
+  const uint64_t K = co_fill_prefix(plen), head = K < total ? K : total;
+  uint64_t have = plen < head ? plen : head;
+  wave_copy(dst, pat, (uint32_t)have);
+  while (have < head) {
+    wave_sync();
+    const uint64_t step = have < head - have ? have : head - have;
+    wave_fill_from_prefix(dst, have, have, step, 0);
+    have += step;
+  }
+  if (head == total) return;
+  const uint64_t rest = total - K;
+  if (ch && rest >= min && co_chunk_count(rest, ch) < (1ull << 31)) {
+    CoArgs a; for (uint32_t k = 0; k < CO_ARGS; k++) a.a[k] = 0;
+    a.a[0] = (uint64_t)dst; a.a[1] = K; a.a[2] = total; a.a[3] = ch;
+    if (co_run(CO_FILL, (uint32_t)co_chunk_count(rest, ch), ch, a, nullptr)) return;
+  }
+  wave_sync();
+  wave_fill_from_prefix(dst, K, K, rest, 0);
+}
+__device__ __noinline__ void co_copy(bptr dst, cbptr src, uint32_t n) {
+  const EH_G KParams* kp = g_ctx.p;
+  const bool on = kp && kp->board;
+  co_copy_with(dst, src, n, on ? kp->co_copy_min : 0u, on ? kp->co_copy_chunk : 0u);
+}
+__device__ __noinline__ bool co_equal(cbptr x, cbptr y, uint32_t n) {
+  const EH_G KParams* kp = g_ctx.p;
+  const bool on = kp && kp->board;
+  return co_equal_with(x, y, n, on ? kp->co_copy_min : 0u, on ? kp->co_copy_chunk : 0u);
+}
+__device__ __noinline__ void wave_fill_periodic(bptr dst, cbptr pat, uint32_t plen, uint64_t total) {
+  const EH_G KParams* kp = g_ctx.p;
+  const bool on = kp && kp->board;
+  co_fill_with(dst, pat, plen, total, on ? kp->co_fill_min : 0u, on ? kp->co_copy_chunk : 0u);
 }
 
 struct LexChunk;
diff --git a/erlamsa_amd/csrc/eh_engine.hip b/erlamsa_amd/csrc/eh_engine.hip
--- a/erlamsa_amd/csrc/eh_engine.hip
+++ b/erlamsa_amd/csrc/eh_engine.hip
@@ -122,11 +122,14 @@
   const uint32_t kind = uni(co_ld32(&j->kind));
   const uint64_t a0 = uni64(j->a[0]), a1 = uni64(j->a[1]), a2 = uni64(j->a[2]);
   if (kind == CO_COPY || kind == CO_EQUAL) {
-    const uint32_t ch = uni((uint32_t)j->a[3]);
-    const uint64_t off = (uint64_t)t * ch;
-    const uint32_t len = a2 - off < ch ? (uint32_t)(a2 - off) : ch;
-    if (kind == CO_COPY) wave_copy_raw((bptr)a0 + off, (cbptr)a1 + off, len);
-    else if (!wave_equal_raw((cbptr)a0 + off, (cbptr)a1 + off, len)) { if (EH_LANE == 0) atomicAdd((EH_G unsigned long long*)&j->acc, 1ull); }
+    const CoSpan sp = co_chunk_span(a2, uni((uint32_t)j->a[3]), t);
+    if (kind == CO_COPY) wave_copy_raw((bptr)a0 + sp.off, (cbptr)a1 + sp.off, sp.len);
+    else if (!wave_equal_raw((cbptr)a0 + sp.off, (cbptr)a1 + sp.off, sp.len)) { if (EH_LANE == 0) atomicAdd((EH_G unsigned long long*)&j->acc, 1ull); }
+    return;
+  }
+  if (kind == CO_FILL) {
+    const CoFillSpan sp = co_fill_span(a1, a2, uni((uint32_t)j->a[3]), t);
+    wave_fill_from_prefix((bptr)a0, a1, sp.off, sp.len, sp.src);
     return;
   }
   if (kind == CO_FBPASS) { fb_pass_chunk(j, t); return; }
@@ -142,6 +145,8 @@
 constexpr int CTR_OCC = 272;
 constexpr int CTR_STATUS = 264;
 constexpr unsigned int CO_LINGER = 24;
+constexpr uint32_t CO_VISIT_BYTES = 512u << 10;
+constexpr uint32_t CO_LINGER_VISIT_BYTES = 2u << 20;
 #ifndef EH_WAVES_PER_SIMD
 #define EH_WAVES_PER_SIMD 2
 #endif
@@ -187,7 +192,7 @@
       if (l == 0) t = atomicAdd(p.ticket, (unsigned long long)TICKET_BATCH);
       tk_next = uni64(t); tk_end = tk_next + TICKET_BATCH;
     }
-    if (p.board && uni(co_ld32(&p.board->open)) != 0) co_help(p.board, 2);
+    if (p.board && uni(co_ld32(&p.board->open)) != 0) co_help(p.board, CO_VISIT_BYTES, p.co_claim_div, p.co_claim_max);
     uint64_t i = tk_next++;
     if (i >= p.n) {
 #ifndef HIPEMU
@@ -199,7 +204,7 @@
           EH_G CoBoard* bd = p.board;
           for (uint32_t spins = 0; spins < (1u << 24); spins++) {
             if (uni64(co_ld64(p.ticket + 3)) >= p.n || uni(co_ld32(&bd->posters)) == 0) break;
-            if (uni(co_ld32(&bd->open)) != 0) co_help(bd, 8);
+            if (uni(co_ld32(&bd->open)) != 0) co_help(bd, CO_LINGER_VISIT_BYTES, p.co_claim_div, p.co_claim_max);
             else { for (int z = 0; z < 6; z++) __builtin_amdgcn_s_sleep(127); }
           }
           linger_ticks = __builtin_amdgcn_s_memrealtime() - lg0;
@@ -380,6 +385,36 @@
   }
 }
 
+__global__ void __launch_bounds__(64) eh_test_coop_kernel(uint8_t* buf_, const uint32_t* jobs_, uint32_t njobs, uint32_t* eq_out_, const KParams* kp_, uint32_t* flag_) {
+  bptr buf = (bptr)buf_; cwptr jobs = (cwptr)jobs_; wptr eq_out = (wptr)eq_out_, flag = (wptr)flag_;
+  const EH_G KParams* kp = (const EH_G KParams*)kp_;
+  EH_G CoBoard* bd = kp->board;
+  if (blockIdx.x != 0) {
+    g_ctx.p = nullptr;
+    for (uint32_t spins = 0; spins < (1u << 18); spins++) {
+      if (uni(co_ld32(flag)) != 0) break;
+      if (uni(co_ld32(&bd->open)) != 0) co_help(bd, CO_LINGER_VISIT_BYTES, kp->co_claim_div, kp->co_claim_max);
+#ifndef HIPEMU
+      else __builtin_amdgcn_s_sleep(64);
+#endif
+    }
+    return;
+  }
+  g_ctx.p = kp; g_ctx.co_posted = 0;
+  for (uint32_t j = 0; j < njobs; j++) {
+    const uint32_t kw = jobs[5 * j], d = jobs[5 * j + 1], s = jobs[5 * j + 2], n = jobs[5 * j + 3], pl = jobs[5 * j + 4];
+    const uint32_t kind = kw & 255u, min = ((kw >> 8) & 4095u) << 8, ch = (kw >> 20) << 8;
+    if (kind == 0) co_copy_with(buf + d, buf + s, n, min, ch);
+    else if (kind == 1) co_fill_with(buf + d, buf + s, pl, n, min, ch);
+    else if (kind == 2) { bool e = co_equal_with(buf + d, buf + s, n, min, ch); if (EH_LANE == 0) eq_out[j] = e ? 1u : 0u; }
+    wave_sync();
+  }
+  if (EH_LANE == 0) {
+    if (g_ctx.co_posted) atomicAdd(&bd->posters, 0xFFFFFFFFu);
+    atomicExch(flag, 1u);
+  }
+}
+
 __global__ void __launch_bounds__(64) eh_test_zlib_kernel(int op, const uint8_t* in_, uint64_t n, uint8_t* out_, uint64_t cap, uint8_t* scratch_, uint64_t* res_) {
   cbptr in = (cbptr)in_; bptr out = (bptr)out_, scratch = (bptr)scratch_; qptr res = (qptr)res_;
   g_ctx.p = nullptr;
diff --git a/erlamsa_amd/csrc/eh_fuse.h b/erlamsa_amd/csrc/eh_fuse.h
--- a/erlamsa_amd/csrc/eh_fuse.h
+++ b/erlamsa_amd/csrc/eh_fuse.h
@@ -384,7 +384,7 @@
 jump:
 #ifdef EH_PROF
   {
-    uint32_t tot = la + lb, b = 0; while ((256u << b) < tot && b < 13) b++;
+    uint32_t tot = la + lb, b = 3; while ((256u << b) < tot && b < 13) b++;
     EH_PT(c, 112 + b);
     if (EH_LANE == 0) { atomicAdd(&c.p->prof[2 * 126], (unsigned long long)prof_rounds); atomicAdd(&c.p->prof[2 * 126 + 1], 1ull); }
   }
diff --git a/erlamsa_amd/csrc/eh_fuse2.h b/erlamsa_amd/csrc/eh_fuse2.h
--- a/erlamsa_amd/csrc/eh_fuse2.h
+++ b/erlamsa_amd/csrc/eh_fuse2.h
@@ -463,7 +463,7 @@
         a.a[0] = (uint64_t)S[s]; a.a[1] = (uint64_t)len[s] | ((uint64_t)g << 32); a.a[2] = (uint64_t)ids[s]; a.a[3] = (uint64_t)RK; a.a[4] = (uint64_t)look;
         a.a[5] = (uint64_t)kill | ((uint64_t)e_pos[s] << 32); a.a[6] = (ek ? 1u : 0u) | ((uint32_t)ins << 8) | (sc_lds ? 2u : 0u); a.a[7] = (uint64_t)mn; a.a[8] = (uint64_t)n1n; a.a[9] = nn; a.a[10] = co_chunk;
         unsigned long long acc = 0;
-        posted = co_run(CO_FBPASS, (len[s] + co_chunk - 1) / co_chunk, a, &acc);
+        posted = co_run(CO_FBPASS, (len[s] + co_chunk - 1) / co_chunk, 4u * co_chunk, a, &acc);
         alive = (uint32_t)acc;
       }
       if (!posted)
diff --git a/erlamsa_amd/csrc/eh_host_launch.h b/erlamsa_amd/csrc/eh_host_launch.h
--- a/erlamsa_amd/csrc/eh_host_launch.h
+++ b/erlamsa_amd/csrc/eh_host_launch.h
@@ -71,7 +71,7 @@
   p.slot_base = dp(ctx->d_slots); p.slot_stride = ctx->slot_stride;
   p.ntiers = pl->ntiers; p.pool_ctr = dp(pl->d_ctr); p.pool_cap[0] = pl->work_cap;
   p.board = (ctx->flags & EH_FLAG_NO_COOP) ? dp((CoBoard*)nullptr) : dp(pl->d_board);
-  co_defaults(&p, ctx->cus);
+  co_defaults(&p);
   p.summary_out = dp(ctx->res.h_sum); p.batch_seq = ++ctx->res.batch_seq;
   if (n == 0) { memset(ctx->res.h_sum, 0, 128); ctx->res.h_sum[9] = ctx->res.batch_seq; }
   for (int t = 1; t <= pl->ntiers; t++) { p.pool_base[t] = dp(pl->base[t]); p.pool_stride[t] = pl->stride[t]; p.pool_cap[t] = pl->cap[t]; p.pool_cnt[t] = pl->cnt[t]; p.pool_ring[t] = dp(pl->ring[t]); }
diff --git a/erlamsa_amd/csrc/eh_host_pool.h b/erlamsa_amd/csrc/eh_host_pool.h
--- a/erlamsa_amd/csrc/eh_host_pool.h
+++ b/erlamsa_amd/csrc/eh_host_pool.h
@@ -68,13 +68,20 @@
 }
 
 static uint32_t co_env(const char* name, uint32_t dflt) { const char* v = getenv(name); if (!v || !*v) return dflt; unsigned long long x = strtoull(v, nullptr, 10); return x > 0 && x < (1ull << 31) ? (uint32_t)x : dflt; }
-static void co_defaults(KParams* p, int cus) {
-  const bool emu = cus < 64;
-  p->co_copy_min = co_env("EH_CO_COPY_MIN", emu ? (8u << 10) : (2u << 20));
-  p->co_copy_chunk = co_env("EH_CO_COPY_CHUNK", emu ? (2u << 10) : (256u << 10));
-  p->co_fb_min = co_env("EH_CO_FB_MIN", emu ? (16u << 10) : (512u << 10));
-  p->co_fb_chunk = co_env("EH_CO_FB_CHUNK", emu ? (4u << 10) : (64u << 10)) & ~1023u;
-  { const char* v = getenv("EH_CO_LINGER"); p->co_linger = v && *v ? (uint32_t)strtoul(v, nullptr, 10) : CO_LINGER; p->pad_co = 0; }
+static void co_defaults(KParams* p) {
+#ifdef HIPEMU
+  const uint32_t copy_min = 8u << 10, copy_chunk = 2u << 10, fb_min = 16u << 10, fb_chunk = 4u << 10;
+#else
+  const uint32_t copy_min = 2u << 20, copy_chunk = 64u << 10, fb_min = 512u << 10, fb_chunk = 16u << 10;
+#endif
+  p->co_copy_min = co_env("EH_CO_COPY_MIN", copy_min);
+  p->co_copy_chunk = co_env("EH_CO_COPY_CHUNK", copy_chunk);
+  p->co_fb_min = co_env("EH_CO_FB_MIN", fb_min);
+  p->co_fb_chunk = co_env("EH_CO_FB_CHUNK", fb_chunk) & ~1023u;
+  p->co_claim_div = co_env("EH_CO_CLAIM_DIV", 4);
+  p->co_claim_max = co_env("EH_CO_CLAIM_MAX", 8);
+  { const char* v = getenv("EH_CO_LINGER"); p->co_linger = v && *v ? (uint32_t)strtoul(v, nullptr, 10) : CO_LINGER; }
+  p->co_fill_min = co_env("EH_CO_FILL_MIN", p->co_copy_min);
   if (p->co_copy_chunk < 1024) p->co_copy_chunk = 1024;
   if (p->co_fb_chunk < 1024) p->co_fb_chunk = 1024;
 }
diff --git a/erlamsa_amd/csrc/eh_host_selftest.h b/erlamsa_amd/csrc/eh_host_selftest.h
--- a/erlamsa_amd/csrc/eh_host_selftest.h
+++ b/erlamsa_amd/csrc/eh_host_selftest.h
@@ -16,6 +16,35 @@
   }
   if (e == hipSuccess) e = hipMemcpy(buf, d, buf_len, hipMemcpyDeviceToHost);
   if (e == hipSuccess && eq_out) e = hipMemcpy(eq_out, de, njobs * 4, hipMemcpyDeviceToHost);
+  HIPCHK(ctx, e);
+  return EH_OK;
+}
+int eh_selftest_coop(eh_ctx* ctx, uint8_t* buf, uint64_t buf_len, const uint32_t* jobs, uint32_t njobs, uint32_t* eq_out) {
+  if (!ctx || !buf || !jobs) return EH_E_INVALID;
+  HIPCHK(ctx, hipSetDevice(ctx->device));
+  DevBuf<uint8_t> d_buf; DevBuf<uint32_t> d_jobs, d_eq, d_flag; DevBuf<CoBoard> d_board; DevBuf<KParams> d_kp;
+  KParams p;
+  memset(&p, 0, sizeof(p));
+  hipError_t e = d_buf.grow(buf_len);
+  if (e == hipSuccess) e = d_jobs.grow(5 * (uint64_t)njobs + 1);
+  if (e == hipSuccess) e = d_eq.grow((uint64_t)njobs + 1);
+  if (e == hipSuccess) e = d_flag.grow(1);
+  if (e == hipSuccess) e = d_board.grow(1);
+  if (e == hipSuccess) e = d_kp.grow(1);
+  uint8_t* d = d_buf; uint32_t* dj = d_jobs; uint32_t* de = d_eq; uint32_t* df = d_flag; KParams* dk = d_kp;
+  if (e == hipSuccess) { p.board = dp(d_board); co_defaults(&p); }
+  if (e == hipSuccess) e = hipMemcpy(d, buf, buf_len, hipMemcpyHostToDevice);
+  if (e == hipSuccess && njobs) e = hipMemcpy(dj, jobs, (uint64_t)njobs * 20, hipMemcpyHostToDevice);
+  if (e == hipSuccess) e = hipMemcpy(dk, &p, sizeof(p), hipMemcpyHostToDevice);
+  if (e == hipSuccess) e = hipMemset(de, 0, ((uint64_t)njobs + 1) * 4);
+  if (e == hipSuccess) e = hipMemset(df, 0, 4);
+  if (e == hipSuccess) e = hipMemset(d_board, 0, sizeof(CoBoard));
+  if (e == hipSuccess) {
+    hipLaunchKernelGGL(eh_test_coop_kernel, dim3(8), dim3(64), 0, 0, d, dj, njobs, de, (const KParams*)dk, df);
+    e = hipDeviceSynchronize();
+  }
+  if (e == hipSuccess) e = hipMemcpy(buf, d, buf_len, hipMemcpyDeviceToHost);
+  if (e == hipSuccess && eq_out && njobs) e = hipMemcpy(eq_out, de, (uint64_t)njobs * 4, hipMemcpyDeviceToHost);
   HIPCHK(ctx, e);
   return EH_OK;
 }
diff --git a/erlamsa_amd/csrc/eh_sgml.h b/erlamsa_amd/csrc/eh_sgml.h
--- a/erlamsa_amd/csrc/eh_sgml.h
+++ b/erlamsa_amd/csrc/eh_sgml.h
@@ -300,7 +300,7 @@
 #define SG_SUB0() do { sub_t0 = __builtin_readcyclecounter(); } while (0)
 #define SG_SUB(k) do { uint64_t n_ = __builtin_readcyclecounter(); if (l == 0) { atomicAdd(&c.p->prof[2 * (k)], (unsigned long long)(n_ - sub_t0)); atomicAdd(&c.p->prof[2 * (k) + 1], 1ull); } sub_t0 = n_; } while (0)
 #define SG_CNT(k, v) do { if (l == 0) { atomicAdd(&c.p->prof[2 * (k)], (unsigned long long)(v)); atomicAdd(&c.p->prof[2 * (k) + 1], 1ull); } } while (0)
-  if (l == 0) { atomicAdd(&c.p->prof[2 * 117], (unsigned long long)(sub_t0 - ph1_t0)); atomicAdd(&c.p->prof[2 * 117 + 1], 1ull); atomicAdd(&c.p->prof[2 * 119], (unsigned long long)nev); atomicAdd(&c.p->prof[2 * 119 + 1], (unsigned long long)L); }
+  if (l == 0) { atomicAdd(&c.p->prof[2 * 44], (unsigned long long)(sub_t0 - ph1_t0)); atomicAdd(&c.p->prof[2 * 44 + 1], 1ull); atomicAdd(&c.p->prof[2 * 46], (unsigned long long)nev); atomicAdd(&c.p->prof[2 * 46 + 1], (unsigned long long)L); }
   uint64_t tz_t0 = __builtin_readcyclecounter();
 #define SG_TZ(k) do { uint64_t n_ = __builtin_readcyclecounter(); if (l == 0) { atomicAdd(&c.p->prof[2 * (k)], (unsigned long long)(n_ - tz_t0)); atomicAdd(&c.p->prof[2 * (k) + 1], 1ull); } tz_t0 = n_; } while (0)
 #else
@@ -377,7 +377,7 @@
     }
     wave_sync();
 #ifdef EH_PROF
-    if (l == 0) { atomicAdd(&c.p->prof[2 * 116], (unsigned long long)(__builtin_readcyclecounter() - bn_t0)); atomicAdd(&c.p->prof[2 * 116 + 1], 1ull); }
+    if (l == 0) { atomicAdd(&c.p->prof[2 * 43], (unsigned long long)(__builtin_readcyclecounter() - bn_t0)); atomicAdd(&c.p->prof[2 * 43 + 1], 1ull); }
 #endif
     return true;
   };
@@ -822,7 +822,7 @@
               wave_sync();
               ab_penalty = 1;
 #ifdef EH_PROF
-              if (l == 0) { atomicAdd(&c.p->prof[2 * 120], (unsigned long long)cnt); atomicAdd(&c.p->prof[2 * 120 + 1], 1ull); }
+              if (l == 0) { atomicAdd(&c.p->prof[2 * 47], (unsigned long long)cnt); atomicAdd(&c.p->prof[2 * 47 + 1], 1ull); }
 #endif
               continue;
             }
@@ -876,7 +876,7 @@
     } while (false);
     if (c.status != CASE_OK) return -3;
     if (ok) SG_TZ(88); else SG_TZ(87);
-    SG_CNT(118, npar - par0);
+    SG_CNT(45, npar - par0);
     SG_SUB0();
     if (ok) {
       if (!first) {
@@ -916,7 +916,7 @@
     { const int r = lane_batches(); if (r) return r; }
     SG_SUB(114);
     uint32_t j = find(ei, 1u << E_LT);
-    SG_SUB(115);
+    SG_SUB(42);
     if (j >= nev) {
       uint32_t n = L - seg_start;
       put(H + seg_start, n); text_len += n;
diff --git a/erlamsa_amd/csrc/eh_tree.h b/erlamsa_amd/csrc/eh_tree.h
--- a/erlamsa_amd/csrc/eh_tree.h
+++ b/erlamsa_amd/csrc/eh_tree.h
@@ -329,7 +329,7 @@
   wave_sync();
   TR_PH(12);
 #ifdef EH_PROF
-  if (l == 0) { atomicAdd(&c.p->prof[2 * 86], (unsigned long long)nlane); atomicAdd(&c.p->prof[2 * 86 + 1], (unsigned long long)nquote); }
+  if (l == 0) { atomicAdd(&c.p->prof[2 * 41], (unsigned long long)nlane); atomicAdd(&c.p->prof[2 * 41 + 1], (unsigned long long)nquote); }
 #endif
   (void)nlane; (void)nquote;
   for (uint32_t i = (uint32_t)l; i < nopen; i += 64) {
diff --git a/erlamsa_amd/engine.py b/erlamsa_amd/engine.py
--- a/erlamsa_amd/engine.py
+++ b/erlamsa_amd/engine.py
@@ -21,7 +21,7 @@
 
 ABI_SYMBOLS = [
     "eh_create", "eh_destroy", "eh_configure", "eh_corpus_upload", "eh_corpus_attach", "eh_fuzz_batch",
-    "eh_fuzz_calls", "eh_reserve", "eh_sync", "eh_result_device", "eh_result_download", "eh_result_fetch", "eh_result_totals", "eh_result_summary", "eh_result_occupancy", "eh_result_diag", "eh_result_cycles", "eh_result_peak", "eh_result_meta", "eh_result_write_files", "eh_result_prof", "eh_selftest_movers", "eh_selftest_zlib",
+    "eh_fuzz_calls", "eh_reserve", "eh_sync", "eh_result_device", "eh_result_download", "eh_result_fetch", "eh_result_totals", "eh_result_summary", "eh_result_occupancy", "eh_result_diag", "eh_result_cycles", "eh_result_peak", "eh_result_meta", "eh_result_write_files", "eh_result_prof", "eh_selftest_movers", "eh_selftest_coop", "eh_selftest_zlib",
     "eh_last_kernel_ms", "eh_pool_stats", "eh_coop_stats", "eh_kernel_name", "eh_abi_version", "eh_mutator_count", "eh_mutator_name",
     "eh_mutator_default_pri", "eh_mutator_on_gpu", "eh_pattern_count", "eh_pattern_name",
     "eh_pattern_default_pri", "eh_pattern_on_gpu", "eh_strerror", "eh_last_error",
@@ -95,6 +95,7 @@
     lib.eh_result_meta.argtypes = [vp, C.c_uint64, vp, C.c_uint64, u64p]
     lib.eh_result_prof.argtypes = [vp, vp]
     lib.eh_selftest_movers.argtypes = [vp, vp, C.c_uint64, vp, C.c_uint32, vp]
+    lib.eh_selftest_coop.argtypes = [vp, vp, C.c_uint64, vp, C.c_uint32, vp]
     lib.eh_selftest_zlib.argtypes = [vp, C.c_int, vp, C.c_uint64, vp, C.c_uint64, vp, vp]
     lib.eh_result_digests.argtypes = [vp, vp]
     lib.eh_result_unique.argtypes = [vp, vp, u64p, u64p]
@@ -602,6 +603,13 @@
         self._chk(self.lib.eh_selftest_movers(self.h, buf.ctypes.data, buf.size, jobs.ctypes.data, len(jobs), eq.ctypes.data))
         return buf, eq
 
+    def selftest_coop(self, buf, jobs):
+        buf = np.ascontiguousarray(buf, dtype=np.uint8).copy()
+        jobs = np.ascontiguousarray(jobs, dtype=np.uint32)
+        eq = np.zeros(len(jobs), dtype=np.uint32)
+        self._chk(self.lib.eh_selftest_coop(self.h, buf.ctypes.data, buf.size, jobs.ctypes.data, len(jobs), eq.ctypes.data))
+        return buf, eq
+
     def coalesce_limits(self, flush_cases, flush_bytes):
         self._chk(self.lib.eh_coalesce_limits(self.h, flush_cases, flush_bytes))
 
diff --git a/include/erlamsa_hip.h b/include/erlamsa_hip.h
--- a/include/erlamsa_hip.h
+++ b/include/erlamsa_hip.h
@@ -151,6 +151,7 @@
 int eh_result_prof(eh_ctx* ctx, uint64_t* prof);
 
 int eh_selftest_movers(eh_ctx* ctx, uint8_t* buf, uint64_t buf_len, const uint32_t* jobs, uint32_t njobs, uint32_t* eq_out);
+int eh_selftest_coop(eh_ctx* ctx, uint8_t* buf, uint64_t buf_len, const uint32_t* jobs, uint32_t njobs, uint32_t* eq_out);
 int eh_selftest_zlib(eh_ctx* ctx, int op, const uint8_t* in, uint64_t n, uint8_t* out, uint64_t cap, uint64_t* out_len, int32_t* ok);
 
 int eh_selftest_sort_by_priority(const uint32_t* pri, uint32_t n, uint32_t* perm);
```

Result: slower. 94370 (-2.0%).
